# seung-lab/crackle

Hardware: AMD Instinct MI355X
Metric: voxels/s encode+decode, 1024x1024x512 uint32; bit-exact .ckl bytes (higher is better)
Workload: dtype u32

## Files before the change

### crackle_amd/_lib.py

```python
import ctypes as C
import os

HERE = os.path.dirname(os.path.abspath(__file__))
LIB_PATH = os.path.join(HERE, "libcrackle_amd_tuning.so" if os.environ.get("CKL_TUNING_LIB") else
                        ("libcrackle_amd_%s.so" % os.environ["CKL_LIB_AB"]) if os.environ.get("CKL_LIB_AB") else "libcrackle_amd.so")

CKL_OK, CKL_ERR_FORMAT, CKL_ERR_RUNTIME, CKL_ERR_ARG, CKL_ERR_NO_DEVICE, CKL_ERR_CRC = range(6)
MEM_HOST, MEM_DEVICE = 0, 1


class HeaderInfo(C.Structure):
  _fields_ = [
    ("format_version", C.c_uint32), ("label_format", C.c_uint32), ("crack_format", C.c_uint32),
    ("is_signed", C.c_uint32), ("data_width", C.c_uint32), ("stored_data_width", C.c_uint32),
    ("sx", C.c_uint32), ("sy", C.c_uint32), ("sz", C.c_uint32),
    ("fortran_order", C.c_uint32), ("markov_model_order", C.c_uint32), ("is_sorted", C.c_uint32),
    ("num_label_bytes", C.c_uint64), ("header_bytes", C.c_uint64),
  ]


MERGE_UNIQUE_FN = C.CFUNCTYPE(C.c_int, C.c_void_p, C.POINTER(C.c_uint64), C.c_uint64, C.POINTER(C.c_void_p), C.POINTER(C.c_uint64))


class EncodeOverrides(C.Structure):
# ... 7 lines not shown

EXPORTS = {
  "ckl_last_error": (C.c_char_p, []),
  "ckl_abi_version": (C.c_int, []),
  "ckl_device_count": (C.c_int, []),
  "ckl_header_info_from_bytes": (C.c_int, [C.c_char_p, C.c_uint64, C.POINTER(HeaderInfo)]),
  "ckl_compress": (C.c_int, [
    C.c_void_p, C.c_int, C.c_int, C.c_int, C.c_int64, C.c_int64, C.c_int64,
    C.c_int, C.c_int, C.c_uint64, C.c_int, C.c_int, C.c_int64,
    C.c_int, C.POINTER(C.c_void_p), C.POINTER(C.c_uint64)]),
  "ckl_free": (None, [C.c_void_p]),
  "ckl_decompress": (C.c_int, [
    C.c_void_p, C.c_uint64, C.c_void_p, C.c_uint64, C.c_int,
    C.c_int64, C.c_int64, C.c_int, C.c_uint64, C.c_int]),
  "ckl_decoder_create": (C.c_int, [C.c_void_p, C.c_uint64, C.c_int64, C.c_int64, C.c_int, C.POINTER(C.c_void_p)]),
  "ckl_decoder_create_device": (C.c_int, [C.c_void_p, C.c_uint64, C.c_int64, C.c_int64, C.c_int, C.POINTER(C.c_void_p)]),
  "ckl_encoder_keep_device_stream": (C.c_int, [C.c_void_p, C.c_int]),
  "ckl_encoder_async_host_copy": (C.c_int, [C.c_void_p, C.c_int]),
  "ckl_encoder_host_wait": (C.c_int, [C.c_void_p]),
  "ckl_encoder_device_stream": (C.c_int, [C.c_void_p, C.POINTER(C.c_void_p), C.POINTER(C.c_uint64)]),
  "ckl_decoder_run": (C.c_int, [C.c_void_p, C.c_void_p, C.c_uint64, C.c_int, C.c_uint64]),
  "ckl_decoder_label_stats": (C.c_int, [C.c_void_p, C.c_uint64, C.c_void_p, C.c_void_p, C.c_void_p, C.c_void_p, C.POINTER(C.c_uint64)]),
  "ckl_decoder_contacts": (C.c_int, [C.c_void_p, C.POINTER(C.c_void_p), C.POINTER(C.c_void_p), C.POINTER(C.c_uint64)]),
  "ckl_decoder_last_timing": (C.c_int, [C.c_void_p, C.POINTER(C.c_float), C.POINTER(C.c_float)]),
  "ckl_decoder_stage_timing": (C.c_int, [C.c_void_p, C.c_int, C.POINTER(C.c_char_p), C.POINTER(C.c_float)]),
  "ckl_decoder_set_stage_events": (C.c_int, [C.c_void_p, C.c_int]),
  "ckl_decoder_destroy": (None, [C.c_void_p]),
  "ckl_encoder_create": (C.c_int, [C.c_int64, C.c_int64, C.c_int64, C.c_int, C.c_int, C.POINTER(C.c_void_p)]),
  "ckl_encoder_run": (C.c_int, [
    C.c_void_p, C.c_void_p, C.c_int64, C.c_int64, C.c_int64,
    C.c_int, C.c_int, C.c_uint64, C.c_int, C.c_int, C.c_int64,
    C.POINTER(EncodeOverrides), C.POINTER(C.c_void_p), C.POINTER(C.c_uint64)]),
  "ckl_encoder_stats": (C.c_int, [
    C.c_void_p, C.c_void_p, C.c_int64, C.c_int64, C.c_int64,
    C.POINTER(C.c_uint64), C.POINTER(C.c_uint64), C.POINTER(C.c_uint64), C.POINTER(C.c_uint64)]),
  "ckl_encoder_markov_stats": (C.c_int, [
    C.c_void_p, C.c_void_p, C.c_int64, C.c_int64, C.c_int64, C.c_int, C.c_uint64, C.c_void_p]),
  "ckl_encoder_components": (C.c_int, [
    C.c_void_p, C.c_void_p, C.c_int64, C.c_int64, C.c_int64, C.c_uint32, C.c_void_p, C.c_void_p]),
  "ckl_encoder_components_device": (C.c_int, [
    C.c_void_p, C.c_void_p, C.c_int64, C.c_int64, C.c_int64, C.c_uint32, C.c_void_p, C.c_void_p]),
  "ckl_encoder_pin_labels": (C.c_int, [
    C.c_void_p, C.c_void_p, C.c_void_p, C.c_int64, C.c_int64, C.c_int64, C.c_void_p,
    C.c_int, C.c_int, C.c_int64, C.POINTER(C.c_void_p), C.POINTER(C.c_uint64)]),
  "ckl_pins_rows_first": (C.c_int, [C.c_void_p, C.c_void_p, C.c_void_p, C.c_int64, C.c_int64, C.c_int64, C.c_int64, C.c_uint64, C.c_void_p, C.c_void_p, C.c_void_p]),
  "ckl_pins_rows_best": (C.c_int, [C.c_void_p, C.c_void_p, C.c_void_p, C.c_int64, C.c_int64, C.c_int64, C.c_int64, C.c_uint64, C.c_void_p, C.c_void_p]),
  "ckl_pins_rows_extent": (C.c_int, [C.c_void_p, C.c_void_p, C.c_void_p, C.c_int64, C.c_int64, C.c_int64, C.c_int64, C.c_uint64, C.c_void_p, C.c_void_p, C.c_void_p, C.c_void_p]),
  "ckl_pins_rows_ids": (C.c_int, [C.c_void_p, C.c_void_p, C.c_int64, C.c_int64, C.c_int64, C.c_int64, C.c_uint64, C.c_void_p, C.c_void_p, C.c_void_p, C.c_void_p]),
  "ckl_pins_rows_section": (C.c_int, [C.c_void_p, C.c_int64, C.c_int64, C.c_int64, C.c_uint64, C.c_void_p, C.c_void_p, C.c_void_p, C.c_void_p, C.c_void_p, C.c_void_p, C.c_void_p,
                                       C.c_int, C.c_int, C.c_int64, C.POINTER(C.c_void_p), C.POINTER(C.c_uint64)]),
  "ckl_encoder_walk_step_kinds": (C.c_int, [C.c_void_p, C.POINTER(C.c_uint32), C.c_uint32, C.POINTER(C.c_uint32)]),
  "ckl_encoder_last_timing": (C.c_int, [C.c_void_p, C.POINTER(C.c_float), C.POINTER(C.c_float)]),
  "ckl_encoder_walk_paths": (C.c_int, [C.c_void_p, C.POINTER(C.c_uint32), C.POINTER(C.c_uint32)]),
  "ckl_encoder_destroy": (None, [C.c_void_p]),
  "ckl_pin_labels_host": (C.c_int, [
    C.c_void_p, C.c_int, C.c_void_p, C.c_int64, C.c_int64, C.c_int64, C.c_void_p,
    C.c_int, C.c_int, C.c_int64, C.POINTER(C.c_void_p), C.POINTER(C.c_uint64)]),
  "ckl_zstack": (C.c_int, [C.POINTER(C.c_char_p), C.POINTER(C.c_uint64), C.c_uint64, C.POINTER(C.c_void_p), C.POINTER(C.c_uint64)]),
  "ckl_decoder_check": (C.c_int, [C.c_void_p, C.c_void_p, C.c_uint64]),
  "ckl_decoder_vcg": (C.c_int, [C.c_void_p, C.c_void_p, C.c_uint64, C.c_int]),
  "ckl_voxel_connectivity_graph": (C.c_int, [C.c_void_p, C.c_uint64, C.c_int, C.c_int, C.c_void_p, C.c_uint64]),
  "ckl_voxel_connectivity_graph_range": (C.c_int, [C.c_void_p, C.c_uint64, C.c_int64, C.c_int64, C.c_int, C.c_int, C.c_void_p, C.c_uint64]),
  "ckl_point_cloud": (C.c_int, [
    C.c_void_p, C.c_uint64, C.c_int64, C.c_int64, C.c_void_p, C.c_uint64, C.c_int, C.c_int, C.c_int,
    C.POINTER(C.c_void_p), C.POINTER(C.c_void_p), C.POINTER(C.c_void_p), C.POINTER(C.c_uint64)]),
  "ckl_reencode_markov": (C.c_int, [C.c_void_p, C.c_uint64, C.c_int, C.c_int, C.POINTER(C.c_void_p), C.POINTER(C.c_uint64)]),
  "ckl_decoder_crack_planes": (C.c_int, [C.c_void_p, C.POINTER(C.c_void_p), C.POINTER(C.c_void_p), C.POINTER(C.c_uint32), C.POINTER(C.c_uint64)]),
  "ckl_zsplit": (C.c_int, [C.c_void_p, C.c_uint64, C.c_int64, C.c_int64, C.POINTER(C.c_void_p), C.POINTER(C.c_uint64)]),
  "ckl_encoder_defer_codes": (C.c_int, [C.c_void_p, C.c_int]),
  "ckl_encoder_codes_to_host": (C.c_int, [C.c_void_p, C.c_void_p, C.c_uint64, C.POINTER(C.c_uint64)]),
  "ckl_host_register": (C.c_int, [C.c_void_p, C.c_uint64]),
  "ckl_host_unregister": (C.c_int, [C.c_void_p]),
  "ckl_array_equal": (C.c_int, [C.c_void_p, C.c_uint64, C.c_void_p, C.c_uint64, C.c_int, C.POINTER(C.c_int)]),
  "ckl_mode_pooling_2x2x1": (C.c_int, [C.c_void_p, C.c_uint64, C.c_int64, C.c_int64, C.c_int, C.POINTER(C.c_void_p), C.POINTER(C.c_uint64), C.POINTER(C.c_void_p), C.POINTER(C.c_uint64)]),
  "ckl_crc32c": (C.c_uint32, [C.c_void_p, C.c_uint64]),
  "ckl_crc32c_combine": (C.c_uint32, [C.c_uint32, C.c_uint32, C.c_uint64]),
}

_lib = None


def lib():
  global _lib
  if _lib is None:
    if not os.path.exists(LIB_PATH):
      raise ImportError(
        f"{LIB_PATH} is missing: build the HIP extension first "
        "(python -m crackle_amd.build, or __graft_entry__.build()). "
        "crackle_amd has no CPU fallback."
      )
    L = C.CDLL(LIB_PATH)
    for name, (res, args) in EXPORTS.items():
      f = getattr(L, name)
      f.restype = res
      f.argtypes = args
    _lib = L
  return _lib


def last_error() -> str:
  return lib().ckl_last_error().decode("utf-8", "replace")


class HostStream:

  def __init__(self, ptr: int, n: int):
    self.ptr, self.n = int(ptr), int(n)

  def __len__(self):
    return self.n

  def view(self) -> memoryview:
    return memoryview((C.c_ubyte * self.n).from_address(self.ptr)).cast("B")

  def tobytes(self) -> bytes:
    return C.string_at(self.ptr, self.n)

  __bytes__ = tobytes

  def __eq__(self, other):
    if isinstance(other, HostStream):
      return self.tobytes() == other.tobytes()
    if isinstance(other, (bytes, bytearray, memoryview)):
      return self.tobytes() == bytes(other)
    return NotImplemented

  def __del__(self):
    try:
      if self.ptr:
        lib().ckl_free(self.ptr)
        self.ptr = 0
    except Exception:
      pass


def as_pointer(binary):
  if hasattr(binary, "ptr") and hasattr(binary, "n"):
    return binary.ptr, binary.n
  return binary, len(binary)
```

### crackle_amd/csrc/ckl_decode.hip

```cpp
#include "ckl_common.hpp"
#include "ckl_runs.hpp"
#include "ckl_strips.hpp"
#include "ckl_strips2.hpp"
#include "ckl_contours.hpp"
#include "ckl_pins.hpp"

#include <algorithm>
#include <deque>
#include <chrono>
#include <memory>
#include <mutex>
#include <type_traits>
#include <tuple>

namespace ckl {

using namespace dev;

enum : uint8_t { SYM_U = 0, SYM_R = 1, SYM_D = 2, SYM_L = 3, SYM_B = 4, SYM_T = 5 };

struct CrackArgs {
	const uint8_t* stream;
	const uint64_t* code_off;
	const uint32_t* code_len;
// ... 2369 lines not shown
		const uint64_t runs_cap = permissible ? d.sxy : std::min<uint64_t>(d.sxy, static_cast<uint64_t>(h.sy) + cap);
		cbase[zi] = ctot; ccap[zi] = static_cast<uint32_t>(cap); ctot += cap;
		est_codes += h.markov_model_order ? payload * 8 / 1.4 : payload * 4.0;
		nbase[zi] = ntot; ncap[zi] = static_cast<uint32_t>(nodes_cap); ntot += nodes_cap;
		rbase[zi] = rtot; rcap[zi] = static_cast<uint32_t>(runs_cap); rtot += runs_cap;
		d.max_rcap = std::max<uint32_t>(d.max_rcap, static_cast<uint32_t>(runs_cap));
	}
	pack.add(d.d_code_off, code_off);
	pack.add(d.d_code_len, code_len);
	pack.add(d.d_cbase, cbase);
	pack.add(d.d_ccap, ccap);
	pack.add(d.d_nbase, nbase);
	pack.add(d.d_ncap, ncap);
	pack.add(d.d_rbase, rbase);
	pack.add(d.d_rcap, rcap);
	std::vector<uint64_t> symbase(d.nslices, 0);
	{
		uint64_t stot = 0;
		for (uint32_t zi = 0; zi < d.nslices; zi++) {
			symbase[zi] = stot;
			const uint64_t tiles = static_cast<uint64_t>(ccap[zi]) / kCrackTile + 1;
			if (tiles > 1) stot += tiles * (4 * kCrackWords + 3) * kCrackBlock;
		}
		pack.add(d.d_symbase, symbase);
		d.d_symbuf.ensure(stot + 4);
	}
	std::vector<uint64_t> mkbase;
	if (h.markov_model_order) {
		d.d_upacked.ensure(ctot / 16 + 2ull * d.nslices + 4);
		mkbase.assign(d.nslices, 0);
		uint64_t mtot = 0;
		for (uint32_t zi = 0; zi < d.nslices; zi++) { mkbase[zi] = mtot; mtot += (code_len[zi] + 3ull) / 4 + 2 + ccap[zi] / 16 + 2; }
		pack.add(d.d_mkbase, mkbase);
		d.d_mkscratch.ensure(mtot + 4);
	}
	{
		const size_t ktot = ctot / 2 + 4ull * d.nslices + 8;
		d.d_ctl_kind.ensure(ktot); d.d_ctl_dx.ensure(ktot); d.d_ctl_dy.ensure(ktot);
		d.d_ctl_depth.ensure(ktot); d.d_ctl_lastT.ensure(ktot); d.d_ctl_link.ensure(ktot);
		d.d_seg_x.ensure(ktot); d.d_seg_y.ensure(ktot); d.d_ctl_gmin.ensure(ktot);
	}
	d.d_nodes.ensure(ntot);
	d.rtot = rtot;

	if (h.markov_model_order) {
		std::vector<uint8_t> model = markov_model_from_stored(buf + hb + gib + h.num_label_bytes, h.markov_model_bytes(), h.markov_model_order);
		pack.add(d.d_model, model);
	}

	d.row_words = (h.sx + 31) / 32;
	d.plane_words = static_cast<uint64_t>(d.row_words) * h.sy;
	d.d_planes.ensure(2 * d.plane_words * d.nslices);
	{
		d.strip_rows = std::max<uint32_t>(1u, kStripWords / d.row_words);
		if (!permissible && d.nslices) {
			const double runs_per_row = 1.0 + 0.5 * est_codes / (static_cast<double>(d.nslices) * h.sy);
			const uint32_t fit = static_cast<uint32_t>(0.7 * kStripCap / runs_per_row);
			d.strip_rows = std::max<uint32_t>(1u, std::min(d.strip_rows, fit));
		}
		if (const char* env = getenv("CKL_CCL_ROWS")) d.strip_rows = std::max<uint32_t>(1u, std::min<uint32_t>(kStripWords / d.row_words, static_cast<uint32_t>(std::max(1, atoi(env)))));
		d.nstrips = (h.sy + d.strip_rows - 1) / d.strip_rows;
		d.strip_ok = h.fortran_order && (h.sx % 4 == 0) && d.row_words <= kStripWords && d.nstrips <= kMaxStrips &&
			d.sxy < 0xFFFF0000ull && !getenv("CKL_DECODE_GENERAL");
		if (d.strip_ok) {
			const bool few = d.nslices <= static_cast<uint32_t>(std::max(1, d.n_cus));
			const size_t lds_share = few ? static_cast<size_t>(d.max_lds) - 8192u : static_cast<size_t>(d.max_lds) / 2u - 6144u;
			d.resolve_cap = static_cast<uint32_t>(std::min<size_t>(kResolveCap, (lds_share - (kMaxStrips + 64u) * 4u) / 4u));
			d.resolve_cap_max = static_cast<uint32_t>(std::min<size_t>(kResolveCap, (static_cast<size_t>(d.max_lds) - 8192u - (kMaxStrips + 64u) * 4u) / 4u));
			if (few && !getenv("CKL_LDS_CONTROLS")) {
				uint32_t nctl = 16384;
				while (nctl > 64 && rec_lds_bytes(nctl) > lds_share) nctl -= 64;
				if (rec_lds_bytes(nctl) <= lds_share && nctl > d.rec_lds_controls) {
					d.rec_lds_controls = nctl;
					d.rec_lds = lds_share & ~static_cast<size_t>(15);
					d.rec_block = kRecBlockWide;
					allow_dynamic_lds(reinterpret_cast<const void*>(&k_crack_match<kRecBlockWide>), d.device, d.rec_lds);
				}
			}
			const size_t nst = static_cast<size_t>(d.nstrips) * d.nslices;
			d.strip_cap = static_cast<uint32_t>(std::min<uint64_t>(kStripCap, static_cast<uint64_t>(d.strip_rows) * h.sx));
			d.d_row_run.ensure(static_cast<size_t>(h.sy) * d.nslices);
			d.d_strip_nruns.ensure(nst); d.d_strip_nsc.ensure(nst);
			d.d_seam_first.ensure(nst * d.row_words); d.d_seam_last.ensure(nst * d.row_words);
			d.d_run_lid.ensure(nst * d.strip_cap + 16); d.d_sc_w.ensure(nst * d.strip_cap);
			d.d_sc_label.ensure(nst * d.strip_cap);
			if (h.label_format != FLAT) d.d_sc_cc.ensure(nst * d.strip_cap);
			d.d_overflow.ensure(1);
			d.use_records = h.sx <= kRecMaxDim && h.sy <= kRecMaxDim && d.nstrips <= kRecMaxStrips && d.rec_lds_controls > 0 && !getenv("CKL_DECODE_RASTER");
			if (d.use_records) {
				const double per_strip = est_codes / 16.0 / (static_cast<double>(d.nslices) * d.nstrips);
				uint32_t cap = static_cast<uint32_t>(std::min<double>(per_strip * 3.0 + 256.0, 65536.0));
				if (const char* env = getenv("CKL_REC_CAP")) cap = static_cast<uint32_t>(std::max(1, atoi(env)));
				d.rec_cap = cap;
				d.d_rec.ensure(nst * cap);
				d.d_rec_count.ensure(nst);
				std::vector<uint64_t> word_off(d.nslices);
				uint64_t wtot = 0;
				d.max_words = 0;
				for (uint32_t zi = 0; zi < d.nslices; zi++) {
					const uint32_t nw = (ccap[zi] / rec_tile(d.rec_block) + 1u) * static_cast<uint32_t>(d.rec_block) * rec_words(d.rec_block);
					word_off[zi] = wtot; wtot += nw;
					d.max_words = std::max(d.max_words, nw);
				}
				pack.add(d.d_word_off, word_off);
				d.d_words.ensure(wtot);
			}
		}
	}
	d.d_ncomp.ensure(d.nslices);
	d.d_slice_err.ensure(d.nslices);
	d.d_crc_acc.ensure(d.nslices);

	struct PinBlock { uint8_t* p = nullptr; hipStream_t s = nullptr; ~PinBlock() { if (p) { (void)hipStreamSynchronize(s); host_out_free(p); } } } pin_block;
	pin_block.s = s;
	const uint8_t* lb = buf + hb + gib;
	const uint64_t nlb = h.num_label_bytes;
	const int sw = h.stored_data_width;
	const int component_width = byte_width(d.sxy);
	uint64_t offset;
	if (h.label_format == FLAT) {
		if (nlb < 8) throw Error(CKL_ERR_RUNTIME, "crackle: label section is malformed or corrupted.");
		d.num_unique = rd_le(lb, 8);
		d.uniq_offset = 8;
		if (d.num_unique > (nlb - 8) / sw) throw Error(CKL_ERR_RUNTIME, "crackle: label section is malformed or corrupted.");
		offset = 8 + static_cast<uint64_t>(sw) * d.num_unique;
	}
	else if (h.label_format == PINS_VARIABLE_WIDTH) {
		if (nlb < static_cast<uint64_t>(sw) + 8) throw Error(CKL_ERR_RUNTIME, "crackle: pin section is malformed or corrupted.");
		d.bgcolor = read_stored(h, lb, 0);
		d.num_unique = rd_le(lb + sw, 8);
		d.uniq_offset = static_cast<uint64_t>(sw) + 8;
		if (d.num_unique > (nlb - 8 - static_cast<uint64_t>(sw)) / sw) throw Error(CKL_ERR_RUNTIME, "crackle: pin section is malformed or corrupted.");
		offset = 8 + static_cast<uint64_t>(sw) * (d.num_unique + 1);
// ... 1671 lines not shown
```

### crackle_amd/csrc/ckl_encode.hip

```cpp
#include "ckl_common.hpp"
#include "ckl_runs.hpp"
#include "ckl_trail.hpp"
#include "ckl_pins_dev.hpp"

#include <algorithm>
#include <atomic>
#include <chrono>
#include <functional>
#include <memory>
#include <mutex>

namespace ckl {

using namespace dev;

template <typename LABEL>
__global__ void __launch_bounds__(kBlock) k_stats(const LABEL* __restrict__ labels, uint64_t voxels, unsigned long long* __restrict__ out ) {
	__shared__ unsigned long long s_max[kWaves], s_pairs[kWaves];
	unsigned long long mx = 0, pairs = 0;
	const uint64_t stride = static_cast<uint64_t>(gridDim.x) * kBlock;
	for (uint64_t i = static_cast<uint64_t>(blockIdx.x) * kBlock + threadIdx.x; i < voxels; i += stride) {
		const LABEL v = labels[i];
		if (static_cast<unsigned long long>(v) > mx) mx = v;
		if (i > 0) pairs += (labels[i - 1] == v);
	}
	for (int d = kWave / 2; d >= 1; d >>= 1) {
		const unsigned long long om = __shfl_xor(mx, d, kWave);
		const unsigned long long op = __shfl_xor(pairs, d, kWave);
		mx = om > mx ? om : mx;
		pairs += op;
	}
	const int lane = threadIdx.x & 63, wave = threadIdx.x >> 6;
	if (lane == 0) { s_max[wave] = mx; s_pairs[wave] = pairs; }
	__syncthreads();
	if (threadIdx.x == 0) {
		for (int w = 1; w < kWaves; w++) { mx = s_max[w] > mx ? s_max[w] : mx; pairs += s_pairs[w]; }
		atomicMax(out, mx);
		atomicAdd(out + 1, pairs);
	}
}

constexpr uint32_t kPlaneUnroll = 4;

template <typename LABEL>
__global__ void __launch_bounds__(kBlock) k_label_planes(
	const LABEL* __restrict__ labels, uint32_t sx, uint32_t sy, uint32_t chunks_per_row,
	uint32_t* __restrict__ planeV, uint32_t* __restrict__ planeH, uint32_t row_words, uint64_t plane_words,
	uint32_t* __restrict__ count_v, uint32_t* __restrict__ count_h
) {
	__shared__ uint32_t s_red[2 * kWaves];
	const uint32_t zi = blockIdx.y;
	const int lane = threadIdx.x & 63, wave = threadIdx.x >> 6;
	const uint32_t units = chunks_per_row * sy;
	const uint32_t unit0 = (blockIdx.x * kWaves + wave) * kPlaneUnroll;
	const LABEL* slice = labels + static_cast<uint64_t>(zi) * sy * sx;
	LABEL v[kPlaneUnroll], up[kPlaneUnroll], lf[kPlaneUnroll];
	uint32_t xs[kPlaneUnroll], ys[kPlaneUnroll];
#pragma unroll
	for (uint32_t k = 0; k < kPlaneUnroll; k++) {
		const uint32_t unit = unit0 + k;
		const uint32_t y = unit / chunks_per_row;
		const uint32_t x = (unit - y * chunks_per_row) * 64u + lane;
		xs[k] = x; ys[k] = y;
// ... 170 lines not shown
			}
			else {
				for (uint32_t q = 0; q < kVecWords; q++) if (word0 + w + q < row_words) { pv[at + q] = sv[r * WPR + w + q]; ph[at + q] = sh[r * WPR + w + q]; }
			}
		}
	}
	nv = wave_sum(nv); nh = wave_sum(nh); pairs = wave_sum(pairs);
	unsigned long long mx = static_cast<unsigned long long>(mxl);
	for (int d = kWave / 2; d >= 1; d >>= 1) { const unsigned long long o = __shfl_xor(mx, d, kWave); mx = o > mx ? o : mx; }
	if (lane == 0) { s_red[wave] = nv; s_red[kWaves + wave] = nh; s_red[2 * kWaves + wave] = pairs; s_max[wave] = mx; }
	__syncthreads();
	if (threadIdx.x == 0) {
		uint32_t tv = 0, th = 0, tp = 0;
		unsigned long long tm = 0;
		for (int w = 0; w < kWaves; w++) { tv += s_red[w]; th += s_red[kWaves + w]; tp += s_red[2 * kWaves + w]; tm = s_max[w] > tm ? s_max[w] : tm; }
		const uint64_t o = static_cast<uint64_t>(zi) * gridDim.x + blockIdx.x;
		partial[o * 4 + 0] = tv; partial[o * 4 + 1] = th; partial[o * 4 + 2] = tp; partial[o * 4 + 3] = 0;
		partial_max[o] = tm;
	}
}

__global__ void __launch_bounds__(kBlock) k_planes_from_cracks(
	const uint32_t* __restrict__ crackV, const uint32_t* __restrict__ crackH, uint32_t sx, uint32_t sy,
	uint32_t row_words, uint64_t plane_words, uint32_t permissible,
	uint32_t* __restrict__ planeV, uint32_t* __restrict__ planeH, uint32_t* __restrict__ counts, uint32_t nslices
) {
	__shared__ uint32_t s_red[kWaves];
	const uint32_t zi = blockIdx.y;
	const uint64_t i = static_cast<uint64_t>(blockIdx.x) * kBlock + threadIdx.x;
	uint32_t nv = 0, nh = 0;
	if (i < plane_words) {
		const uint32_t y = static_cast<uint32_t>(i / row_words);
		const uint32_t w = static_cast<uint32_t>(i - static_cast<uint64_t>(y) * row_words);
		const uint32_t left = sx - w * 32u;
		const uint32_t in_row = left >= 32u ? 0xFFFFFFFFu : ((1u << left) - 1u);
		const uint32_t mv = in_row & (w == 0 ? 0xFFFFFFFEu : 0xFFFFFFFFu);
		const uint32_t mh = y >= 1 ? in_row : 0u;
		const uint64_t at = zi * plane_words + i;
		const uint32_t inv = permissible ? 0xFFFFFFFFu : 0u;
		const uint32_t v = (crackV[at] ^ inv) & mv, h = (crackH[at] ^ inv) & mh;
		planeV[at] = v; planeH[at] = h;
		nv = __popc(v); nh = __popc(h);
	}
	nv = block_sum(nv, s_red); nh = block_sum(nh, s_red);
	if (threadIdx.x == 0) {
		if (nv) atomicAdd(counts + zi, nv);
		if (nh) atomicAdd(counts + nslices + zi, nh);
	}
}

__global__ void __launch_bounds__(kBlock) k_planes_reduce(
	const uint32_t* __restrict__ partial, const unsigned long long* __restrict__ partial_max, uint32_t nblk,
	unsigned long long* __restrict__ out ,
	unsigned long long* __restrict__ total_pairs
) {
	__shared__ uint32_t s_red[kWaves];
	__shared__ unsigned long long s_max[kWaves];
	const uint32_t zi = blockIdx.x;
	uint32_t tv = 0, th = 0, tp = 0;
	unsigned long long tm = 0;
	for (uint32_t b = threadIdx.x; b < nblk; b += kBlock) {
		const uint64_t o = static_cast<uint64_t>(zi) * nblk + b;
		tv += partial[o * 4 + 0]; th += partial[o * 4 + 1]; tp += partial[o * 4 + 2];
		const unsigned long long m = partial_max[o];
		tm = m > tm ? m : tm;
	}
	tv = block_sum(tv, s_red); th = block_sum(th, s_red); tp = block_sum(tp, s_red);
	for (int d = kWave / 2; d >= 1; d >>= 1) { const unsigned long long o = __shfl_xor(tm, d, kWave); tm = o > tm ? o : tm; }
	if ((threadIdx.x & 63) == 0) s_max[threadIdx.x >> 6] = tm;
	__syncthreads();
	if (threadIdx.x == 0) {
		for (int w = 0; w < kWaves; w++) tm = s_max[w] > tm ? s_max[w] : tm;
		out[4ull * zi + 0] = tv; out[4ull * zi + 1] = th; out[4ull * zi + 2] = tp; out[4ull * zi + 3] = tm;
		atomicAdd(total_pairs, static_cast<unsigned long long>(tp));
	}
}

enum : uint8_t { CODE_UP = 0, CODE_RIGHT = 1, CODE_DOWN = 2, CODE_LEFT = 3, CODE_NONE = 0xFE, CODE_TOMB = 0xFF };

struct FinishArgs {
	int sx, sy, xw, yw;
	uint32_t z0;
	uint32_t markov;
	const uint64_t* cbase;
	const uint64_t* kbase;
	const uint32_t* n_chains;
	const uint32_t* n_raw;
	const uint32_t* n_valid;
	const uint8_t* cp;
	const uint32_t* chain_node;
	const uint32_t* chain_off;
	const uint32_t* chain_clen;
	uint32_t* chain_order;
	uint32_t* chain_dst;
	uint32_t* chain_vstart;
	uint8_t* fcode;
	uint8_t* dcode;
	const uint64_t* pbase;
	uint8_t* payload;
	const uint64_t* bbase;
	uint8_t* boc;
	uint32_t* payload_len;
	uint32_t* boc_len;
};

__device__ __forceinline__ void put_le_dev(uint8_t* p, uint32_t v, int w) {
	for (int i = 0; i < w; i++) p[i] = static_cast<uint8_t>((v >> (8 * i)) & 0xFF);
}

constexpr int kFinishBlock = 1024;
constexpr int kFinishWaves = kFinishBlock / kWave;

constexpr uint32_t kFinishChains = 2048;

__global__ void __launch_bounds__(kFinishBlock) k_finish(FinishArgs a) {
	__shared__ uint32_t s_scan[kFinishWaves];
	__shared__ uint32_t s_node[kFinishChains], s_clen[kFinishChains], s_off[kFinishChains], s_ord[kFinishChains], s_dst[kFinishChains], s_vst[kFinishChains];
	const uint32_t zi = blockIdx.x + a.z0;
	const int tid = threadIdx.x;
	const uint32_t nch = a.n_chains[zi], nraw = a.n_raw[zi], nvalid = a.n_valid[zi];
	const uint8_t* cp = a.cp + a.cbase[zi];
	uint8_t* fcode = a.fcode + a.cbase[zi];
	const bool staged = nch <= kFinishChains;
	const uint32_t* ch_node = a.chain_node + a.kbase[zi];
	const uint32_t* ch_off = a.chain_off + a.kbase[zi];
	const uint32_t* ch_clen = a.chain_clen + a.kbase[zi];
// ... 205 lines not shown
		__syncthreads();
		for (uint32_t i = threadIdx.x; i < entries; i += kBlock) { const uint32_t v = s_hist[i]; if (v) atomicAdd(hist + i, v); }
	}
}

__global__ void __launch_bounds__(kBlock) k_markov_pack(
	const uint8_t* __restrict__ dcode, const uint64_t* __restrict__ cbase, const uint32_t* __restrict__ n_valid,
	int order, const uint8_t* __restrict__ model ,
	const uint64_t* __restrict__ pbase, uint8_t* __restrict__ payload, uint32_t* __restrict__ payload_len
) {
	__shared__ uint32_t s_scan[kWaves];
	const uint32_t zi = blockIdx.x;
	const uint8_t* d = dcode + cbase[zi];
	const uint32_t n = n_valid[zi];
	uint32_t* words = reinterpret_cast<uint32_t*>(payload + pbase[zi]);
	constexpr uint32_t kPer = 8;
	uint32_t carry = 0;
	for (uint32_t tile = 0; tile < n; tile += kBlock * kPer) {
		const uint32_t g0 = tile + threadIdx.x * kPer;
		uint32_t bits[kPer], lens[kPer], tot_len = 0;
#pragma unroll
		for (uint32_t k = 0; k < kPer; k++) {
			const uint32_t g = g0 + k;
			bits[k] = 0; lens[k] = 0;
			if (g < n) {
				if (g == 0) { bits[k] = d[0]; lens[k] = 2; }
				else {
					const uint32_t r = model[markov_ctx(d, g, order) * 4u + d[g]];
					bits[k] = (r == 0) ? 0u : (r == 1) ? 1u : (r == 2) ? 3u : 7u;
					lens[k] = (r == 0) ? 1u : (r == 1) ? 2u : 3u;
				}
			}
			tot_len += lens[k];
		}
		uint32_t v[1] = { tot_len }, tot[1];
		block_excl_add<1>(v, tot, s_scan);
		uint32_t off = carry + v[0];
#pragma unroll
		for (uint32_t k = 0; k < kPer; k++) {
			if (lens[k] && bits[k]) {
				const uint32_t w = off >> 5, sh = off & 31;
				atomicOr(words + w, bits[k] << sh);
				if (sh + lens[k] > 32) atomicOr(words + w + 1, bits[k] >> (32 - sh));
			}
			off += lens[k];
		}
		carry += tot[0];
	}
	if (threadIdx.x == 0) payload_len[zi] = (carry + 7) / 8;
}

template <typename LABEL>
__global__ void __launch_bounds__(kBlock) k_mapping_comps(
	const LABEL* __restrict__ labels, RunArrays r, uint64_t sxy,
	const uint64_t* __restrict__ comp_off, uint64_t* __restrict__ mapping
) {
	const uint32_t zi = blockIdx.y;
	const uint32_t c = blockIdx.x * kBlock + threadIdx.x;
	if (c >= r.ncomp[zi]) return;
	mapping[comp_off[zi] + c] = static_cast<uint64_t>(labels[zi * sxy + r.comp_pix[r.rbase[zi] + c]]);
}


__global__ void __launch_bounds__(kBlock) k_paint_components(
	const uint32_t* __restrict__ planeV, uint32_t row_words, uint64_t plane_words, uint32_t sx, uint64_t sxy,
	const uint32_t* __restrict__ word_base, const uint64_t* __restrict__ rbase, const uint32_t* __restrict__ run_cc,
	const uint64_t* __restrict__ comp_off, uint32_t id_base, uint32_t* __restrict__ out
) {
	const uint32_t zi = blockIdx.y;
	const uint32_t px = blockIdx.x * kBlock + threadIdx.x;
	if (px >= sxy) return;
	const uint32_t y = px / sx, x = px - y * sx;
	const uint32_t w = x >> 5, bit = x & 31u;
	const uint64_t wi = zi * plane_words + static_cast<uint64_t>(y) * row_words + w;
	uint32_t b = planeV[wi];
	if (w == 0) b |= 1u;
	const uint32_t run = word_base[wi] - 1u + __popc(b & (0xFFFFFFFFu >> (31u - bit)));
	out[zi * sxy + px] = run_cc[rbase[zi] + run] + static_cast<uint32_t>(comp_off[zi]) + id_base;
}

__global__ void __launch_bounds__(kBlock) k_paint_components4(
	const uint32_t* __restrict__ planeV, uint32_t row_words, uint64_t plane_words, uint32_t sx, uint64_t sxy,
	const uint32_t* __restrict__ word_base, const uint64_t* __restrict__ rbase, const uint32_t* __restrict__ run_cc,
	const uint64_t* __restrict__ comp_off, uint32_t id_base, uint32_t* __restrict__ out
) {
	const uint32_t zi = blockIdx.y;
	const uint32_t px = (blockIdx.x * kBlock + threadIdx.x) * 4u;
	if (px >= sxy) return;
	const uint32_t y = px / sx, x = px - y * sx;
	const uint32_t w = x >> 5, bit = x & 31u;
	const uint64_t wi = zi * plane_words + static_cast<uint64_t>(y) * row_words + w;
	uint32_t b = planeV[wi];
	if (w == 0) b |= 1u;
	const uint32_t* cc = run_cc + rbase[zi];
	const uint32_t add = static_cast<uint32_t>(comp_off[zi]) + id_base;
	uint32_t run = word_base[wi] - 1u + __popc(b & (0xFFFFFFFFu >> (31u - bit)));
	uint4 o;
	o.x = cc[run] + add;
	run += (b >> (bit + 1u)) & 1u; o.y = cc[run] + add;
	run += (b >> (bit + 2u)) & 1u; o.z = cc[run] + add;
	run += (b >> (bit + 3u)) & 1u; o.w = cc[run] + add;
	*reinterpret_cast<uint4*>(out + zi * sxy + px) = o;
}

inline void launch_paint_components(hipStream_t s, const uint32_t* planeV, uint32_t row_words, uint64_t plane_words, int64_t sx, int64_t sy, int64_t sz,
	const uint32_t* word_base, const uint64_t* rbase, const uint32_t* run_cc, const uint64_t* comp_off, uint32_t id_base, uint32_t* out) {
	const uint64_t sxy = static_cast<uint64_t>(sx) * sy;
	const bool four = sx % 4 == 0 && (reinterpret_cast<uintptr_t>(out) & 15u) == 0;
	const uint64_t threads = four ? sxy / 4 : sxy;
	const dim3 grid(static_cast<uint32_t>((threads + kBlock - 1) / kBlock), static_cast<uint32_t>(sz));
	if (four) hipLaunchKernelGGL(k_paint_components4, grid, dim3(kBlock), 0, s, planeV, row_words, plane_words, static_cast<uint32_t>(sx), sxy, word_base, rbase, run_cc, comp_off, id_base, out);
	else hipLaunchKernelGGL(k_paint_components, grid, dim3(kBlock), 0, s, planeV, row_words, plane_words, static_cast<uint32_t>(sx), sxy, word_base, rbase, run_cc, comp_off, id_base, out);
}
// ... 329 lines not shown
	hipLaunchKernelGGL(k_copy_bytes, dim3(blocks), dim3(kBlock), 0, s, src, dst, n);
}

struct VolumeStats { uint64_t max_label = 0, pairs = 0, first = 0, last = 0; };

struct ckl_encoder {
	int device = 0;
	hipStream_t stream = nullptr;
	hipStream_t stream2 = nullptr;
	hipEvent_t ev0 = nullptr, ev1 = nullptr, evk0 = nullptr, evk1 = nullptr, ev_in = nullptr;
	hipEvent_t evd0 = nullptr, evd1 = nullptr;
	float trail_ms = 0.f;
	hipEvent_t ev_prezero = nullptr;
	float pipeline_ms = 0.f, dominant_ms = 0.f;
	int64_t max_sx = 0, max_sy = 0, max_sz = 0;
	int dtype_bytes = 0;

	DevBuf<unsigned long long> d_stats;
	DevBuf<uint4> d_adjm;
	DevBuf<uint32_t> d_slice_err;
	DevBuf<uint64_t> d_cbase, d_sbase, d_kbase, d_pbase, d_bbase, d_out_off, d_comp_off;
	DevBuf<uint32_t> d_ccap, d_scap, d_kcap;
	DevBuf<uint8_t> d_crack_tables;
	DevBuf<uint8_t> d_cp, d_fcode, d_dcode, d_payload, d_boc, d_codes_out, d_model;
	DevBuf<uint32_t> d_code_report;
	uint64_t codes_capacity = 0;
	bool defer_codes = false;
	bool keep_device_stream = false;
	bool async_host_copy = false;
	bool host_copy_pending = false;
	hipStream_t stream_copy = nullptr;
	hipStream_t stream_tab = nullptr;
	hipEvent_t ev_codes = nullptr;
	void* tables_staging = nullptr;
	bool uploads_by_kernel = false;
	hipEvent_t ev_labels_crc = nullptr;
	DevBuf<uint32_t> d_labels_crc;
	DevBuf<uint8_t> d_stream_out;
	uint64_t device_stream_bytes = 0;
	uint64_t last_codes_total = 0;
	DevBuf<uint32_t> d_stack_node, d_stack_code;
	DevBuf<uint32_t> d_chain_node, d_chain_off, d_chain_clen, d_chain_order, d_chain_dst, d_chain_vstart;
	DevBuf<uint32_t> d_n_chains, d_n_raw, d_n_valid, d_payload_len, d_boc_len;
	DevBuf<uint32_t> d_hist;
	DevBuf<uint32_t> d_planes, d_count_vh;
	uint32_t row_words = 0;
	uint64_t plane_words = 0;
	std::vector<uint32_t> count_v, count_h;
	DevBuf<uint64_t> d_rbase;
	DevBuf<uint32_t> d_rcap, d_word_base, d_parent, d_run_start, d_run_cc, d_comp_pix, d_nruns, d_ncomp, d_idbits, d_blk_roots;
	DevBuf<uint16_t> d_run_local;
	DevBuf<uint32_t> d_G, d_crc_acc;
	DevBuf<uint32_t> d_flat_report;
	uint64_t g_table_pixels = 0;
	DevBuf<uint64_t> d_mapping, d_sorted, d_uniq, d_label_hash, d_label_list;
	DevBuf<uint8_t> d_keys;
	DevBuf<uint32_t> d_cc_volume;
	DevBuf<uint32_t> d_pin_kept, d_pin_u32;
	DevBuf<uint8_t> d_pin_tables;
	DevBuf<uint64_t> d_pin_u64;
	DevBuf<uint32_t> d_slice_err2, d_n_uniq, d_uniq_blk;
	DevBuf<uint8_t> d_labels_bin;
	uint32_t flat_max_rcap = 0;
	const void* planes_for = nullptr;
	const void* trail_for = nullptr;
	bool trail_perm = false;
	int trail_order = 0;
	VolumeStats planes_stats;
	int64_t planes_dims[3] = { 0, 0, 0 };
	std::vector<uint64_t> h_rbase;
	std::vector<uint32_t> h_rcap;
	std::vector<uint32_t> count_special, count_corner;
	DevBuf<uint32_t> d_plane_partial, t_blk_special, t_blk_corner;
	DevBuf<unsigned long long> d_plane_partial_max, d_plane_out;
	uint32_t graph_blocks = 0;
	uint32_t tiles_x = 0, tiles_y = 0, mtx2 = 0;
	uint64_t adjm_stride = 0;
	bool graph_permissible = false;
	bool planes_deferred = false;
	bool trail_zeroed = false;
	DevBuf<uint64_t> t_nbase, t_cobase, t_ibase;
	DevBuf<uint32_t> t_ncap, t_cocap, t_icap, t_max_steps;
	size_t last_trail_slices = 0;
	DevBuf<uint32_t> t_counters;
	DevBuf<uint32_t> t_node_vertex, t_vert2node, t_corner_vertex;
	DevBuf<uint8_t> t_node_adj;
	DevBuf<uint32_t> t_dart_end, t_dart_len, t_dart_minv, t_dart_minpos, t_parent, t_start_bits, t_starts;
	DevBuf<uint4> t_dart_codes;
	DevBuf<uint8_t> t_dart_inline;
	DevBuf<unsigned long long> t_compmin;
	DevBuf<uint32_t> t_items, t_item_off, t_chain_item0, t_events, t_chain_ev0, t_ev_lnd, t_ev_item;

	~ckl_encoder() {
		if (ev0) (void)hipEventDestroy(ev0);
		if (ev1) (void)hipEventDestroy(ev1);
		if (evk0) (void)hipEventDestroy(evk0);
		if (evk1) (void)hipEventDestroy(evk1);
		if (evd0) (void)hipEventDestroy(evd0);
		if (evd1) (void)hipEventDestroy(evd1);
		if (ev_in) (void)hipEventDestroy(ev_in);
		if (ev_prezero) (void)hipEventDestroy(ev_prezero);
		if (stream) (void)hipStreamDestroy(stream);
		if (stream2) (void)hipStreamDestroy(stream2);
		if (stream_copy) { (void)hipStreamSynchronize(stream_copy); (void)hipStreamDestroy(stream_copy); }
		if (stream_tab) { (void)hipStreamSynchronize(stream_tab); (void)hipStreamDestroy(stream_tab); }
		if (ev_codes) (void)hipEventDestroy(ev_codes);
		if (tables_staging) host_out_free(tables_staging);
		if (ev_labels_crc) (void)hipEventDestroy(ev_labels_crc);
	}
};

namespace {

template <typename T>
void upload(DevBuf<T>& d, const std::vector<T>& h, hipStream_t s) {
	d.ensure(h.size());
	if (!h.empty()) CKL_HIP(hipMemcpyAsync(d.p, h.data(), h.size() * sizeof(T), hipMemcpyHostToDevice, s));
}
struct UploadPacker {
	struct Item { void* buf; size_t off, count; void (*bind)(void*, uint8_t*, size_t); };
	std::vector<Item> items;
	std::vector<uint8_t> image;
	template <typename T>
	void add(DevBuf<T>& dst, const std::vector<T>& src) {
		const size_t off = (image.size() + 255) & ~static_cast<size_t>(255);
		image.resize(off + std::max<size_t>(src.size(), 1) * sizeof(T));
		if (!src.empty()) memcpy(image.data() + off, src.data(), src.size() * sizeof(T));
		items.push_back({ &dst, off, src.size(), [](void* b, uint8_t* base, size_t n) { static_cast<DevBuf<T>*>(b)->borrow(reinterpret_cast<T*>(base), n); } });
	}
	void commit(DevBuf<uint8_t>& block, hipStream_t s, void** staging = nullptr) {
		if (image.empty()) return;
		for (const Item& it : items) it.bind(it.buf, nullptr, 0);
		block.ensure(image.size());
		if (staging) {
			if (*staging) host_out_free(*staging);
			*staging = host_out_alloc(std::max<size_t>(image.size(), 64u << 10));
			memcpy(*staging, image.data(), image.size());
			upload_small(block.p, *staging, image.size(), s, *staging);
		}
		else CKL_HIP(hipMemcpyAsync(block.p, image.data(), image.size(), hipMemcpyHostToDevice, s));
		for (const Item& it : items) it.bind(it.buf, block.p + it.off, it.count);
	}
};

template <typename T>
std::vector<T> download(const T* p, size_t n, hipStream_t s) {
	std::vector<T> h(n);
	if (n) CKL_HIP(hipMemcpyAsync(h.data(), p, n * sizeof(T), hipMemcpyDeviceToHost, s));
	CKL_HIP(hipStreamSynchronize(s));
	return h;
}


template <typename LABEL>
VolumeStats volume_stats(ckl_encoder& e, const LABEL* labels, uint64_t voxels) {
	VolumeStats st;
	if (voxels == 0) return st;
	hipStream_t s = e.stream;
	e.d_stats.ensure(2);
	CKL_HIP(hipMemsetAsync(e.d_stats.p, 0, 2 * sizeof(unsigned long long), s));
	const uint32_t blocks = static_cast<uint32_t>(std::min<uint64_t>((voxels + kBlock - 1) / kBlock, 256ull * 8));
	hipLaunchKernelGGL(k_stats<LABEL>, dim3(blocks), dim3(kBlock), 0, s, labels, voxels, e.d_stats.p);
	auto r = download(e.d_stats.p, 2, s);
	st.max_label = r[0]; st.pairs = r[1];
	LABEL f, l;
// ... 33 lines not shown
	std::vector<unsigned long long> mine;
	if (!fetched) { mine = download(e.d_plane_out.p, 4ull * ns, e.stream); fetched = &mine; }
	const std::vector<unsigned long long>& o = *fetched;
	e.count_v.resize(ns); e.count_h.resize(ns);
	VolumeStats v;
	for (uint32_t zi = 0; zi < ns; zi++) {
		e.count_v[zi] = static_cast<uint32_t>(o[4ull * zi]);
		e.count_h[zi] = static_cast<uint32_t>(o[4ull * zi + 1]);
		v.pairs += o[4ull * zi + 2];
		v.max_label = std::max<uint64_t>(v.max_label, o[4ull * zi + 3]);
	}
	e.planes_deferred = false;
	if (st) *st = v;
}

void trail_prezero(ckl_encoder& e, int64_t sx, int64_t sy, int64_t sz) {
	hipStream_t s = e.stream2;
	const uint32_t ns = static_cast<uint32_t>(sz);
	const uint64_t nverts = static_cast<uint64_t>(sx + 1) * (sy + 1);
	const uint32_t start_words = static_cast<uint32_t>((nverts + 31) / 32);
	e.d_slice_err.ensure(ns);
	e.t_counters.ensure(7 * static_cast<size_t>(ns));
	e.t_start_bits.ensure(static_cast<size_t>(start_words) * ns);
	CKL_HIP(hipMemsetAsync(e.d_slice_err.p, 0, ns * sizeof(uint32_t), s));
	CKL_HIP(hipMemsetAsync(e.t_counters.p, 0, 7 * static_cast<size_t>(ns) * sizeof(uint32_t), s));
	CKL_HIP(hipMemsetAsync(e.t_start_bits.p, 0, static_cast<size_t>(start_words) * ns * sizeof(uint32_t), s));
	CKL_HIP(hipEventRecord(e.ev_prezero, s));
	e.trail_zeroed = true;
}

template <typename LABEL>
void planes_pass(ckl_encoder& e, const LABEL* labels, int64_t sx, int64_t sy, int64_t sz, VolumeStats* st, bool defer = false) {
	hipStream_t s = e.stream;
	const uint32_t ns = static_cast<uint32_t>(sz);
	e.trail_zeroed = false;
	e.planes_deferred = false;
	e.row_words = static_cast<uint32_t>((sx + 31) / 32);
	e.plane_words = static_cast<uint64_t>(e.row_words) * sy;
	e.d_planes.ensure(2 * e.plane_words * ns);
	constexpr uint32_t P = 16 / sizeof(LABEL);
	const bool fast = !getenv("CKL_PLANES_GENERIC") && sx >= static_cast<int64_t>(P) && sx % P == 0 && (reinterpret_cast<uintptr_t>(labels) & 15u) == 0;
	if (fast) {
		const uint32_t strips = static_cast<uint32_t>((sx + 64 * P - 1) / (64 * P));
		const uint32_t bands = static_cast<uint32_t>((sy + kBandRows - 1) / kBandRows);
		const uint32_t nblk = (strips * bands + kWaves - 1) / kWaves;
		e.d_plane_partial.ensure(4ull * nblk * ns);
		e.d_plane_partial_max.ensure(static_cast<size_t>(nblk) * ns);
		e.d_plane_out.ensure(4ull * ns + 1);
		trail_prezero(e, sx, sy, sz);
		hipLaunchKernelGGL(k_label_planes_stream<LABEL>, dim3(nblk, ns), dim3(kBlock), 0, s,
			labels, static_cast<uint32_t>(sx), static_cast<uint32_t>(sy), strips, bands,
			e.d_planes.p, e.d_planes.p + e.plane_words * ns, e.row_words, e.plane_words,
			e.d_plane_partial.p, e.d_plane_partial_max.p, e.d_plane_out.p + 4ull * ns);
		hipLaunchKernelGGL(k_planes_reduce, dim3(ns), dim3(kBlock), 0, s, e.d_plane_partial.p, e.d_plane_partial_max.p, nblk, e.d_plane_out.p, e.d_plane_out.p + 4ull * ns);
		e.planes_deferred = defer;
		if (!e.planes_deferred) planes_collect(e, ns, st);
		return;
	}
	if (st) *st = volume_stats<LABEL>(e, labels, static_cast<uint64_t>(sx) * sy * sz);
	e.d_count_vh.ensure(2 * static_cast<size_t>(ns));
	CKL_HIP(hipMemsetAsync(e.d_count_vh.p, 0, 2 * static_cast<size_t>(ns) * sizeof(uint32_t), s));
	const uint32_t chunks = static_cast<uint32_t>((sx + 63) / 64);
	const uint64_t units = static_cast<uint64_t>(chunks) * sy;
	hipLaunchKernelGGL(k_label_planes<LABEL>, dim3(static_cast<uint32_t>((units + kWaves * kPlaneUnroll - 1) / (kWaves * kPlaneUnroll)), ns), dim3(kBlock), 0, s,
		labels, static_cast<uint32_t>(sx), static_cast<uint32_t>(sy), chunks,
		e.d_planes.p, e.d_planes.p + e.plane_words * ns, e.row_words, e.plane_words,
		e.d_count_vh.p, e.d_count_vh.p + ns);
	std::vector<uint32_t> c = download(e.d_count_vh.p, 2 * static_cast<size_t>(ns), s);
	e.count_v.assign(c.begin(), c.begin() + ns);
	e.count_h.assign(c.begin() + ns, c.end());
}

void graph_pass(ckl_encoder& e, int64_t sx, int64_t sy, int64_t sz, int perm_mode, VolumeStats* st = nullptr) {
	hipStream_t s = e.stream;
	const uint32_t ns = static_cast<uint32_t>(sz);
	e.tiles_x = static_cast<uint32_t>((sx + 1 + kTrailTileDim - 1) / kTrailTileDim);
	e.tiles_y = static_cast<uint32_t>((sy + 1 + 7) / 8);
	const uint32_t mtx = static_cast<uint32_t>((sx + 1 + 7) / 8), mty = static_cast<uint32_t>((sy + 1 + 7) / 8);
	e.mtx2 = (mtx + 1) / 2;
	e.adjm_stride = static_cast<uint64_t>(e.mtx2) * ((mty + 1) / 2) * 4 * 2;
	e.d_adjm.ensure(e.adjm_stride * ns);
	e.graph_blocks = (e.tiles_x * e.tiles_y + kBlock - 1) / kBlock;
	e.t_blk_special.ensure(static_cast<size_t>(e.graph_blocks) * ns);
	e.t_blk_corner.ensure(static_cast<size_t>(e.graph_blocks) * ns);
	e.d_count_vh.ensure(4 * static_cast<size_t>(ns));
	if (perm_mode == 2 && !e.planes_deferred) throw Error(CKL_ERR_RUNTIME, "crackle_amd: internal: crack format left to the device without deferred counts");
	const unsigned long long half_voxels = static_cast<unsigned long long>(static_cast<int64_t>(static_cast<uint64_t>(sx) * sy * sz) / 2);
	hipLaunchKernelGGL(k_trail_graph, dim3(e.graph_blocks, ns), dim3(kBlock), 0, s,
		e.d_planes.p, e.d_planes.p + e.plane_words * ns, e.row_words, e.plane_words,
		static_cast<uint32_t>(sx), static_cast<uint32_t>(sy), static_cast<uint32_t>(perm_mode),
		perm_mode == 2 ? e.d_plane_out.p + 4ull * ns : nullptr, half_voxels,
		reinterpret_cast<uint32_t*>(e.d_adjm.p), e.adjm_stride * 4,
		e.mtx2, e.tiles_x, e.tiles_y, e.t_blk_special.p, e.t_blk_corner.p);
	hipLaunchKernelGGL(k_trail_count_scan, dim3(ns), dim3(kBlock), 0, s, e.t_blk_special.p, e.t_blk_corner.p, e.graph_blocks,
		e.d_count_vh.p + 2 * static_cast<size_t>(ns), e.d_count_vh.p + 3 * static_cast<size_t>(ns));
	std::vector<unsigned long long> po;
	if (e.planes_deferred) {
		po.resize(4ull * ns);
		CKL_HIP(hipMemcpyAsync(po.data(), e.d_plane_out.p, po.size() * sizeof(unsigned long long), hipMemcpyDeviceToHost, s));
	}
	std::vector<uint32_t> c = download(e.d_count_vh.p + 2 * static_cast<size_t>(ns), 2 * static_cast<size_t>(ns), s);
	e.count_special.assign(c.begin(), c.begin() + ns);
	e.count_corner.assign(c.begin() + ns, c.end());
	VolumeStats v;
	if (!po.empty()) planes_collect(e, ns, &v, &po);
	if (st && !po.empty()) *st = v;
	e.graph_permissible = perm_mode == 2 ? static_cast<int64_t>(v.pairs) < static_cast<int64_t>(static_cast<uint64_t>(sx) * sy * sz) / 2 : perm_mode == 1;
}

struct CrackResult {
	std::vector<uint32_t> code_len;
	uint64_t total = 0;
	bool any_chain = false;
};

inline size_t trail_walk_lds(uint32_t max_special) { return (static_cast<size_t>(max_special) + 256) * 16 + 1024; }

void crack_pass(
	ckl_encoder& e, int64_t sx, int64_t sy, int64_t sz, bool permissible,
	int markov_order, bool hist_only, const std::vector<uint8_t>* model_in,
	std::vector<uint32_t>* hist_out, std::vector<uint8_t>* model_out, CrackResult* result,
	const std::function<void()>& overlap = std::function<void()>(), bool reuse_trail = false
) {
	hipStream_t s = e.stream;
	const uint32_t ns = static_cast<uint32_t>(sz);
	const uint64_t nverts = static_cast<uint64_t>(sx + 1) * (sy + 1);
	e.d_slice_err.ensure(ns);
	const bool prezeroed = e.trail_zeroed && !reuse_trail;
	e.trail_zeroed = false;
	if (prezeroed) CKL_HIP(hipStreamWaitEvent(s, e.ev_prezero, 0));
	if (!reuse_trail && !prezeroed) CKL_HIP(hipMemsetAsync(e.d_slice_err.p, 0, ns * sizeof(uint32_t), s));
	const uint64_t interior = static_cast<uint64_t>(sx > 0 ? sx - 1 : 0) * sy + static_cast<uint64_t>(sx) * (sy > 0 ? sy - 1 : 0);

	std::vector<uint64_t> cbase(ns), sbase(ns), kbase(ns);
	std::vector<uint32_t> ccap(ns), scap(ns), kcap(ns), max_steps(ns);
	std::vector<uint64_t> nbase(ns), cobase(ns), ibase(ns);
	std::vector<uint32_t> ncap(ns), cocap(ns), icap(ns);
	uint64_t ctot = 0, stot = 0, ktot = 0, ntot = 0, cotot = 0, itot = 0;
	uint32_t max_ncap = 0, max_cocap = 0, max_icap = 0, max_special = 0;
	bool any = false;
	for (uint32_t zi = 0; zi < ns; zi++) {
		const uint64_t differ = static_cast<uint64_t>(e.count_v[zi]) + e.count_h[zi];
		const uint64_t E = permissible ? interior - differ : differ;
		any = any || E > 0;
		const uint64_t cc = ((7 * E + 16 + 15) / 16) * 16;
		if (cc > 0xFFFFFFF0ull) throw Error(CKL_ERR_RUNTIME, "crackle_amd: slice has too many crack edges");
		cbase[zi] = ctot; ccap[zi] = static_cast<uint32_t>(cc); ctot += cc;
		max_steps[zi] = static_cast<uint32_t>(E + 1);
		const uint64_t nc = ((static_cast<uint64_t>(e.count_special[zi]) + e.count_corner[zi] + 16) / 16) * 16;
		if (nc >= (1ull << 28)) throw Error(CKL_ERR_RUNTIME, "crackle_amd: slice has too many crack vertices");
		nbase[zi] = ntot; ncap[zi] = static_cast<uint32_t>(nc); ntot += nc;
		cobase[zi] = cotot; cocap[zi] = e.count_corner[zi]; cotot += e.count_corner[zi];
		const uint64_t ic = 7 * nc + 16;
		ibase[zi] = itot; icap[zi] = static_cast<uint32_t>(ic); itot += ic;
// ... 52 lines not shown
	fa.cp = e.d_cp.p; fa.chain_node = e.d_chain_node.p; fa.chain_off = e.d_chain_off.p; fa.chain_clen = e.d_chain_clen.p;
	fa.chain_order = e.d_chain_order.p; fa.chain_dst = e.d_chain_dst.p; fa.chain_vstart = e.d_chain_vstart.p;
	fa.fcode = e.d_fcode.p; fa.dcode = e.d_dcode.p;
	fa.pbase = e.d_pbase.p; fa.payload = e.d_payload.p; fa.bbase = e.d_bbase.p; fa.boc = e.d_boc.p;
	fa.payload_len = e.d_payload_len.p; fa.boc_len = e.d_boc_len.p;

	unsigned long long* ta_dbg = nullptr;
	size_t trail_lds_used = 0;
	DevBuf<unsigned long long> d_tdbg;
	CKL_HIP(hipEventRecord(e.evk0, s));
	if (!reuse_trail) {
		e.t_counters.ensure(7 * static_cast<size_t>(ns));
		if (!prezeroed) CKL_HIP(hipMemsetAsync(e.t_counters.p, 0, 7 * static_cast<size_t>(ns) * sizeof(uint32_t), s));
		e.t_node_vertex.ensure(ntot); e.t_node_adj.ensure(ntot + 16); e.t_vert2node.ensure(nverts * ns);
		e.t_corner_vertex.ensure(cotot);
		e.t_dart_end.ensure(4 * ntot); e.t_dart_len.ensure(4 * ntot); e.t_dart_minv.ensure(4 * ntot); e.t_dart_minpos.ensure(4 * ntot);
		e.t_dart_codes.ensure(4 * ntot); e.t_dart_inline.ensure(4 * ntot);
		e.t_parent.ensure(ntot); e.t_compmin.ensure(ntot); e.t_starts.ensure(ntot);
		const uint32_t start_words = static_cast<uint32_t>((nverts + 31) / 32);
		e.t_start_bits.ensure(static_cast<size_t>(start_words) * ns);
		if (!prezeroed) CKL_HIP(hipMemsetAsync(e.t_start_bits.p, 0, static_cast<size_t>(start_words) * ns * sizeof(uint32_t), s));
		e.t_items.ensure(itot); e.t_item_off.ensure(itot); e.t_chain_item0.ensure(ktot);
		e.t_events.ensure(itot); e.t_chain_ev0.ensure(ktot); e.t_ev_lnd.ensure(itot); e.t_ev_item.ensure(itot);

		TrailArgs ta;
		ta.adjm = e.d_adjm.p; ta.adjm_stride = e.adjm_stride; ta.mtx2 = e.mtx2; ta.tiles_x = e.tiles_x; ta.tiles_y = e.tiles_y;
		ta.planeV = e.d_planes.p; ta.planeH = e.d_planes.p + e.plane_words * ns; ta.row_words = e.row_words; ta.plane_words = e.plane_words;
		ta.sx = static_cast<uint32_t>(sx); ta.sy = static_cast<uint32_t>(sy); ta.inv = e.graph_permissible ? 0xFFFFFFFFu : 0u;
		ta.sxe = static_cast<uint32_t>(sx + 1); ta.sye = static_cast<uint32_t>(sy + 1); ta.nverts = static_cast<uint32_t>(nverts);
		ta.max_steps = e.t_max_steps.p;
		ta.nbase = e.t_nbase.p; ta.ncap = e.t_ncap.p;
		ta.n_nodes = e.t_counters.p; ta.n_corners = e.t_counters.p + 2 * ns;
		ta.n_starts = e.t_counters.p + 3 * ns; ta.n_items = e.t_counters.p + 4 * ns;
		ta.node_vertex = e.t_node_vertex.p; ta.node_adj = e.t_node_adj.p; ta.vert2node = e.t_vert2node.p;
		ta.cobase = e.t_cobase.p; ta.cocap = e.t_cocap.p; ta.corner_vertex = e.t_corner_vertex.p;
		ta.dart_end = e.t_dart_end.p; ta.dart_len = e.t_dart_len.p; ta.dart_minv = e.t_dart_minv.p; ta.dart_minpos = e.t_dart_minpos.p;
		ta.dart_codes = e.t_dart_codes.p; ta.dart_inline = e.t_dart_inline.p;
		ta.parent = e.t_parent.p; ta.compmin = e.t_compmin.p;
		ta.start_bits = e.t_start_bits.p; ta.start_words = start_words; ta.starts = e.t_starts.p;
		ta.ibase = e.t_ibase.p; ta.icap = e.t_icap.p; ta.items = e.t_items.p; ta.item_off = e.t_item_off.p;
		ta.sbase = e.d_sbase.p; ta.scap = e.d_scap.p; ta.stack_node = e.d_stack_node.p; ta.stack_item = e.d_stack_code.p;
		ta.kbase = e.d_kbase.p; ta.kcap = e.d_kcap.p;
		ta.chain_node = e.d_chain_node.p; ta.chain_item0 = e.t_chain_item0.p; ta.chain_off = e.d_chain_off.p; ta.chain_clen = e.d_chain_clen.p;
		ta.n_chains = e.d_n_chains.p; ta.n_raw = e.d_n_raw.p; ta.n_valid = e.d_n_valid.p;
		ta.cbase = e.d_cbase.p; ta.ccap = e.d_ccap.p; ta.cp = e.d_cp.p; ta.slice_err = e.d_slice_err.p;

		e.last_trail_slices = ns;
		ta.events = e.t_events.p; ta.n_events = e.t_counters.p + 5 * ns; ta.seg_len_sum = e.t_counters.p + 6 * ns; ta.chain_ev0 = e.t_chain_ev0.p; ta.ev_lnd = e.t_ev_lnd.p; ta.ev_item = e.t_ev_item.p;
		ta.dbg = nullptr;
		{ const char* env = getenv("CKL_TRAIL_WALK"); ta.walk_plain = (env && !strcmp(env, "plain")) ? 1u : 0u; ta.walk_no_regs = (env && !strcmp(env, "lds")) ? 1u : 0u; }
		{ const char* env = getenv("CKL_TRAIL_WALK_STACK"); ta.walk_stack_cap = env ? static_cast<uint32_t>(std::max(1, atoi(env))) : 0xFFFFFFFFu; }
		if (kTuning && getenv("CKL_TRAIL_DIAG")) { d_tdbg.ensure(16); CKL_HIP(hipMemsetAsync(d_tdbg.p, 0, 128, s)); ta.dbg = d_tdbg.p; ta_dbg = d_tdbg.p; }
		ta.graph_blocks = e.graph_blocks; ta.blk_special = e.t_blk_special.p; ta.blk_corner = e.t_blk_corner.p;
		int max_lds = 0;
		CKL_HIP(hipDeviceGetAttribute(&max_lds, hipDeviceAttributeMaxSharedMemoryPerBlock, e.device));
		const size_t budget = static_cast<size_t>(max_lds > 1024 ? max_lds - 1024 : 0);
		const uint32_t dart_blocks = (4 * max_ncap + kWalkChunk * kWaves - 1) / (kWalkChunk * kWaves);
		size_t clds = (static_cast<size_t>(max_special) + 1024) * 4;
		if (const char* env = getenv("CKL_TRAIL_LDS")) clds = static_cast<size_t>(std::max(0, atoi(env)));
		clds = (std::min(budget, std::max<size_t>(clds, 1024)) / 16) * 16;
		CKL_HIP(hipFuncSetAttribute(reinterpret_cast<const void*>(&k_trail_components), hipFuncAttributeMaxDynamicSharedMemorySize, static_cast<int>(clds)));
		size_t lds = trail_walk_lds(max_special);
		if (const char* env = getenv("CKL_TRAIL_LDS")) lds = static_cast<size_t>(std::max(0, atoi(env)));
		lds = std::min(budget, std::max<size_t>(lds, 4096));
		lds = (lds / 16) * 16;
		CKL_HIP(hipFuncSetAttribute(reinterpret_cast<const void*>(&k_trail_walk), hipFuncAttributeMaxDynamicSharedMemorySize, static_cast<int>(lds)));
		trail_lds_used = lds;
		HT_MARK("c:setup");

		ta.z0 = 0;
		fa.z0 = 0;
		if (any) {
			hipLaunchKernelGGL(k_trail_nodes, dim3(e.graph_blocks, ns), dim3(kBlock), 0, s, ta);
			hipLaunchKernelGGL(k_trail_segments, dim3(dart_blocks, ns), dim3(kBlock), 0, s, ta);
			if (max_cocap) hipLaunchKernelGGL(k_trail_loops, dim3((max_cocap + kBlock - 1) / kBlock, ns), dim3(kBlock), 0, s, ta);
			hipLaunchKernelGGL(k_trail_components, dim3(ns), dim3(kCompBlock), clds, s, ta, static_cast<uint32_t>(clds));
		}
		CKL_HIP(hipEventRecord(e.evd0, s));
		hipLaunchKernelGGL(k_trail_walk, dim3(ns), dim3(kWave), lds, s, ta, static_cast<uint32_t>(lds));
		CKL_HIP(hipEventRecord(e.evd1, s));
		hipLaunchKernelGGL(k_trail_items, dim3(ns), dim3(kItemsBlock), 0, s, ta);
		hipLaunchKernelGGL(k_trail_offsets, dim3(ns), dim3(kBlock), 0, s, ta);
		hipLaunchKernelGGL(k_trail_expand, dim3((max_icap + kExpandChunk * kWaves - 1) / (kExpandChunk * kWaves), ns), dim3(kBlock), 0, s, ta);
		hipLaunchKernelGGL(k_finish, dim3(ns), dim3(kFinishBlock), 0, s, fa);
	}
	CKL_HIP(hipEventRecord(e.evk1, s));
	HT_MARK("c:enqueue");
	if (kTuning && getenv("CKL_TRAIL_DIAG")) {
		std::vector<uint32_t> c = download(e.t_counters.p, 5 * static_cast<size_t>(ns), s);
		double m[5] = { 0 };
		for (int k = 0; k < 5; k++) for (uint32_t zi = 0; zi < ns; zi++) m[k] += static_cast<double>(c[static_cast<size_t>(k) * ns + zi]) / ns;
		double sp = 0, co = 0;
		for (uint32_t zi = 0; zi < ns; zi++) { sp += static_cast<double>(e.count_special[zi]) / ns; co += static_cast<double>(e.count_corner[zi]) / ns; }
		if (ta_dbg) {
			std::vector<unsigned long long> g = download(ta_dbg, 16, s);
			if (g[11]) fprintf(stderr, "[ckl trail diag, k_trail_walk] mean cycles per slice: table fill=%.0f fill + walk=%.0f\n", static_cast<double>(g[6]) / g[11], static_cast<double>(g[7]) / g[11]);
			if (g[11]) fprintf(stderr, "[ckl trail diag, k_trail_walk] slices=%llu iterations/slice=%.0f cycles/iteration=%.0f clock=%.2f GHz (cycles / 100 MHz ticks)\n",
				g[11], static_cast<double>(g[8]) / g[11], g[8] ? static_cast<double>(g[9]) / g[8] : 0.0, g[10] ? static_cast<double>(g[9]) / (g[10] * 10.0) : 0.0);
			fprintf(stderr, "[ckl trail diag, k_trail_components, mean cycles per slice] union=%.0f component minima=%.0f starts/splits=%.0f bitmap scan=%.0f\n",
				static_cast<double>(g[12]) / ns, static_cast<double>(g[13]) / ns, static_cast<double>(g[14]) / ns, static_cast<double>(g[15]) / ns);
			fprintf(stderr, "[ckl trail diag, k_trail_segments] waves=%llu iterations/wave mean=%.1f max=%llu cycles/wave mean=%.0f max=%llu cycles/iteration=%.0f active lanes/iteration=%.1f\n",
				g[4], g[4] ? static_cast<double>(g[0]) / g[4] : 0.0, g[1], g[4] ? static_cast<double>(g[2]) / g[4] : 0.0, g[3],
				g[0] ? static_cast<double>(g[2]) / g[0] : 0.0, g[0] ? static_cast<double>(g[5]) / g[0] : 0.0);
		}
		fprintf(stderr, "[ckl trail diag] max degree-1/3/4 vertices of a slice=%u, k_trail_walk LDS=%zu bytes\n", max_special, trail_lds_used);
		fprintf(stderr, "[ckl trail diag, mean per slice] degree-1/3/4 vertices=%.0f corners=%.0f nodes=%.0f starts=%.0f items=%.0f\n", sp, co, m[0], m[3], m[4]);
	}

	const bool early_tail = !markov_order && result != nullptr;
	auto enqueue_tail = [&]() {
		e.d_out_off.ensure(ns);
		e.d_code_report.ensure(static_cast<size_t>(ns) + 3);
		e.d_codes_out.ensure(e.codes_capacity + 8);
		hipLaunchKernelGGL(k_code_offsets, dim3(1), dim3(kBlock), 0, s, e.d_boc_len.p, e.d_payload_len.p, e.d_slice_err.p, ns, e.d_out_off.p, e.d_code_report.p);
		hipLaunchKernelGGL(k_gather_codes, dim3(ns), dim3(kBlock), 0, s, e.d_boc.p, e.d_bbase.p, e.d_boc_len.p,
			e.d_payload.p, e.d_pbase.p, e.d_payload_len.p, e.d_out_off.p, e.d_codes_out.p);
	};
	if (early_tail) enqueue_tail();
	if (overlap) overlap();
// ... 44 lines not shown
}

struct FlatResult {
	std::vector<uint32_t> ncomp;
	std::vector<uint32_t> crcs;
	uint64_t total = 0;
};

void ensure_geom_table(ckl_encoder& e, uint64_t sxy) {
	if (e.g_table_pixels == sxy && e.d_G.p) return;
	hipStream_t s = e.stream2;
	const uint32_t npx = static_cast<uint32_t>(sxy);
	const uint32_t B = 1024, nblk = npx / B + 1;
	std::vector<uint32_t> g_base(B), blk_g(nblk), blk_x(nblk);
	const uint32_t X = gf_xpow(32);
	g_base[0] = 0;
	for (uint32_t i = 1; i < B; i++) g_base[i] = gf_mul(X, g_base[i - 1] ^ 0x80000000u);
	const uint32_t gB = gf_mul(X, g_base[B - 1] ^ 0x80000000u);
	const uint32_t XB = gf_xpow(32ull * B);
	blk_g[0] = 0; blk_x[0] = 0x80000000u;
	for (uint32_t k = 1; k < nblk; k++) {
		blk_g[k] = blk_g[k - 1] ^ gf_mul(blk_x[k - 1], gB);
		blk_x[k] = gf_mul(blk_x[k - 1], XB);
	}
	DevBuf<uint32_t> t_base, t_g, t_x;
	upload(t_base, g_base, s); upload(t_g, blk_g, s); upload(t_x, blk_x, s);
	e.d_G.ensure(static_cast<size_t>(npx) + 1);
	hipLaunchKernelGGL(k_build_geom_table, dim3(npx / kBlock + 1), dim3(kBlock), 0, s, t_base.p, t_g.p, t_x.p, npx, e.d_G.p);
	CKL_HIP(hipStreamSynchronize(s));
	e.g_table_pixels = sxy;
}

void flat_enqueue(ckl_encoder& e, int64_t sx, int64_t sy, int64_t sz) {
	hipStream_t s = e.stream2;
	const uint32_t ns = static_cast<uint32_t>(sz);
	const uint64_t sxy = static_cast<uint64_t>(sx) * sy;
	ensure_geom_table(e, sxy);

	std::vector<uint64_t>& rbase = e.h_rbase;
	std::vector<uint32_t>& rcap = e.h_rcap;
	rbase.assign(ns, 0); rcap.assign(ns, 0);
	uint64_t rtot = 0;
	uint32_t max_rcap = 0;
	for (uint32_t zi = 0; zi < ns; zi++) {
		const uint64_t runs = static_cast<uint64_t>(sy) + e.count_v[zi];
		rbase[zi] = rtot; rcap[zi] = static_cast<uint32_t>(runs); rtot += runs;
		max_rcap = std::max<uint32_t>(max_rcap, static_cast<uint32_t>(runs));
	}
	e.flat_max_rcap = max_rcap;
	upload(e.d_rbase, rbase, s); upload(e.d_rcap, rcap, s);
	e.d_word_base.ensure(e.plane_words * ns);
	e.d_parent.ensure(rtot); e.d_run_start.ensure(rtot); e.d_run_cc.ensure(rtot); e.d_comp_pix.ensure(rtot);
	e.d_nruns.ensure(ns);
	e.d_flat_report.ensure(4 * static_cast<size_t>(ns));
	e.d_ncomp.borrow(e.d_flat_report.p, ns); e.d_crc_acc.borrow(e.d_flat_report.p + ns, ns);
	e.d_idbits.borrow(e.d_flat_report.p + 2 * static_cast<size_t>(ns), ns); e.d_slice_err2.borrow(e.d_flat_report.p + 3 * static_cast<size_t>(ns), ns);
	CKL_HIP(hipMemsetAsync(e.d_slice_err2.p, 0, ns * sizeof(uint32_t), s));

	RunGeom g;
	g.planeV = e.d_planes.p; g.planeH = e.d_planes.p + e.plane_words * ns;
	g.row_words = e.row_words; g.plane_words = e.plane_words;
	g.flip = 1u;
	g.sx = static_cast<uint32_t>(sx); g.sy = static_cast<uint32_t>(sy);
	RunArrays ra;
	ra.word_base = e.d_word_base.p; ra.rbase = e.d_rbase.p; ra.rcap = e.d_rcap.p;
	ra.parent = e.d_parent.p; ra.run_start = e.d_run_start.p; ra.run_cc = e.d_run_cc.p;
	ra.nruns = e.d_nruns.p; ra.ncomp = e.d_ncomp.p; ra.slice_err = e.d_slice_err2.p;
	ra.comp_pix = e.d_comp_pix.p;
	hipLaunchKernelGGL(k_run_index, dim3(ns), dim3(kIndexBlock), 0, s, g, ra);
	launch_run_union(s, ns, g, ra);
	ResolveScratch rs;
	rs.nblk = (max_rcap + kBlock - 1) / kBlock;
	e.d_run_local.ensure(rtot);
	e.d_blk_roots.ensure(static_cast<size_t>(rs.nblk) * ns);
	rs.run_local = e.d_run_local.p; rs.blk_roots = e.d_blk_roots.p;
	launch_run_resolve(s, ns, ra, rs, e.d_G.p, static_cast<uint32_t>(sxy), 0u, e.d_crc_acc.p, e.d_idbits.p);
	HT_MARK("f:enqueue");
}

template <typename LABEL>
void flat_collect(ckl_encoder& e, const LABEL* labels, int64_t sx, int64_t sy, int64_t sz, FlatResult& out) {
	hipStream_t s = e.stream2;
	const uint32_t ns = static_cast<uint32_t>(sz);
	const uint64_t sxy = static_cast<uint64_t>(sx) * sy;
	std::vector<uint32_t> acc, idbits, errs;
	if (e.d_ncomp.p == e.d_flat_report.p && e.d_flat_report.p) {
		const std::vector<uint32_t> rep = download(e.d_flat_report.p, 4 * static_cast<size_t>(ns), s);
		out.ncomp.assign(rep.begin(), rep.begin() + ns);
		acc.assign(rep.begin() + ns, rep.begin() + 2 * static_cast<size_t>(ns));
		idbits.assign(rep.begin() + 2 * static_cast<size_t>(ns), rep.begin() + 3 * static_cast<size_t>(ns));
		errs.assign(rep.begin() + 3 * static_cast<size_t>(ns), rep.end());
		HT_MARK("f:wait");
	}
	else {
		out.ncomp = download(e.d_ncomp.p, ns, s);
		HT_MARK("f:wait");
		acc = download(e.d_crc_acc.p, ns, s);
		idbits = download(e.d_idbits.p, ns, s);
		errs = download(e.d_slice_err2.p, ns, s);
	}
	for (uint32_t zi = 0; zi < ns; zi++) if (errs[zi]) throw Error(CKL_ERR_RUNTIME, "crackle_amd: run table overflow on z=" + std::to_string(zi));
	const uint32_t init_term = gf_mul(0xFFFFFFFFu, gf_xpow(32ull * sxy));
	out.crcs.resize(ns);
	uint32_t fix_bits = 0xFFFFFFFFu, fix = 0;
	for (uint32_t zi = 0; zi < ns; zi++) {
		if (idbits[zi] != fix_bits) { fix_bits = idbits[zi]; fix = gf_xpow(32 - fix_bits); }
		out.crcs[zi] = ~(gf_mul(acc[zi], fix) ^ init_term);
	}

	std::vector<uint64_t> comp_off(ns);
	uint64_t total = 0;
	for (uint32_t zi = 0; zi < ns; zi++) { comp_off[zi] = total; total += out.ncomp[zi]; }
	upload(e.d_comp_off, comp_off, s);
	e.d_mapping.ensure(total + 1);
	RunArrays ra;
	ra.word_base = e.d_word_base.p; ra.rbase = e.d_rbase.p; ra.rcap = e.d_rcap.p;
	ra.parent = e.d_parent.p; ra.run_start = e.d_run_start.p; ra.run_cc = e.d_run_cc.p;
	ra.nruns = e.d_nruns.p; ra.ncomp = e.d_ncomp.p; ra.slice_err = e.d_slice_err2.p;
	ra.comp_pix = e.d_comp_pix.p;
	uint32_t max_ncomp = 1;
	for (uint32_t zi = 0; zi < ns; zi++) max_ncomp = std::max(max_ncomp, out.ncomp[zi]);
	hipLaunchKernelGGL(k_mapping_comps<LABEL>, dim3((max_ncomp + kBlock - 1) / kBlock, ns), dim3(kBlock), 0, s,
		labels, ra, sxy, e.d_comp_off.p, e.d_mapping.p);
	CKL_HIP(hipStreamSynchronize(s));
	out.total = total;
}

struct PinLabelLists {
	DevBuf<uint64_t> d_tab;
	DevBuf<uint32_t> d_count;
	uint32_t slots = 0;
	hipEvent_t ready = nullptr;
	~PinLabelLists() { if (ready) (void)hipEventDestroy(ready); }
};
void pin_label_table_enqueue(ckl_encoder& e, const uint64_t* comp_label, const uint64_t* first_any_dev, uint64_t N, PinLabelLists& t) {
	hipStream_t s = e.stream2;
	if (N > (1ull << 30)) throw Error(CKL_ERR_RUNTIME, "crackle_amd: too many components for pin labels");
	uint32_t slots = 1024;
	while (slots < 2 * N) slots <<= 1;
	t.slots = slots;
	t.d_tab.ensure(4ull * slots + 1);
	t.d_count.ensure(1);
	CKL_HIP(hipMemsetAsync(t.d_tab.p, 0xFF, (2ull * slots) * sizeof(uint64_t), s));
	CKL_HIP(hipMemsetAsync(t.d_tab.p + 4ull * slots, 0xFF, sizeof(uint64_t), s));
	CKL_HIP(hipMemsetAsync(t.d_count.p, 0, sizeof(uint32_t), s));
	unsigned long long* tab = reinterpret_cast<unsigned long long*>(t.d_tab.p);
	hipLaunchKernelGGL(k_pin_label_first, dim3(static_cast<uint32_t>((N + kPinBlock - 1) / kPinBlock)), dim3(kPinBlock), 0, s,
		reinterpret_cast<const unsigned long long*>(comp_label), reinterpret_cast<const unsigned long long*>(first_any_dev), N, tab, tab + slots, slots - 1u, tab + 4ull * slots);
	hipLaunchKernelGGL(k_pin_label_list, dim3((slots + kPinBlock - 1) / kPinBlock), dim3(kPinBlock), 0, s, tab, tab + slots, slots, t.d_count.p, tab + 2ull * slots, tab + 3ull * slots);
	if (!t.ready) CKL_HIP(hipEventCreateWithFlags(&t.ready, hipEventDisableTiming));
	CKL_HIP(hipEventRecord(t.ready, s));
}
void pin_label_table_collect(ckl_encoder& e, PinLabelLists& t, PinCandidates& pc) {
	if (!e.stream_tab) CKL_HIP(hipStreamCreateWithFlags(&e.stream_tab, hipStreamNonBlocking));
	hipStream_t s = e.stream_tab;
	CKL_HIP(hipStreamWaitEvent(s, t.ready, 0));
	const uint32_t nl = download(t.d_count.p, 1, s)[0];
	pc.label_value = download(t.d_tab.p + 2ull * t.slots, nl, s);
	pc.label_first = download(t.d_tab.p + 3ull * t.slots, nl, s);
	const uint64_t max_first = download(t.d_tab.p + 4ull * t.slots, 1, s)[0];
	if (max_first != kPinNoKey) { pc.label_value.push_back(kPinNoKey); pc.label_first.push_back(max_first); }
}
void pin_label_table(ckl_encoder& e, const uint64_t* comp_label, const uint64_t* first_any_dev, uint64_t N, PinCandidates& pc) {
	PinLabelLists t;
	pin_label_table_enqueue(e, comp_label, first_any_dev, N, t);
	pin_label_table_collect(e, t, pc);
}

template <typename LABEL>
void pin_dedup_pass(ckl_encoder& e, const LABEL* labels, const PinVolume& v) {
	hipStream_t s = e.stream2;
	const bool by_thread = getenv("CKL_PINS_ROW_THREADS") != nullptr;
	if (v.sz <= 1024u && !by_thread) {
		const dim3 wgrid((v.sy + kPinWaves - 1) / kPinWaves), wblock(64 * kPinWaves);
		const bool groups = v.sx % 4u == 0 && (reinterpret_cast<uintptr_t>(labels) % (4 * sizeof(LABEL))) == 0 && !getenv("CKL_PINS_COLUMN_LOADS");
#define CKL_DEDUP(K) do { \
			if (groups) hipLaunchKernelGGL((k_pin_dedup_wave<LABEL, K, 4>), wgrid, wblock, 0, s, labels, v); \
			else hipLaunchKernelGGL((k_pin_dedup_wave<LABEL, K, 1>), wgrid, wblock, 0, s, labels, v); \
// ... 384 lines not shown
		hipLaunchKernelGGL(k_unique_scatter, dim3(ub), dim3(kBlock), 0, s, e.d_sorted.p, static_cast<uint32_t>(n_sort), e.d_uniq_blk.p, e.d_uniq.p);
	}
	}
	uint64_t uniq_bound = N;
	if (ov && ov->merge_unique) {
		HT_MARK("l:enqueue");
		const uint32_t n_local = merge_unsorted ? static_cast<uint32_t>(n_sort) : download(e.d_n_uniq.p, 1, s)[0];
		std::vector<uint64_t> local = download(merge_unsorted ? e.d_label_list.p : e.d_uniq.p, n_local, s);
		HT_MARK("l:local");
		const uint64_t* merged = nullptr;
		uint64_t n_merged = 0;
		if (ov->merge_unique(ov->merge_ctx, local.data(), n_local, &merged, &n_merged) != 0 || (!merged && n_merged))
			throw Error(CKL_ERR_RUNTIME, "crackle_amd: the merge_unique callback failed");
		HT_MARK("l:merge");
		if (n_merged < n_local || n_merged > 0xFFFFFFFFull) throw Error(CKL_ERR_ARG, "crackle_amd: merge_unique returned a list that cannot contain the slab's labels");
		e.d_uniq.ensure(n_merged + 1);
		if (n_merged) CKL_HIP(hipMemcpyAsync(e.d_uniq.p, merged, n_merged * sizeof(uint64_t), hipMemcpyHostToDevice, s));
		const uint32_t nm = static_cast<uint32_t>(n_merged);
		CKL_HIP(hipMemcpyAsync(e.d_n_uniq.p, &nm, sizeof(uint32_t), hipMemcpyHostToDevice, s));
		CKL_HIP(hipStreamSynchronize(s));
		e.d_labels_bin.ensure(8 + n_merged * static_cast<uint64_t>(stored_width) + static_cast<uint64_t>(ns) * component_width + N * 4 + 16);
		uniq_bound = std::max<uint64_t>(uniq_bound, n_merged);
	}
	e.d_labels_bin.ensure(8 + N * static_cast<uint64_t>(stored_width) + static_cast<uint64_t>(ns) * component_width + N * 4 + 16);
	const uint64_t work = std::max<uint64_t>(std::max<uint64_t>(uniq_bound, ns), 1);
	hipLaunchKernelGGL(k_flat_section, dim3(static_cast<uint32_t>((work + kBlock - 1) / kBlock)), dim3(kBlock), 0, s,
		e.d_uniq.p, e.d_n_uniq.p, stored_width, e.d_ncomp.p, ns, component_width, e.d_mapping.p, static_cast<uint32_t>(N), e.d_labels_bin.p);
	HT_MARK("l:enqueue");
	const uint32_t nu = download(e.d_n_uniq.p, 1, s)[0];
	HT_MARK("l:wait");
	return 8 + static_cast<uint64_t>(nu) * stored_width + static_cast<uint64_t>(ns) * component_width + N * static_cast<uint64_t>(byte_width(nu));
}

template <typename LABEL>
void encode_typed(
	ckl_encoder& e, const LABEL* labels, int64_t sx, int64_t sy, int64_t sz,
	bool allow_pins, bool fortran_order, uint64_t markov_model_order,
	bool optimize_pins, bool auto_bgcolor, int64_t manual_bgcolor,
	const ckl_encode_overrides* ov, uint8_t** out, uint64_t* out_len
) {
	const uint64_t voxels = static_cast<uint64_t>(sx) * sy * sz;
	hipStream_t s = e.stream;
	CKL_HIP(hipEventRecord(e.ev0, s));

	HostTimer ht;
	g_ht = &ht;
	VolumeStats st;
	e.trail_zeroed = false;
	const bool planes_cached = ov && voxels > 0 && e.planes_for == static_cast<const void*>(labels)
		&& e.planes_dims[0] == sx && e.planes_dims[1] == sy && e.planes_dims[2] == sz;
	e.planes_for = nullptr;
	const bool labels_first = getenv("CKL_NO_OVERLAP") || static_cast<uint64_t>(sx) * sy > (1536ull * 1536ull)
		|| (getenv("CKL_LABELS_AT_WALK") && atoi(getenv("CKL_LABELS_AT_WALK")) == 0);
	if (voxels > 0 && !planes_cached) planes_pass<LABEL>(e, labels, sx, sy, sz, &st, !labels_first);
	else if (planes_cached) st = e.planes_stats;
	ht.mark("planes");
	bool graph_done = false;
	if (e.planes_deferred) {
		int perm_mode = 2;
		if (ov && ov->force_crack_format >= 0) perm_mode = ov->force_crack_format == PERMISSIBLE ? 1 : 0;
		e.trail_for = nullptr;
		graph_pass(e, sx, sy, sz, perm_mode, &st);
		graph_done = true;
		ht.mark("graph");
	}
	int stored_width = byte_width(st.max_label);
	if (ov && ov->force_stored_width) stored_width = ov->force_stored_width;

	Header head;
	head.crack_format = IMPERMISSIBLE;
	head.label_format = PINS_VARIABLE_WIDTH;
	if (static_cast<int64_t>(st.pairs) < static_cast<int64_t>(voxels) / 2) {
		head.crack_format = PERMISSIBLE;
		head.label_format = FLAT;
	}
	if (ov && ov->force_crack_format >= 0) {
		head.crack_format = ov->force_crack_format;
		head.label_format = ov->force_crack_format == PERMISSIBLE ? FLAT : PINS_VARIABLE_WIDTH;
	}
	if (sz == 1 || !allow_pins) head.label_format = FLAT;
	if (ov && ov->force_label_format >= 0) head.label_format = ov->force_label_format;
	e.uploads_by_kernel = head.label_format == FLAT;
	head.is_signed = false;
	head.data_width = static_cast<int>(sizeof(LABEL));
	head.stored_data_width = stored_width;
	head.sx = static_cast<uint32_t>(sx); head.sy = static_cast<uint32_t>(sy); head.sz = static_cast<uint32_t>(sz);
	head.log2_grid_size = 31;
	head.fortran_order = fortran_order;
	head.markov_model_order = static_cast<int>(markov_model_order & 0xFF);
	head.is_sorted = true;

	if (voxels == 0) {
		std::vector<uint8_t> hb;
		head.write(hb);
		uint8_t* o = static_cast<uint8_t*>(malloc(hb.size()));
		if (!o) throw Error(CKL_ERR_RUNTIME, "crackle_amd: out of host memory");
		memcpy(o, hb.data(), hb.size());
		*out = o; *out_len = hb.size();
		return;
	}
	if (optimize_pins) throw Error(CKL_ERR_ARG, "crackle_amd: allow_pins=2 (find_optimal_pins) is out of scope");
	if (head.label_format != FLAT && head.label_format != PINS_VARIABLE_WIDTH) throw Error(CKL_ERR_ARG, "crackle_amd: unsupported label format");
	if (head.markov_model_order > 13) throw Error(CKL_ERR_ARG, "crackle_amd: markov_model_order > 13 is not supported on device");

	bool labels_at_walk = false;
	if (labels_first && !graph_done) flat_enqueue(e, sx, sy, sz);
	const bool trail_cached = !graph_done && planes_cached && ov && ov->has_model && head.markov_model_order > 0 && e.trail_for == static_cast<const void*>(labels)
		&& e.trail_perm == (head.crack_format == PERMISSIBLE) && e.trail_order == head.markov_model_order;
	e.trail_for = nullptr;
	if (graph_done && e.graph_permissible != (head.crack_format == PERMISSIBLE)) throw Error(CKL_ERR_RUNTIME, "crackle_amd: internal: device and host disagree on the crack format");
	if (!trail_cached && !graph_done) graph_pass(e, sx, sy, sz, head.crack_format == PERMISSIBLE ? 1 : 0);
	ht.mark("graph");
	if (!labels_first) {
		uint32_t max_special = 0;
		for (uint32_t v : e.count_special) max_special = std::max(max_special, v);
		int max_lds = 0;
		CKL_HIP(hipDeviceGetAttribute(&max_lds, hipDeviceAttributeMaxSharedMemoryPerBlock, e.device));
		labels_at_walk = max_special < 5000 && 2 * trail_walk_lds(max_special) + 40960 <= static_cast<size_t>(max_lds);
		if (!labels_at_walk) flat_enqueue(e, sx, sy, sz);
	}

	const bool permissible = head.crack_format == PERMISSIBLE;
	{
		const uint64_t interior = static_cast<uint64_t>(sx > 0 ? sx - 1 : 0) * sy + static_cast<uint64_t>(sx) * (sy > 0 ? sy - 1 : 0);
		bool any = false;
		for (int64_t z = 0; z < sz && !any; z++) {
			const uint64_t differ = static_cast<uint64_t>(e.count_v[z]) + e.count_h[z];
			any = (permissible ? interior - differ : differ) > 0;
		}
		if (!any && !(ov && ov->has_model)) head.markov_model_order = 0;
	}
	std::vector<uint8_t> forced_model;
	const std::vector<uint8_t>* model_in = nullptr;
	if (ov && ov->has_model && head.markov_model_order > 0) {
		const size_t rows = static_cast<size_t>(1) << (2 * head.markov_model_order);
		forced_model.assign(ov->model, ov->model + rows * 4);
		model_in = &forced_model;
	}

	FlatResult fr;
	std::vector<uint8_t> pins_binary;
	uint64_t label_bytes = 0;
	const uint64_t off_index = Header::kBytes;
	const uint64_t off_labels = off_index + 4ull * (sz + 1);
	uint64_t est_code_bytes = 0;
	{
		const uint64_t interior = static_cast<uint64_t>(sx > 0 ? sx - 1 : 0) * sy + static_cast<uint64_t>(sx) * (sy > 0 ? sy - 1 : 0);
		const int xw = byte_width(static_cast<uint64_t>(sx) + 1), yw = byte_width(static_cast<uint64_t>(sy) + 1);
		for (int64_t z = 0; z < sz; z++) {
			const uint64_t differ = static_cast<uint64_t>(e.count_v[z]) + e.count_h[z];
			const uint64_t E = permissible ? interior - differ : differ;
			const uint64_t codes = E + 4ull * (static_cast<uint64_t>(e.count_special[z]) + e.count_corner[z]) + 16;
			est_code_bytes += (head.markov_model_order ? (3 * codes + 7) / 8 : (codes + 3) / 4) + 8;
			est_code_bytes += 4 + yw + 64ull * (yw + 2 * xw);
		}
	}
	if (getenv("CKL_SMALL_ESTIMATE")) est_code_bytes = 0;
	const uint64_t model_bytes_est = head.markov_model_order ? (1ull << (2 * head.markov_model_order)) : 0;
	struct HostOut { void* p = nullptr; ~HostOut() { if (p) host_out_free(p); } } early;
	uint64_t early_cap = 0;
	uint32_t labels_crc = 0;
	const int component_width = byte_width(static_cast<uint64_t>(sx) * sy);
	hipStream_t s2 = e.stream2;
	bool labels_stay = false;
	auto label_side = [&]() {
		if (labels_at_walk) {
			CKL_HIP(hipStreamWaitEvent(s2, e.evd0, 0));
			flat_enqueue(e, sx, sy, sz);
		}
		flat_collect<LABEL>(e, labels, sx, sy, sz, fr);
		HT_MARK("flat");
		const uint64_t N = fr.total;
		if (head.label_format == PINS_VARIABLE_WIDTH) {
			if (N > 0xFFFFFFFFull) throw Error(CKL_ERR_RUNTIME, "crackle_amd: too many components");
			e.d_cc_volume.ensure(voxels);
			launch_paint_components(s2, e.d_planes.p, e.row_words, e.plane_words, sx, sy, sz, e.d_word_base.p, e.d_rbase.p, e.d_run_cc.p, e.d_comp_off.p, 0u, e.d_cc_volume.p);
			pins_binary = pins_section_plain<LABEL>(e, labels, e.d_cc_volume.p, e.d_mapping.p, sx, sy, sz, N, fr.ncomp, head.pin_index_width(), stored_width, auto_bgcolor, manual_bgcolor);
			label_bytes = pins_binary.size();
		}
		else {
			label_bytes = flat_section(e, N, stored_width, component_width, static_cast<uint32_t>(sz), ov);
			HT_MARK("label_table");
			labels_stay = e.async_host_copy && e.keep_device_stream && !e.defer_codes && label_bytes > 0;
			early_cap = off_labels + label_bytes + model_bytes_est + est_code_bytes + 4ull * (sz + 1) + 64;
			early.p = host_out_alloc(early_cap);
			HT_MARK("l:buffer");
			uint8_t* eo = static_cast<uint8_t*>(early.p);
			if (labels_stay) {
				e.d_labels_crc.ensure(1 + kBlock);
				if (!e.ev_labels_crc) CKL_HIP(hipEventCreateWithFlags(&e.ev_labels_crc, hipEventDisableTiming));
				crc32c_device(e.d_labels_bin.p, label_bytes, e.d_labels_crc.p + 1, e.d_labels_crc.p, s2);
				CKL_HIP(hipEventRecord(e.ev_labels_crc, s2));
			}
			else {
				if (label_bytes) CKL_HIP(hipMemcpyAsync(eo + off_labels, e.d_labels_bin.p, label_bytes, hipMemcpyDeviceToHost, s2));
				CKL_HIP(hipStreamSynchronize(s2));
				labels_crc = crc32c(eo + off_labels, label_bytes);
			}
			HT_MARK("labels_d2h");
		}
	};

	CrackResult cr;
	std::vector<uint8_t> model, stored_model;
	if (getenv("CKL_NO_OVERLAP")) {
		crack_pass(e, sx, sy, sz, permissible, head.markov_model_order, false, model_in, nullptr, &model, &cr, std::function<void()>(), trail_cached);
		label_side();
	}
	else crack_pass(e, sx, sy, sz, permissible, head.markov_model_order, false, model_in, nullptr, &model, &cr, label_side, trail_cached);
	ht.mark("cracks");
	if (head.markov_model_order > 0) stored_model = markov_model_to_stored(model);

	head.num_label_bytes = label_bytes;
	const uint64_t off_model = off_labels + label_bytes;
	const uint64_t off_codes = off_model + stored_model.size();
	const uint64_t off_tail = off_codes + cr.total;
	const uint64_t total = off_tail + 4ull * (sz + 1);
	uint8_t* o;
	if (early.p && total <= early_cap) { o = static_cast<uint8_t*>(early.p); early.p = nullptr; }
	else {
		o = static_cast<uint8_t*>(host_out_alloc(total));
		if (early.p && label_bytes) memcpy(o + off_labels, static_cast<uint8_t*>(early.p) + off_labels, label_bytes);
	}
	try {
		e.last_codes_total = cr.total;
		if (head.label_format == PINS_VARIABLE_WIDTH) {
			if (label_bytes) memcpy(o + off_labels, pins_binary.data(), label_bytes);
			labels_crc = crc32c(o + off_labels, label_bytes);
		}
		std::vector<uint8_t> hb;
		head.write(hb);
		memcpy(o, hb.data(), hb.size());
		auto put4 = [&](uint64_t at, uint32_t v) { for (int b = 0; b < 4; b++) o[at + b] = static_cast<uint8_t>((v >> (8 * b)) & 0xFF); };
		for (int64_t z = 0; z < sz; z++) put4(off_index + 4ull * z, cr.code_len[z]);
		put4(off_index + 4ull * sz, crc32c(o + off_index, 4ull * sz));
		if (!stored_model.empty()) memcpy(o + off_model, stored_model.data(), stored_model.size());
		for (int64_t z = 0; z < sz; z++) put4(off_tail + 4 + 4ull * z, fr.crcs[z]);
		put4(off_tail, labels_crc);
		e.device_stream_bytes = 0;
		if (e.keep_device_stream) {
			e.d_stream_out.ensure(total + 16);
			uint8_t* ds = e.d_stream_out.p;
			const void* up = head.label_format == FLAT ? o : nullptr;
			upload_small(ds, o, off_labels, s, up);
			if (label_bytes) {
				if (head.label_format == FLAT) copy_bytes_device(e.d_labels_bin.p, ds + off_labels, label_bytes, s);
				else CKL_HIP(hipMemcpyAsync(ds + off_labels, o + off_labels, label_bytes, hipMemcpyHostToDevice, s));
			}
			if (!stored_model.empty()) upload_small(ds + off_model, o + off_model, stored_model.size(), s, up);
			if (cr.total) copy_bytes_device(e.d_codes_out.p, ds + off_codes, cr.total, s);
			upload_small(ds + off_tail, o + off_tail, 4ull * (sz + 1), s, up);
			if (labels_stay) {
				CKL_HIP(hipStreamWaitEvent(s, e.ev_labels_crc, 0));
				CKL_HIP(hipMemcpyAsync(ds + off_tail, e.d_labels_crc.p, 4, hipMemcpyDeviceToDevice, s));
			}
			e.device_stream_bytes = total;
		}
		if (cr.total && !e.defer_codes) {
			if (e.async_host_copy && e.keep_device_stream) {
				if (!e.stream_copy) CKL_HIP(hipStreamCreateWithFlags(&e.stream_copy, hipStreamNonBlocking));
				if (!e.ev_codes) CKL_HIP(hipEventCreateWithFlags(&e.ev_codes, hipEventDisableTiming));
				CKL_HIP(hipEventRecord(e.ev_codes, s));
				CKL_HIP(hipStreamWaitEvent(e.stream_copy, e.ev_codes, 0));
				CKL_HIP(hipMemcpyAsync(o + off_codes, e.d_codes_out.p, cr.total, hipMemcpyDeviceToHost, e.stream_copy));
				if (labels_stay) {
					CKL_HIP(hipMemcpyAsync(o + off_labels, e.d_labels_bin.p, label_bytes, hipMemcpyDeviceToHost, e.stream_copy));
					CKL_HIP(hipMemcpyAsync(o + off_tail, e.d_labels_crc.p, 4, hipMemcpyDeviceToHost, e.stream_copy));
				}
				e.host_copy_pending = true;
			}
			else CKL_HIP(hipMemcpyAsync(o + off_codes, e.d_codes_out.p, cr.total, hipMemcpyDeviceToHost, s));
		}
		ht.mark("assembly");
		CKL_HIP(hipEventRecord(e.ev1, s));
		CKL_HIP(hipStreamSynchronize(s));
		ht.mark("codes_d2h");
		CKL_HIP(hipGetLastError());
		CKL_HIP(hipEventElapsedTime(&e.pipeline_ms, e.ev0, e.ev1));
		CKL_HIP(hipEventElapsedTime(&e.trail_ms, e.evk0, e.evk1));
		CKL_HIP(hipEventElapsedTime(&e.dominant_ms, e.evd0, e.evd1));
	}
	catch (...) {
		if (e.host_copy_pending) { (void)hipStreamSynchronize(e.stream_copy); e.host_copy_pending = false; }
		host_out_free(o);
		throw;
	}
	*out = o;
	*out_len = total;
}

void reencode_markov(const uint8_t* buf, uint64_t n, int markov_order, int device, uint8_t** out, uint64_t* out_len) {
	if (n < Header::kBytesV0) throw Error(CKL_ERR_FORMAT, "crackle: Input too small to be a valid stream. Bytes: " + std::to_string(n));
	Header head = Header::parse(buf, n);
	if (markov_order < 0 || markov_order > 13) throw Error(CKL_ERR_ARG, "crackle_amd: markov_model_order must be in [0, 13] on device");
	auto copy_out = [&](const uint8_t* p, uint64_t len) {
		uint8_t* o = static_cast<uint8_t*>(host_out_alloc(len));
		memcpy(o, p, len);
		*out = o; *out_len = len;
// ... 65 lines not shown
	try {
		if (cr.total) CKL_HIP(hipMemcpyAsync(o + off_codes, enc.e->d_codes_out.p, cr.total, hipMemcpyDeviceToHost, enc.e->stream));
		std::vector<uint8_t> hb;
		head.write(hb);
		memcpy(o, hb.data(), hb.size());
		auto put4 = [&](uint64_t at, uint32_t v) { for (int b = 0; b < 4; b++) o[at + b] = static_cast<uint8_t>((v >> (8 * b)) & 0xFF); };
		for (uint64_t z = 0; z < sz; z++) put4(off_index + 4 * z, cr.code_len[z]);
		if (!v0) put4(off_index + 4 * sz, crc32c(o + off_index, 4 * sz));
		memcpy(o + off_labels, buf + off_labels, head.num_label_bytes);
		if (!stored_model.empty()) memcpy(o + off_model, stored_model.data(), stored_model.size());
		if (tail_bytes) memcpy(o + off_tail, buf + old_tail, tail_bytes);
		if (cr.total) CKL_HIP(hipStreamSynchronize(enc.e->stream));
		lap("assembly");
	}
	catch (...) { host_out_free(o); throw; }
	*out = o;
	*out_len = total;
}

void check_dims(int64_t sx, int64_t sy, int64_t sz, int dtype_bytes, int is_signed) {
	if (is_signed) throw Error(CKL_ERR_ARG, "Signed integer data types are not currently supported.");
	if (dtype_bytes != 1 && dtype_bytes != 2 && dtype_bytes != 4 && dtype_bytes != 8) throw Error(CKL_ERR_ARG, "crackle_amd: dtype width must be 1, 2, 4 or 8 bytes");
	if (sx < 0 || sy < 0 || sz < 0) throw Error(CKL_ERR_ARG, "crackle_amd: negative dimension");
	if (sx > 0x7FFFFFF0ll || sy > 0x7FFFFFF0ll || sz > 0x7FFFFFF0ll) throw Error(CKL_ERR_ARG, "crackle_amd: dimension too large");
	if (static_cast<uint64_t>(sx + 1) * static_cast<uint64_t>(sy + 1) >= (1ull << 30)) throw Error(CKL_ERR_ARG, "crackle_amd: slices of 2^30 or more crack vertices are not supported");
}

}

extern "C" {

int ckl_encoder_create(int64_t sx, int64_t sy, int64_t sz, int dtype_bytes, int device, ckl_encoder** out) {
	try {
		if (!out) throw Error(CKL_ERR_ARG, "crackle_amd: null argument");
		check_dims(sx, sy, sz, dtype_bytes, 0);
		select_device(device);
		std::unique_ptr<ckl_encoder> e(new ckl_encoder());
		e->device = device;
		e->max_sx = sx; e->max_sy = sy; e->max_sz = sz; e->dtype_bytes = dtype_bytes;
		CKL_HIP(hipStreamCreateWithFlags(&e->stream, hipStreamNonBlocking));
		{
			int lo = 0, hi = 0;
			CKL_HIP(hipDeviceGetStreamPriorityRange(&lo, &hi));
			CKL_HIP(hipStreamCreateWithPriority(&e->stream2, hipStreamNonBlocking, hi));
		}
		CKL_HIP(hipEventCreate(&e->ev0));
		CKL_HIP(hipEventCreate(&e->ev1));
		CKL_HIP(hipEventCreate(&e->evk0));
		CKL_HIP(hipEventCreate(&e->evk1));
		CKL_HIP(hipEventCreate(&e->evd0));
		CKL_HIP(hipEventCreate(&e->evd1));
		CKL_HIP(hipEventCreateWithFlags(&e->ev_in, hipEventDisableTiming));
		CKL_HIP(hipEventCreateWithFlags(&e->ev_prezero, hipEventDisableTiming));
		*out = e.release();
		return CKL_OK;
	}
	catch (const Error& e) { set_last_error(e.what()); return e.status; }
	catch (const std::exception& e) { set_last_error(e.what()); return CKL_ERR_RUNTIME; }
}

int ckl_encoder_run(
	ckl_encoder* e, const void* labels_device, int64_t sx, int64_t sy, int64_t sz,
	int allow_pins, int fortran_order, uint64_t markov_model_order,
	int optimize_pins, int auto_bgcolor, int64_t manual_bgcolor,
	const ckl_encode_overrides* overrides, uint8_t** out, uint64_t* out_len
) {
	try {
		if (!e || !out || !out_len) throw Error(CKL_ERR_ARG, "crackle_amd: null argument");
		check_dims(sx, sy, sz, e->dtype_bytes, 0);
		if (markov_model_order > 15) throw Error(CKL_ERR_ARG, "crackle_amd: markov_model_order must be in [0, 15]");
		select_device(e->device);
		if (e->host_copy_pending) {
			CKL_HIP(hipStreamSynchronize(e->stream_copy));
			e->host_copy_pending = false;
		}
		wait_for_default_stream(e->stream, e->ev_in);
		wait_for_default_stream(e->stream2, e->ev_in);
		const auto t_run0 = std::chrono::steady_clock::now();
#define CKL_ENC(T) encode_typed<T>(*e, reinterpret_cast<const T*>(labels_device), sx, sy, sz, allow_pins != 0, fortran_order != 0, \
	markov_model_order, optimize_pins != 0, auto_bgcolor != 0, manual_bgcolor, overrides, out, out_len)
		if (e->dtype_bytes == 1) CKL_ENC(uint8_t);
		else if (e->dtype_bytes == 2) CKL_ENC(uint16_t);
		else if (e->dtype_bytes == 4) CKL_ENC(uint32_t);
		else CKL_ENC(uint64_t);
#undef CKL_ENC
		if (getenv("CKL_PROFILE")) {
			fprintf(stderr, "[ckl encoder_run ms] encode=%.2f\n", std::chrono::duration<double, std::milli>(std::chrono::steady_clock::now() - t_run0).count());
		}
		return CKL_OK;
	}
	catch (const Error& err) { set_last_error(err.what()); return err.status; }
	catch (const std::exception& err) { set_last_error(err.what()); return CKL_ERR_RUNTIME; }
}

int ckl_reencode_markov(const uint8_t* buf, uint64_t n, int markov_model_order, int device, uint8_t** out, uint64_t* out_len) {
	try {
		if (!buf || !out || !out_len) throw Error(CKL_ERR_ARG, "crackle_amd: null argument");
		select_device(device);
		reencode_markov(buf, n, markov_model_order, device, out, out_len);
		return CKL_OK;
	}
	catch (const Error& err) { set_last_error(err.what()); return err.status; }
	catch (const std::exception& err) { set_last_error(err.what()); return CKL_ERR_RUNTIME; }
}

int ckl_encoder_defer_codes(ckl_encoder* e, int defer) {
// ... 319 lines not shown

int ckl_pins_rows_section(ckl_encoder* e, int64_t sx, int64_t sy, int64_t sz, uint64_t n_components, const uint32_t* ncomp_host,
	const uint64_t* comp_label, const uint64_t* first_any, const uint64_t* choice, const uint32_t* ze_plus1, const uint64_t* offsets, const uint32_t* ids,
	int stored_width, int auto_bgcolor, int64_t manual_bgcolor, uint8_t** out, uint64_t* out_len) {
	try {
		if (!e || !ncomp_host || !comp_label || !first_any || !choice || !ze_plus1 || !offsets || !ids || !out || !out_len) throw Error(CKL_ERR_ARG, "crackle_amd: null argument");
		if (sx <= 0 || sy <= 0 || sz <= 0) throw Error(CKL_ERR_ARG, "crackle_amd: empty volume");
		if (stored_width != 1 && stored_width != 2 && stored_width != 4 && stored_width != 8) throw Error(CKL_ERR_ARG, "crackle_amd: stored width must be 1, 2, 4 or 8 bytes");
		const uint64_t N = n_components;
		if (N == 0 || N >= kPinNone) throw Error(CKL_ERR_ARG, "crackle_amd: component count out of range");
		select_device(e->device);
		wait_for_default_stream(e->stream2, e->ev_in);
		std::vector<uint32_t> nc(ncomp_host, ncomp_host + sz);
		HostTimer ht;
		g_ht = &ht;
		const std::vector<uint8_t> bin = pins_section_from_device(*e, sx, sy, sz, N, nc, comp_label, first_any, choice, ze_plus1, offsets, ids, stored_width, auto_bgcolor != 0, manual_bgcolor);
		ht.mark("p:cover");
		uint8_t* p = static_cast<uint8_t*>(host_out_alloc(bin.size() ? bin.size() : 1));
		memcpy(p, bin.data(), bin.size());
		*out = p;
		*out_len = bin.size();
		return CKL_OK;
	}
	catch (const Error& err) { set_last_error(err.what()); return err.status; }
	catch (const std::exception& err) { set_last_error(err.what()); return CKL_ERR_RUNTIME; }
}

int ckl_encoder_last_timing(const ckl_encoder* e, float* pipeline_ms, float* dominant_kernel_ms) {
	if (!e) { set_last_error("crackle_amd: null encoder"); return CKL_ERR_ARG; }
	if (pipeline_ms) *pipeline_ms = e->pipeline_ms;
	if (dominant_kernel_ms) *dominant_kernel_ms = e->dominant_ms;
	return CKL_OK;
}

int ckl_encoder_walk_paths(ckl_encoder* e, uint32_t* fast_slices, uint32_t* compiled_slices) {
	try {
		if (!e) throw Error(CKL_ERR_ARG, "crackle_amd: null encoder");
		uint32_t fast = 0, plain = 0;
		const size_t ns = e->last_trail_slices;
		if (ns && e->t_counters.p) {
			select_device(e->device);
			std::vector<uint32_t> nev(ns);
			CKL_HIP(hipMemcpy(nev.data(), e->t_counters.p + 5 * ns, ns * sizeof(uint32_t), hipMemcpyDeviceToHost));
			for (uint32_t v : nev) { if (v & (kEvFormatAddr12 | kEvWalkWide)) fast++; else if (v) plain++; }
		}
		if (fast_slices) *fast_slices = fast;
		if (compiled_slices) *compiled_slices = plain;
		return CKL_OK;
	}
	catch (const Error& err) { set_last_error(err.what()); return err.status; }
	catch (const std::exception& err) { set_last_error(err.what()); return CKL_ERR_RUNTIME; }
}

__global__ void __launch_bounds__(kBlock) k_trail_step_kinds(const uint32_t* __restrict__ events, const uint64_t* __restrict__ ibase, const uint32_t* __restrict__ n_events, uint32_t* __restrict__ counts) {
	__shared__ uint32_t s_c[5];
	const uint32_t zi = blockIdx.x;
	if (threadIdx.x < 5) s_c[threadIdx.x] = 0u;
	__syncthreads();
	const uint32_t n = n_events[zi] & ~(dev::kEvFormatAddr12 | dev::kEvWalkWide);
	const uint32_t* ev = events + ibase[zi];
	uint32_t c[4] = { 0, 0, 0, 0 };
	for (uint32_t i = threadIdx.x; i < n; i += kBlock) c[ev[i] >> 30]++;
	for (int k = 0; k < 4; k++) if (c[k]) atomicAdd(&s_c[k], c[k]);
	if (threadIdx.x == 0) {
		uint32_t run = 0, longest = 0;
		for (uint32_t i = 0; i < n; i++) { if ((ev[i] >> 30) == 1u) run = 0; else { run++; longest = run > longest ? run : longest; } }
		s_c[4] = longest;
	}
	__syncthreads();
	if (threadIdx.x < 5) counts[zi * 5u + threadIdx.x] = s_c[threadIdx.x];
}

int ckl_encoder_walk_step_kinds(ckl_encoder* e, uint32_t* counts, uint32_t max_slices, uint32_t* n_slices) {
	try {
		if (!e || !counts || !n_slices) throw Error(CKL_ERR_ARG, "crackle_amd: null argument");
		const size_t ns = e->last_trail_slices;
		*n_slices = static_cast<uint32_t>(ns);
		if (!ns || !e->t_counters.p || !e->t_events.p) { *n_slices = 0; return CKL_OK; }
		if (ns > max_slices) throw Error(CKL_ERR_ARG, "crackle_amd: counts holds fewer slices than the last run had");
		select_device(e->device);
		DevBuf<uint32_t> d_counts;
		d_counts.ensure(ns * 5);
		hipLaunchKernelGGL(k_trail_step_kinds, dim3(static_cast<uint32_t>(ns)), dim3(kBlock), 0, e->stream, e->t_events.p, e->t_ibase.p, e->t_counters.p + 5 * ns, d_counts.p);
		CKL_HIP(hipMemcpyAsync(counts, d_counts.p, ns * 5 * sizeof(uint32_t), hipMemcpyDeviceToHost, e->stream));
		CKL_HIP(hipStreamSynchronize(e->stream));
		return CKL_OK;
	}
	catch (const Error& err) { set_last_error(err.what()); return err.status; }
	catch (const std::exception& err) { set_last_error(err.what()); return CKL_ERR_RUNTIME; }
}

void ckl_encoder_destroy(ckl_encoder* e) { delete e; }

int ckl_compress(
	const void* labels, int labels_mem, int dtype_bytes, int is_signed,
	int64_t sx, int64_t sy, int64_t sz,
	int allow_pins, int fortran_order, uint64_t markov_model_order,
	int optimize_pins, int auto_bgcolor, int64_t manual_bgcolor,
	int device, uint8_t** out, uint64_t* out_len
) {
	ckl_encoder* e = nullptr;
	try {
		check_dims(sx, sy, sz, dtype_bytes, is_signed);
		if (!out || !out_len) throw Error(CKL_ERR_ARG, "crackle_amd: null argument");
		if (static_cast<uint64_t>(sx) * sy * sz == 0) {
			Header head;
// ... 41 lines not shown
```

### crackle_amd/csrc/ckl_strips.hpp

```cpp
#pragma once

#include "ckl_runs.hpp"
#include <type_traits>

namespace ckl {
namespace dev {

constexpr uint32_t kStripWords = 1024;
constexpr uint32_t kStripCap = 2560;
constexpr uint32_t kStripRunsPerThread = kStripCap / kBlock;
constexpr uint32_t kStripBitmapWords = kStripCap / 32;
constexpr uint32_t kStripEdgeCap = kStripWords + kStripCap / 2;
constexpr uint32_t kStripOverflow = 0xFFFFFFFFu;
constexpr int kResolveBlock = 1024;
constexpr uint32_t kResolveCap = 0xFFFFu;
constexpr uint32_t kMaxStrips = 1024;

struct StripArrays {
	uint16_t* run_lid;
	uint32_t* sc_w;
	uint32_t* sc_cc;
	void* sc_label;
	uint32_t* strip_nruns;
	uint32_t* strip_nsc;
// ... 43 lines not shown
		const uint32_t unit = horiz ? 1u : 0x10000u;
		const uint32_t neg = ((kind ^ (kind >> 1)) & 1u) ^ 1u;
		const uint32_t q = neg ? p - unit : p + unit;
		const uint32_t c = p < q ? p : q;
		const uint32_t col = c & 0xFFFFu, row = c >> 16;
		const uint32_t qx = q & 0xFFFFu, qy = q >> 16;
		if (qx > sx || qy > sy) bad |= 1u;
		else {
			const bool ok = horiz ? (row - 1u < sy - 1u && col < sx) : (col - 1u < sx - 1u && row < sy);
			const uint32_t rel = row - y0;
			if (ok && rel < rows) atomicOr((horiz ? sH : sV) + rel * rw + (col >> 5), 1u << (col & 31u));
		}
		p = q;
	}
}

__device__ __forceinline__ void raster_half_record(
	const uint4 rec, uint32_t h, uint32_t y0, uint32_t y1, uint32_t rlo_h, uint32_t sx, uint32_t sy, uint32_t rw, uint32_t* lds_v, uint32_t* lds_h, uint32_t& bad
) {
	constexpr uint32_t kLo = 0x55555555u;
	uint32_t p = rec.x;
	uint32_t kinds = rec.y, flags = rec.z;
	if (h) {
		const uint32_t ms = flags & kLo & 0xFFFFu, pv = kinds;
		const uint32_t mR = ms & ~(pv >> 1) & pv, mL = ms & (pv >> 1) & pv, mD = ms & (pv >> 1) & ~pv, mU = ms & ~(pv >> 1) & ~pv;
		p += __popc(mR) - __popc(mL) + ((__popc(mD) - __popc(mU)) << 16);
		if (flags & 0xAAAAu) p += rec.w;
		kinds >>= 16; flags >>= 16;
	}
#pragma unroll
	for (uint32_t k = 0; k < 8; k++) {
		const uint32_t j = (flags >> (2u * k + 1u)) & 1u;
		p += rec.w & (0u - j);
		const uint32_t e = (flags >> (2u * k)) & 1u;
		const uint32_t kind = (kinds >> (2u * k)) & 3u;
		const uint32_t horiz = kind & 1u;
		const uint32_t neg = ((kind ^ (kind >> 1)) & 1u) ^ 1u;
		const uint32_t unit = horiz ? 1u : 0x10000u;
		const uint32_t d = ((unit ^ (0u - neg)) + neg) & (0u - e);
		const uint32_t q = p + d;
		const uint32_t c = p < q ? p : q;
		const uint32_t col = c & 0xFFFFu, row = c >> 16;
		bad |= ((q & 0xFFFFu) > sx || (q >> 16) > sy) ? 1u : 0u;
		const uint32_t rlo = horiz ? rlo_h : y0, clo = horiz ? 0u : 1u;
		const bool ok = e != 0u && (row - rlo) <= (y1 - 1u - rlo) && row >= rlo && (col - clo) <= (sx - 1u - clo) && col >= clo;
		uint32_t* base = horiz ? lds_h : lds_v;
		const uint32_t at = ok ? (row - y0) * rw + (col >> 5) : 0u;
		atomicOr(base + at, ok ? (1u << (col & 31u)) : 0u);
		p = q;
	}
}

constexpr uint32_t kStripCclWords = (kStripCap + kStripEdgeCap + kStripWords / 2 + 2 * kStripBitmapWords + kWaves + 2 + 7) & ~7u;
template <bool DIAG, bool RECORDS>
__device__ __forceinline__ void strip_ccl_body(
	const RunGeom& g, const StripArrays& sa, const RecordLists& rl, const uint32_t* __restrict__ G, uint32_t n_pixels, unsigned long long* __restrict__ diag,
	uint32_t zi, uint32_t k, uint32_t* lds
) {
	uint32_t* s_parent = lds;
	uint32_t* s_mem = s_parent + kStripCap;
	uint16_t* s_wb = reinterpret_cast<uint16_t*>(s_mem + kStripEdgeCap);
	uint32_t* s_b = s_mem;
	uint16_t* s_pool = reinterpret_cast<uint16_t*>(s_mem + kStripWords);
	uint32_t* s_bm = s_mem + kStripEdgeCap + kStripWords / 2;
	uint32_t* s_bmbase = s_bm + kStripBitmapWords;
	uint32_t* s_scan = s_bmbase + kStripBitmapWords;
	uint32_t* s_misc = s_scan + kWaves;
	static_assert((kStripCap * 4) % 16 == 0 && (kStripEdgeCap * 4) % 16 == 0, "tables stay 16-byte aligned");
	unsigned long long d_t = DIAG ? __builtin_amdgcn_s_memtime() : 0ull;
	auto stamp = [&](int slot) {
		if (DIAG && threadIdx.x == 0) {
			const unsigned long long now = __builtin_amdgcn_s_memtime();
			atomicAdd(diag + slot, now - d_t);
			d_t = now;
		}
	};
	const uint32_t rw = g.row_words;
	const uint32_t t = threadIdx.x;
	const uint32_t si = zi * sa.nstrips + k;
	const uint32_t y0 = k * sa.strip_rows;
	const uint32_t y1 = min(y0 + sa.strip_rows, g.sy);
	const uint32_t nw = (y1 - y0) * rw;
	const uint64_t slot = static_cast<uint64_t>(si) * sa.cap;
	uint32_t b[4], up[4], upl[4], cnt = 0;
	if (RECORDS) {
		static_assert(kStripCap >= kStripWords, "plane H piece is built in the union-find table");
		uint32_t* sV = s_mem;
		uint32_t* sH = s_parent;
		const uint32_t n_rec = min(rl.count[si], rl.cap);
		const uint4* list = rl.rec + static_cast<uint64_t>(si) * rl.cap;
		uint4 first = list[(t >> 1) < rl.cap ? (t >> 1) : 0u];
#pragma unroll
		for (uint32_t j = 0; j < 4; j++) { sV[t * 4u + j] = 0u; sH[t * 4u + j] = 0u; }
		__syncthreads();
		uint32_t bad = 0;
		{
			const uint32_t half = t & 1u, rlo_h = y0 ? y0 : 1u;
			if ((t >> 1) < n_rec) raster_half_record(first, half, y0, y1, rlo_h, g.sx, g.sy, rw, sV, sH, bad);
			for (uint32_t r = (t >> 1) + kBlock / 2u; r < n_rec; r += kBlock / 2u) raster_half_record(list[r], half, y0, y1, rlo_h, g.sx, g.sy, rw, sV, sH, bad);
		}
		if (bad) atomicOr(sa.slice_err + zi, ERR_RANGE);
		__syncthreads();
		stamp(5);
		const uint4 v4 = *reinterpret_cast<const uint4*>(sV + t * 4u);
		const uint4 h4 = *reinterpret_cast<const uint4*>(sH + t * 4u);
		b[0] = v4.x; b[1] = v4.y; b[2] = v4.z; b[3] = v4.w;
		up[0] = h4.x; up[1] = h4.y; up[2] = h4.z; up[3] = h4.w;
		upl[0] = sH[t ? t * 4u - 1u : 0u];
		if (t * 4u < nw) {
			uint32_t* pv = const_cast<uint32_t*>(g.planeV) + zi * g.plane_words + static_cast<uint64_t>(y0) * rw;
// ... 14 lines not shown
#pragma unroll
		for (uint32_t j = 0; j < 4; j++) {
			const uint32_t wl = t * 4u + j;
			const uint32_t at = wl < nw ? wl : 0u;
			b[j] = pv[at];
			up[j] = ph[at];
		}
		upl[0] = ph[(t * 4u < nw && t) ? t * 4u - 1u : 0u];
	}
	uint32_t w[4];
	{
		const uint32_t yy = (t * 4u) / rw;
		uint32_t ww = t * 4u - yy * rw;
#pragma unroll
		for (uint32_t j = 0; j < 4; j++) { w[j] = ww; if (++ww == rw) ww = 0; }
	}
	upl[0] = (w[0] && t * 4u >= rw && t * 4u < nw) ? g.ups_of(upl[0], w[0] - 1u) : 0u;
#pragma unroll
	for (uint32_t j = 0; j < 4; j++) {
		const uint32_t wl = t * 4u + j;
		b[j] = wl < nw ? g.breaks_of(b[j], w[j]) : 0u;
		up[j] = (wl >= rw && wl < nw) ? g.ups_of(up[j], w[j]) : 0u;
		cnt += __popc(b[j]);
	}
#pragma unroll
	for (uint32_t j = 1; j < 4; j++) upl[j] = w[j] ? up[j - 1] : 0u;
	uint32_t v[1] = { cnt }, tot[1];
	block_excl_add<1>(v, tot, s_scan);
	const uint32_t nloc = tot[0];
	if (nloc > sa.cap) {
		if (t == 0) { sa.strip_nruns[si] = kStripOverflow; sa.strip_nsc[si] = 0u; atomicOr(sa.overflow, 1u); }
		return;
	}
	stamp(0);
	{
		uint32_t local = v[0];
		uint32_t px = ((t * 4u) / rw) * g.sx;
#pragma unroll
		for (uint32_t j = 0; j < 4; j++) {
			const uint32_t wl = t * 4u + j;
			if (j && w[j] == 0) px += g.sx;
			if (wl < nw) {
				s_b[wl] = b[j];
				s_wb[wl] = static_cast<uint16_t>(local);
				for (uint32_t m = b[j]; m; m &= m - 1u) s_pool[local++] = static_cast<uint16_t>(px + w[j] * 32u + (__ffs(m) - 1u));
			}
		}
	}
	for (uint32_t j = t; j < nloc; j += kBlock) s_parent[j] = j;
	if (t < kStripBitmapWords) s_bm[t] = 0u;
	__syncthreads();
	stamp(1);
	uint32_t gv[kStripRunsPerThread];
	{
		const uint32_t p0 = y0 * g.sx;
#pragma unroll
		for (uint32_t i = 0; i < kStripRunsPerThread; i++) {
			const uint32_t j = t + i * kBlock;
			gv[i] = G[n_pixels - (p0 + s_pool[j < nloc ? j : 0u])];
		}
	}
	{
		uint32_t yy = (t * 4u) / rw;
#pragma unroll
		for (uint32_t j = 0; j < 4; j++) {
			const uint32_t wl = t * 4u + j;
			if (j && w[j] == 0) yy++;
			if (wl >= nw) break;
			const uint16_t wbv = s_wb[wl];
			if (w[j] == 0) sa.row_run[static_cast<uint64_t>(zi) * g.sy + y0 + yy] = wbv;
			if (wl < rw) sa.seam_first[static_cast<uint64_t>(si) * rw + wl] = wbv;
			if (wl + rw >= nw) sa.seam_last[static_cast<uint64_t>(si) * rw + (wl + rw - nw)] = wbv;
		}
	}
	{
		uint32_t c[4], b_up[4], base_up[4], base_here[4], n_e = 0;
#pragma unroll
		for (uint32_t j = 0; j < 4; j++) {
			const uint32_t wl = t * 4u + j;
			const uint32_t above = up[j] ? wl - rw : 0u;
			b_up[j] = s_b[above]; base_up[j] = s_wb[above]; base_here[j] = s_wb[wl < nw ? wl : 0u];
			c[j] = up[j] & (~((up[j] << 1) | (upl[j] >> 31)) | b[j] | b_up[j]);
			n_e += __popc(c[j]);
		}
		uint32_t ve[1] = { n_e }, te[1];
		block_excl_add<1>(ve, te, s_scan);
		const uint32_t n_edges = te[0];
		if (n_edges <= kStripEdgeCap) {
			uint32_t at = ve[0];
#pragma unroll
			for (uint32_t j = 0; j < 4; j++) {
				for (uint32_t cc = c[j]; cc; cc &= cc - 1u) {
					const uint32_t m = mask_le(__ffs(cc) - 1u);
					s_mem[at++] = (base_here[j] + __popc(b[j] & m) - 1u) | ((base_up[j] + __popc(b_up[j] & m) - 1u) << 16);
				}
			}
			__syncthreads();
			for (uint32_t e = t; e < n_edges; e += kBlock) { const uint32_t pr = s_mem[e]; sm_unite(s_parent, pr & 0xFFFFu, pr >> 16); }
		}
		else {
#pragma unroll
			for (uint32_t j = 0; j < 4; j++) {
				for (uint32_t cc = c[j]; cc; cc &= cc - 1u) {
					const uint32_t m = mask_le(__ffs(cc) - 1u);
					sm_unite(s_parent, base_here[j] + __popc(b[j] & m) - 1u, base_up[j] + __popc(b_up[j] & m) - 1u);
				}
			}
		}
	}
	__syncthreads();
	stamp(2);
	uint32_t root[kStripRunsPerThread];
#pragma unroll
	for (uint32_t i = 0; i < kStripRunsPerThread; i++) {
		const uint32_t j = t + i * kBlock;
		root[i] = j < nloc ? sm_find(s_parent, j) : 0u;
		if (j < nloc && root[i] == j) atomicOr(s_bm + (j >> 5), 1u << (j & 31u));
	}
	__syncthreads();
	if (t < kWave) {
		static_assert(kStripBitmapWords <= 2 * kWave, "two bitmap words per lane");
		const uint32_t c0 = t < kStripBitmapWords ? __popc(s_bm[t]) : 0u;
		const uint32_t c1 = t + kWave < kStripBitmapWords ? __popc(s_bm[t + kWave]) : 0u;
		const uint32_t i0 = wave_incl_add(c0);
		const uint32_t tot0 = __shfl(i0, kWave - 1, kWave);
		const uint32_t i1 = wave_incl_add(c1);
		if (t < kStripBitmapWords) s_bmbase[t] = i0 - c0;
		if (t + kWave < kStripBitmapWords) s_bmbase[t + kWave] = tot0 + i1 - c1;
		if (t == kWave - 1) s_misc[1] = tot0 + i1;
	}
	__syncthreads();
	const uint32_t nsc = s_misc[1];
	uint16_t* lid_out = sa.run_lid + slot;
	const bool narrow = nsc <= 256u;
#pragma unroll
	for (uint32_t i = 0; i < kStripRunsPerThread; i++) {
		const uint32_t j = t + i * kBlock;
		if (j >= nloc) break;
		const uint32_t r = root[i];
		const uint32_t lid = s_bmbase[r >> 5] + __popc(s_bm[r >> 5] & ((1u << (r & 31u)) - 1u));
		s_pool[j] = static_cast<uint16_t>(lid);
		if (narrow) reinterpret_cast<uint8_t*>(lid_out)[j] = static_cast<uint8_t>(lid);
		else lid_out[j] = static_cast<uint16_t>(lid);
	}
	for (uint32_t j = t; j < nsc; j += kBlock) s_parent[j] = 0u;
	__syncthreads();
	stamp(3);
#pragma unroll
	for (uint32_t i = 0; i < kStripRunsPerThread; i++) {
		const uint32_t j = t + i * kBlock;
		if (j >= nloc) break;
		atomicXor(s_parent + s_pool[j], gv[i]);
		if (j) atomicXor(s_parent + s_pool[j - 1], gv[i]);
	}
	if (t == 0 && nloc) atomicXor(s_parent + s_pool[nloc - 1], G[n_pixels - y1 * g.sx]);
	__syncthreads();
	uint32_t* w_out = sa.sc_w + slot;
	for (uint32_t j = t; j < nsc; j += kBlock) w_out[j] = s_parent[j];
	if (t == 0) { sa.strip_nruns[si] = nloc; sa.strip_nsc[si] = nsc; }
	stamp(4);
}

template <bool DIAG, bool RECORDS>
static __global__ void __launch_bounds__(kBlock, 7) k_strip_ccl(RunGeom g, StripArrays sa, RecordLists rl, const uint32_t* __restrict__ G, uint32_t n_pixels, unsigned long long* __restrict__ diag) {
	__shared__ __attribute__((aligned(16))) uint32_t s_lds[kStripCclWords];
	strip_ccl_body<DIAG, RECORDS>(g, sa, rl, G, n_pixels, diag, blockIdx.y + sa.zbase, blockIdx.x, s_lds);
}

struct ResolveArgs {
	uint32_t idbits, crc_fix, check_crc;
	const uint32_t* crc_expect;
	const uint32_t* ncomp_expect;
	const uint64_t* comp_off;
	const uint64_t* label_map;
	const uint8_t* keys;
	const uint8_t* uniq;
	uint32_t key_width, stored_width, is_signed;
	uint64_t num_unique;
	uint32_t has_label;
	uint64_t label;
	uint32_t cap;
	uint32_t* host_flags;
	uint32_t host_flags_n;
};

template <int W>
__device__ __forceinline__ uint64_t ld_le(const uint8_t* p) {
	if constexpr (W == 1) return *p;
	else if constexpr (W == 2) { uint16_t v; __builtin_memcpy(&v, p, 2); return v; }
	else if constexpr (W == 4) { uint32_t v; __builtin_memcpy(&v, p, 4); return v; }
	else { uint64_t v; __builtin_memcpy(&v, p, 8); return v; }
}
template <typename F>
__device__ __forceinline__ void with_width(uint32_t w, F&& f) {
	switch (w) {
		case 1: f(std::integral_constant<int, 1>{}); break;
		case 2: f(std::integral_constant<int, 2>{}); break;
		case 4: f(std::integral_constant<int, 4>{}); break;
		default: f(std::integral_constant<int, 8>{}); break;
	}
}

template <typename OUT, bool LABELS, bool DIAG>
__device__ __forceinline__ bool slice_resolve_body(
	const RunGeom& g, const StripArrays& sa, const ResolveArgs& ra, uint32_t* __restrict__ ncomp_out, unsigned long long* __restrict__ diag,
	uint32_t zi, uint32_t* s_tab, uint32_t* s_scbase, uint32_t* s_scan, uint32_t* s_flag_p
) {
	uint32_t& s_flag = *s_flag_p;
	static_assert(kResolveCap <= 0xFFFFu, "index and rank share a table entry");
	constexpr int NW = kResolveBlock / kWave;
	unsigned long long d_t = DIAG ? __builtin_amdgcn_s_memtime() : 0ull;
	auto stamp = [&](int slot) {
		if (DIAG && threadIdx.x == 0) {
			const unsigned long long now = __builtin_amdgcn_s_memtime();
			atomicAdd(diag + slot, now - d_t);
			d_t = now;
		}
	};
	const uint32_t t = threadIdx.x;
	const uint32_t ns = sa.nstrips;
	const uint32_t rw = g.row_words;
	const uint32_t si0 = zi * ns;
	const uint32_t items = (ns - 1u) * rw;
	constexpr uint32_t kSeamPer = 2;
	uint32_t q_up[kSeamPer], q_prev[kSeamPer], q_bh[kSeamPer], q_bu[kSeamPer], q_wh[kSeamPer], q_wu[kSeamPer];
	auto seam_load = [&](uint32_t it0) {
#pragma unroll
		for (uint32_t u = 0; u < kSeamPer; u++) {
			const uint32_t it_raw = it0 + u * kResolveBlock + t;
			const uint32_t it = it_raw < items ? it_raw : 0u;
			const uint32_t seam = it / rw, w = it - seam * rw;
			const uint32_t k = seam + 1u, y = k * sa.strip_rows;
			const uint64_t at = zi * g.plane_words + static_cast<uint64_t>(y) * rw + w;
			const uint32_t h = g.planeH[at], hp = g.planeH[w ? at - 1u : at];
			const uint32_t vh = g.planeV[at], vu = g.planeV[at - rw];
			q_wh[u] = sa.seam_first[static_cast<uint64_t>(si0 + k) * rw + w];
			q_wu[u] = sa.seam_last[static_cast<uint64_t>(si0 + k - 1u) * rw + w];
			q_up[u] = it_raw < items ? g.ups_of(h, w) : 0u;
			q_prev[u] = w ? (g.ups_of(hp, w - 1u) >> 31) : 0u;
			q_bh[u] = g.breaks_of(vh, w); q_bu[u] = g.breaks_of(vu, w);
		}
	};
	if (items) seam_load(0);
	uint32_t my_nsc = 0;
	if (t == 0) s_flag = 0;
	__syncthreads();
	if (t < ns) {
		const uint32_t nr = sa.strip_nruns[si0 + t];
		if (nr == kStripOverflow) s_flag = 1;
		my_nsc = sa.strip_nsc[si0 + t];
	}
	uint32_t v[1] = { my_nsc }, tot[1];
	block_excl_add<1, NW>(v, tot, s_scan);
	if (t < ns) s_scbase[t] = v[0];
	if (t == 0) s_scbase[ns] = tot[0];
	const uint32_t total = tot[0];
	__syncthreads();
	if (s_flag || total > ra.cap) {
		if (t == 0) {
			atomicOr(sa.overflow, s_flag ? 1u : 2u);
			if (ra.host_flags) { ra.host_flags[ra.host_flags_n + (s_flag ? 0u : 1u)] = 1u; ra.host_flags[zi] = sa.slice_err[zi]; }
		}
		return false;
	}
	for (uint32_t i = t; i < total; i += kResolveBlock) s_tab[i] = i;
	__syncthreads();
	stamp(0);
	for (uint32_t it0 = 0; it0 < items; it0 += kSeamPer * kResolveBlock) {
		if (it0) seam_load(it0);
#pragma unroll
		for (uint32_t u = 0; u < kSeamPer; u++) {
			if (!q_up[u]) continue;
			const uint32_t it = it0 + u * kResolveBlock + t;
			const uint32_t k = it / rw + 1u;
			const uint16_t* lid_h = sa.run_lid + static_cast<uint64_t>(si0 + k) * sa.cap;
			const uint16_t* lid_u = sa.run_lid + static_cast<uint64_t>(si0 + k - 1u) * sa.cap;
			const uint32_t nsc_h = s_scbase[k + 1u] - s_scbase[k], nsc_u = s_scbase[k] - s_scbase[k - 1u];
			for (uint32_t c = q_up[u] & (~((q_up[u] << 1) | q_prev[u]) | q_bh[u] | q_bu[u]); c; c &= c - 1u) {
				const uint32_t m = mask_le(__ffs(c) - 1u);
				const uint32_t jh = q_wh[u] + __popc(q_bh[u] & m) - 1u, ju = q_wu[u] + __popc(q_bu[u] & m) - 1u;
				if (jh >= sa.cap || ju >= sa.cap) continue;
				const uint32_t lh = strip_lid(lid_h, nsc_h, jh), lu = strip_lid(lid_u, nsc_u, ju);
				if (lh < nsc_h && lu < nsc_u) sm_unite(s_tab, s_scbase[k] + lh, s_scbase[k - 1u] + lu);
			}
		}
	}
	__syncthreads();
	stamp(1);
	const uint32_t per = (total + kResolveBlock - 1) / kResolveBlock;
	const uint32_t i0 = min(total, t * per), i1 = min(total, i0 + per);
	for (uint32_t i = i0; i < i1; i++) sm_store(s_tab, i, sm_find(s_tab, i));
	__syncthreads();
	uint32_t nroot = 0;
	for (uint32_t i = i0; i < i1; i++) nroot += s_tab[i] == i ? 1u : 0u;
	constexpr uint32_t kPer = 4;
	uint32_t strip0 = 0;
	if (i0 < i1) {
		uint32_t lo = 0, hi = ns;
		while (lo + 1 < hi) { const uint32_t mid = (lo + hi) >> 1; if (s_scbase[mid] <= i0) lo = mid; else hi = mid; }
		strip0 = lo;
	}
	uint32_t v2[1] = { nroot }, tot2[1];
	block_excl_add<1, NW>(v2, tot2, s_scan);
	{
		uint32_t rk = v2[0];
		for (uint32_t i = i0; i < i1; i++) if (s_tab[i] == i) s_tab[i] = i | (rk++ << 16);
	}
	__syncthreads();
	stamp(2);
	const uint32_t ncomp = tot2[0];
	const uint32_t nexp = ra.ncomp_expect[zi];
	const uint64_t coff = ra.comp_off[zi];
	uint32_t part = 0;
	uint32_t sidx = strip0;
	for (uint32_t r0 = i0; r0 < i1; r0 += kPer) {
		uint32_t cc[kPer], wgt[kPer];
		uint64_t gi[kPer], key[kPer];
#pragma unroll
		for (uint32_t q = 0; q < kPer; q++) {
			const uint32_t i = r0 + q;
			const bool on = i < i1;
			const uint32_t ii = on ? i : i0;
			if (on) while (sidx + 1 < ns && s_scbase[sidx + 1] <= ii) sidx++;
			const uint32_t sq = on ? sidx : strip0;
			gi[q] = static_cast<uint64_t>(si0 + sq) * sa.cap + (ii - s_scbase[sq]);
			cc[q] = s_tab[s_tab[ii] & 0xFFFFu] >> 16;
			wgt[q] = sa.sc_w[gi[q]];
			key[q] = 0;
		}
		uint64_t lab[kPer];
		if (LABELS) {
			with_width(ra.key_width, [&](auto W) {
#pragma unroll
				for (uint32_t q = 0; q < kPer; q++) key[q] = ld_le<decltype(W)::value>(ra.keys + (coff + (cc[q] < nexp ? cc[q] : 0u)) * static_cast<uint64_t>(decltype(W)::value));
			});
#pragma unroll
			for (uint32_t q = 0; q < kPer; q++) lab[q] = 0;
			if (ra.num_unique) {
				with_width(ra.stored_width, [&](auto W) {
#pragma unroll
					for (uint32_t q = 0; q < kPer; q++) lab[q] = ld_le<decltype(W)::value>(ra.uniq + (key[q] < ra.num_unique ? key[q] : 0ull) * static_cast<uint64_t>(decltype(W)::value));
				});
			}
		}
#pragma unroll
		for (uint32_t q = 0; q < kPer; q++) {
			if (r0 + q >= i1) continue;
			if (LABELS) {
				uint64_t val = 0;
				if (cc[q] < nexp && key[q] < ra.num_unique) {
					val = lab[q];
					if (ra.is_signed && ra.stored_width < 8u && (val >> (8u * ra.stored_width - 1u))) val |= ~0ull << (8u * ra.stored_width);
				}
				if (ra.has_label) val = (val == ra.label);
				static_cast<OUT*>(sa.sc_label)[gi[q]] = static_cast<OUT>(val);
			}
			else sa.sc_cc[gi[q]] = cc[q];
			uint32_t wg = wgt[q];
			for (int j = static_cast<int>(ra.idbits) - 1; j >= 0; j--) {
				part ^= ((cc[q] >> j) & 1u) ? wg : 0u;
				wg = (wg >> 1) ^ ((wg & 1u) ? kCrcPoly : 0u);
			}
		}
	}
	part = wave_xor(part);
	if ((t & (kWave - 1)) == 0) s_scan[t >> 6] = part;
	__syncthreads();
	if (t == 0) {
		uint32_t x = 0;
		for (int wv = 0; wv < NW; wv++) x ^= s_scan[wv];
		uint32_t e = 0;
		if (ncomp != nexp) e |= ERR_NCOMP;
		else if (ra.check_crc && gf_mul(x, ra.crc_fix) != ra.crc_expect[zi]) e |= ERR_CRC;
		if (e) atomicOr(sa.slice_err + zi, e);
		ncomp_out[zi] = ncomp;
		if (ra.host_flags) ra.host_flags[zi] = sa.slice_err[zi] | e;
	}
	stamp(3);
	return true;
}

template <typename OUT, bool LABELS, bool DIAG>
static __global__ void __launch_bounds__(kResolveBlock, 8) k_slice_resolve(RunGeom g, StripArrays sa, ResolveArgs ra, uint32_t* __restrict__ ncomp_out, unsigned long long* __restrict__ diag) {
	extern __shared__ __attribute__((aligned(16))) uint32_t s_tab[];
	__shared__ uint32_t s_scbase[kMaxStrips + 1];
	__shared__ uint32_t s_scan[kResolveBlock / kWave];
	__shared__ uint32_t s_flag;
	slice_resolve_body<OUT, LABELS, DIAG>(g, sa, ra, ncomp_out, diag, blockIdx.x + sa.zbase, s_tab, s_scbase, s_scan, &s_flag);
}

template <typename OUT>
static __global__ void __launch_bounds__(kBlock) k_strip_labels(StripArrays sa, ResolveArgs ra) {
	const uint32_t zi = blockIdx.y + sa.zbase;
	const uint32_t si = zi * sa.nstrips + blockIdx.x;
	if (sa.strip_nruns[si] == kStripOverflow) return;
	const uint32_t n = min(sa.strip_nsc[si], sa.cap);
	const uint32_t nexp = ra.ncomp_expect[zi];
	const uint64_t coff = ra.comp_off[zi];
	const uint64_t slot = static_cast<uint64_t>(si) * sa.cap;
	for (uint32_t j = threadIdx.x; j < n; j += kBlock) {
		const uint32_t c = sa.sc_cc[slot + j];
		uint64_t val = c < nexp ? ra.label_map[coff + c] : 0ull;
		if (ra.has_label) val = (val == ra.label);
		static_cast<OUT*>(sa.sc_label)[slot + j] = static_cast<OUT>(val);
	}
}

__device__ __forceinline__ uint32_t strip_component_of_pixel(const RunGeom& g, const StripArrays& sa, uint32_t zi, uint32_t x, uint32_t y) {
	const uint32_t k = y / sa.strip_rows;
	const uint32_t si = zi * sa.nstrips + k;
	const uint32_t nr = sa.strip_nruns[si];
	if (nr == kStripOverflow) return 0xFFFFFFFFu;
	uint32_t run = sa.row_run[static_cast<uint64_t>(zi) * g.sy + y];
	const uint32_t wx = x >> 5;
	for (uint32_t w = 0; w < wx; w++) run += __popc(g.breaks(zi, y, w));
	run += __popc(g.breaks(zi, y, wx) & mask_le(x & 31u)) - 1u;
	if (run >= nr || run >= sa.cap) return 0xFFFFFFFFu;
	const uint64_t slot = static_cast<uint64_t>(si) * sa.cap;
	const uint32_t lid = strip_lid(sa.run_lid + slot, sa.strip_nsc[si], run);
	return lid < sa.cap ? sa.sc_cc[slot + lid] : 0xFFFFFFFFu;
}

}
// ... 2 lines not shown
```

### crackle_amd/csrc/ckl_trail.hpp

```cpp
#pragma once

#include "ckl_device.hpp"

namespace ckl {
namespace dev {

constexpr uint32_t kTrailTileShift = 5, kTrailTileDim = 32;
__device__ __forceinline__ uint32_t mt_index(uint32_t mx, uint32_t my, uint32_t mtx2) {
	return (((my >> 1) * mtx2 + (mx >> 1)) << 2) | ((my & 1u) << 1) | (mx & 1u);
}
struct MicroTile {
	uint4 lo, hi;
	uint32_t mx, my;
	__device__ __forceinline__ bool holds(uint32_t x, uint32_t y) const { return (x >> 3) == mx && (y >> 3) == my; }
	__device__ __forceinline__ uint32_t nib(uint32_t x, uint32_t y) const {
		const uint32_t r = y & 7u;
		const uint32_t a0 = (r & 1u) ? lo.y : lo.x, a1 = (r & 1u) ? lo.w : lo.z, a2 = (r & 1u) ? hi.y : hi.x, a3 = (r & 1u) ? hi.w : hi.z;
		const uint32_t b0 = (r & 2u) ? a1 : a0, b1 = (r & 2u) ? a3 : a2;
		return (((r & 4u) ? b1 : b0) >> ((x & 7u) * 4u)) & 15u;
	}
};

enum : uint32_t { TRAIL_ERR_CAPACITY = 1u };
constexpr uint32_t kDartNone = 0xFFFFFFFFu;
// ... 166 lines not shown
) {
	__shared__ uint32_t s_red[2 * kWaves];
	__shared__ uint4 s_out[kWaves][kWave * 8];
	const int lane = threadIdx.x & 63, wave = threadIdx.x >> 6;
	const uint32_t zi = blockIdx.y;
	const bool permissible = perm_mode == 2u ? static_cast<long long>(*total_pairs) < static_cast<long long>(half_voxels) : perm_mode != 0u;
	const uint32_t item = blockIdx.x * kBlock + threadIdx.x;
	const uint32_t mtx = (sx + 1u + 7u) >> 3;
	uint32_t ns = 0, nc = 0;
	uint32_t my_base = 0, my_tiles = 0;
	if (item < tiles_x * tiles_y) {
		const uint32_t ty = item / tiles_x, tx = item - ty * tiles_x;
		TileRowBits b[8];
		trail_rows8(planeV + zi * plane_words, planeH + zi * plane_words, row_words, sx, sy, tx, ty << 3, permissible ? 0xFFFFFFFFu : 0u, b);
		my_base = mt_index(tx * 4u, ty, mtx2) * 32u;
		my_tiles = min(4u, mtx - min(mtx, tx * 4u));
#pragma unroll
		for (uint32_t q = 0; q < 4; q++) {
			uint32_t w[8];
#pragma unroll
			for (uint32_t k = 0; k < 8; k++)
				w[k] = spread8((b[k].R >> (8 * q)) & 255u) | (spread8((b[k].L >> (8 * q)) & 255u) << 1)
					| (spread8((b[k].D >> (8 * q)) & 255u) << 2) | (spread8((b[k].U >> (8 * q)) & 255u) << 3);
			s_out[wave][lane * 8 + ((2u * q) ^ (lane & 7))] = make_uint4(w[0], w[1], w[2], w[3]);
			s_out[wave][lane * 8 + ((2u * q + 1u) ^ (lane & 7))] = make_uint4(w[4], w[5], w[6], w[7]);
		}
#pragma unroll
		for (uint32_t k = 0; k < 8; k++) { ns += __popc(trail_special_mask(b[k])); nc += __popc(trail_corner_mask(b[k])); }
	}
	{
		uint8_t* dst = reinterpret_cast<uint8_t*>(adjm_words + zi * adjm_stride_words);
#pragma unroll
		for (uint32_t i = 0; i < 8; i++) {
			const uint32_t owner = i * 8u + (lane >> 3), p = lane & 7u;
			const uint32_t base = __shfl(my_base, owner, kWave), have = __shfl(my_tiles, owner, kWave);
			const uint4 v = s_out[wave][owner * 8u + (p ^ (owner & 7u))];
			const uint32_t q = p >> 1;
			if (q < have) *reinterpret_cast<uint4*>(dst + base + (q >> 1) * 128u + (q & 1u) * 32u + (p & 1u) * 16u) = v;
		}
	}
	ns = wave_sum(ns); nc = wave_sum(nc);
	if (lane == 0) { s_red[wave] = ns; s_red[kWaves + wave] = nc; }
	__syncthreads();
	if (threadIdx.x == 0) {
		uint32_t ts = 0, tc = 0;
		for (int w = 0; w < kWaves; w++) { ts += s_red[w]; tc += s_red[kWaves + w]; }
		blk_special[static_cast<uint64_t>(zi) * gridDim.x + blockIdx.x] = ts;
		blk_corner[static_cast<uint64_t>(zi) * gridDim.x + blockIdx.x] = tc;
	}
}

static __global__ void __launch_bounds__(kBlock) k_trail_count_scan(
	uint32_t* __restrict__ blk_special, uint32_t* __restrict__ blk_corner, uint32_t nblk,
	uint32_t* __restrict__ tot_special, uint32_t* __restrict__ tot_corner
) {
	__shared__ uint32_t s_scan[2 * kWaves];
	const uint32_t zi = blockIdx.x;
	uint32_t* bs = blk_special + static_cast<uint64_t>(zi) * nblk;
	uint32_t* bc = blk_corner + static_cast<uint64_t>(zi) * nblk;
	uint32_t cs = 0, cc = 0;
	for (uint32_t b0 = 0; b0 < nblk; b0 += kBlock) {
		const uint32_t b = b0 + threadIdx.x;
		uint32_t v[2] = { b < nblk ? bs[b] : 0u, b < nblk ? bc[b] : 0u }, tot[2];
		block_excl_add<2>(v, tot, s_scan);
		if (b < nblk) { bs[b] = cs + v[0]; bc[b] = cc + v[1]; }
		cs += tot[0]; cc += tot[1];
	}
	if (threadIdx.x == 0) { tot_special[zi] = cs; tot_corner[zi] = cc; }
}

static __global__ void __launch_bounds__(kBlock) k_trail_nodes(TrailArgs a) {
	__shared__ uint32_t s_scan[2 * kWaves];
	const uint32_t zi = blockIdx.y + a.z0;
	const uint32_t item = blockIdx.x * kBlock + threadIdx.x;
	TileRowBits b[8];
	uint32_t x0 = 0, y0 = 0;
	if (item < a.tiles_x * a.tiles_y) {
		const uint32_t ty = item / a.tiles_x, tx = item - ty * a.tiles_x;
		x0 = tx << kTrailTileShift; y0 = ty << 3;
		trail_rows8(a.planeV + zi * a.plane_words, a.planeH + zi * a.plane_words, a.row_words, a.sx, a.sy, tx, y0, a.inv, b);
	}
	else {
#pragma unroll
		for (int k = 0; k < 8; k++) b[k] = TileRowBits{ 0, 0, 0, 0 };
	}
	uint32_t v[2] = { 0, 0 }, tot[2];
#pragma unroll
	for (uint32_t k = 0; k < 8; k++) { v[0] += __popc(trail_special_mask(b[k])); v[1] += __popc(trail_corner_mask(b[k])); }
	block_excl_add<2>(v, tot, s_scan);
	uint32_t j = a.blk_special[static_cast<uint64_t>(zi) * a.graph_blocks + blockIdx.x] + v[0];
	uint32_t c = a.blk_corner[static_cast<uint64_t>(zi) * a.graph_blocks + blockIdx.x] + v[1];
	const uint64_t nb = a.nbase[zi];
	const uint32_t ncap = a.ncap[zi], cocap = a.cocap[zi];
	uint32_t err = 0;
#pragma unroll
	for (uint32_t k = 0; k < 8; k++) {
		const uint32_t y = y0 + k;
		const TileRowBits& r = b[k];
		for (uint32_t m = trail_special_mask(r); m; m &= m - 1u) {
			const uint32_t i = __ffs(m) - 1;
			const uint32_t vtx = y * a.sxe + x0 + i;
			if (j < ncap) {
				a.node_vertex[nb + j] = vtx;
				a.node_adj[nb + j] = static_cast<uint8_t>(((r.R >> i) & 1u) | (((r.L >> i) & 1u) << 1) | (((r.D >> i) & 1u) << 2) | (((r.U >> i) & 1u) << 3));
				a.vert2node[static_cast<uint64_t>(zi) * a.nverts + vtx] = j;
			}
			else err = TRAIL_ERR_CAPACITY;
			j++;
		}
		for (uint32_t m = trail_corner_mask(r); m; m &= m - 1u) {
			const uint32_t i = __ffs(m) - 1;
			if (c < cocap) a.corner_vertex[a.cobase[zi] + c] = y * a.sxe + x0 + i;
			else err = TRAIL_ERR_CAPACITY;
			c++;
		}
	}
	if (err) atomicOr(a.slice_err + zi, err);
	if (blockIdx.x == gridDim.x - 1 && threadIdx.x == kBlock - 1) {
		a.n_nodes[zi] = min(j, ncap);
		a.n_corners[zi] = min(c, cocap);
	}
// ... 1347 lines not shown
```

### crackle_amd/distributed.py

```python
import ctypes as C
from typing import Optional, Sequence, Tuple

import numpy as np
import torch
import torch.distributed as dist

from . import _lib

FLAT = 0
IMPERMISSIBLE, PERMISSIBLE = 0, 1


def _byte_width(x: int) -> int:
  return 1 if x <= 0xFF else 2 if x <= 0xFFFF else 4 if x <= 0xFFFFFFFF else 8


def stats_to_model(hist: np.ndarray) -> np.ndarray:
  hist = np.asarray(hist, dtype=np.uint64).reshape(-1, 4)
  order = np.lexsort((-np.arange(4)[None, :].repeat(hist.shape[0], 0), -hist.astype(np.int64)), axis=1)
  model = np.empty_like(order, dtype=np.uint8)
  rows = np.arange(hist.shape[0])[:, None]
  model[rows, order] = np.arange(4, dtype=np.uint8)[None, :]
  return np.ascontiguousarray(model)

# ... 387 lines not shown
                    first_kept.data_ptr(), best.data_ptr(), choice.data_ptr(), ze_plus1.data_ptr())

  def pins_rows_ids(self, cc_rows, sx, rows, sz, y0, n, choice, ze_plus1, offsets, ids):
    self._rows_call(self._L.ckl_pins_rows_ids, cc_rows.data_ptr(), sx, rows, sz, y0, n, choice.data_ptr(), ze_plus1.data_ptr(), offsets.data_ptr(), ids.data_ptr())

  def pins_rows_section(self, sx, sy, sz, n, ncomp_all: np.ndarray, comp_label, first_any, choice, ze_plus1, offsets, ids, stored_width: int) -> np.ndarray:
    nc = np.ascontiguousarray(ncomp_all, dtype=np.uint32)
    out_p, out_n = C.c_void_p(), C.c_uint64()
    self._rows_call(self._L.ckl_pins_rows_section, sx, sy, sz, n, nc.ctypes.data, comp_label.data_ptr(), first_any.data_ptr(), choice.data_ptr(),
                    ze_plus1.data_ptr(), offsets.data_ptr(), ids.data_ptr(), int(stored_width), 1, 0, C.byref(out_p), C.byref(out_n))
    try:
      return np.frombuffer(C.string_at(out_p.value, out_n.value), dtype=np.uint8)
    finally:
      self._L.ckl_free(out_p)

  def keep_device_stream(self, shape, itemsize: int, keep: bool = True):
    self._L.ckl_encoder_keep_device_stream(self._encoder(shape, itemsize), int(bool(keep)))

  def async_host_copy(self, shape, itemsize: int, on: bool = True):
    self._L.ckl_encoder_async_host_copy(self._encoder(shape, itemsize), int(bool(on)))

  def host_wait(self):
    if self._enc and self._L.ckl_encoder_host_wait(self._enc) != _lib.CKL_OK:
      raise RuntimeError(_lib.last_error())

  def device_stream(self) -> DeviceStream:
    p, n = C.c_void_p(), C.c_uint64()
    rc = self._L.ckl_encoder_device_stream(self._enc, C.byref(p), C.byref(n))
    if rc != _lib.CKL_OK:
      raise RuntimeError(_lib.last_error())
    return DeviceStream(p.value, n.value, owner=self, generation=self._stream_generation)

  def defer_codes(self, shape, itemsize: int, defer: bool):
    self._L.ckl_encoder_defer_codes(self._encoder(shape, itemsize), int(bool(defer)))

  def codes_to_host(self, dst_ptr: int, capacity: int) -> int:
    n = C.c_uint64()
    rc = self._L.ckl_encoder_codes_to_host(self._enc, dst_ptr, capacity, C.byref(n))
    if rc != _lib.CKL_OK:
      raise RuntimeError(_lib.last_error())
    return int(n.value)

  def encoder_timing(self) -> Tuple[float, float]:
    p, k = C.c_float(), C.c_float()
    if self._enc:
      self._L.ckl_encoder_last_timing(self._enc, C.byref(p), C.byref(k))
    return p.value, k.value

  def walk_paths(self) -> Tuple[int, int]:
    f, c = C.c_uint32(), C.c_uint32()
    if self._enc and self._L.ckl_encoder_walk_paths(self._enc, C.byref(f), C.byref(c)) != _lib.CKL_OK:
      raise RuntimeError(_lib.last_error())
    return f.value, c.value

  def walk_step_kinds(self, max_slices: int = 1 << 16):
    buf = (C.c_uint32 * (5 * max_slices))()
    n = C.c_uint32()
    if not self._enc:
      return np.zeros((0, 5), np.uint32)
    if self._L.ckl_encoder_walk_step_kinds(self._enc, buf, max_slices, C.byref(n)) != _lib.CKL_OK:
      raise RuntimeError(_lib.last_error())
    return np.frombuffer(buf, dtype=np.uint32, count=5 * n.value).reshape(n.value, 5).copy()

  def open_decoder(self, binary: bytes, z_start: int, z_end: int):
    return HipDecodeSession(binary, z_start, z_end, self.device_index)

  def __del__(self):
    try:
      if self._enc:
        self._L.ckl_encoder_destroy(self._enc)
    except Exception:
      pass


class ShardedCodec:

  def __init__(self, backend, rank: int = 0, world: int = 1, device="cpu", compute_device=None, force_sharded: bool = False):
    self.force_sharded = bool(force_sharded)
    self.backend = backend
    self.rank, self.world = int(rank), int(world)
    self.device = torch.device(device)
    self.compute_device = torch.device(compute_device) if compute_device is not None else self.device
    self._shared = None
    self._shared_vol = None

  def _gather_rows(self, mine: np.ndarray) -> np.ndarray:
    t = torch.from_numpy(np.ascontiguousarray(mine, dtype=np.int64)).to(self.device)
    import os
    if dist.get_backend() == "nccl" and not os.environ.get("CKL_SHARDED_LIST_GATHER"):
      out = torch.empty(self.world * t.numel(), dtype=torch.int64, device=self.device)
      dist.all_gather_into_tensor(out, t)
      return out.cpu().numpy().reshape(self.world, t.numel())
    parts = [torch.empty_like(t) for _ in range(self.world)]
    dist.all_gather(parts, t)
    return torch.stack(parts).cpu().numpy()

  def compress(self, vol, slab_shape, markov_model_order: int = 0, allow_pins: bool = False, fortran_order: bool = True, defer: bool = False):
    be = self.backend
    if self.world == 1 and not self.force_sharded:
      whole = be.encode(vol, slab_shape, allow_pins, fortran_order, markov_model_order, None)
      def _done():
        if hasattr(be, "host_wait"):
          be.host_wait()
        return whole
      return _done if defer else _done()
    import os, time
# ... 458 lines not shown
```

### include/crackle_amd.h

```cpp
#ifndef CRACKLE_AMD_H
#define CRACKLE_AMD_H

#include <stdint.h>

#ifdef __cplusplus
extern "C" {
#endif

typedef enum ckl_status {
	CKL_OK = 0,
	CKL_ERR_FORMAT = 1,
	CKL_ERR_RUNTIME = 2,
	CKL_ERR_ARG = 3,
	CKL_ERR_NO_DEVICE = 4,
	CKL_ERR_CRC = 5
} ckl_status;

enum { CKL_MEM_HOST = 0, CKL_MEM_DEVICE = 1 };

const char* ckl_last_error(void);

int ckl_abi_version(void);

int ckl_device_count(void);
// ... 87 lines not shown
int ckl_encoder_run(
	ckl_encoder* e, const void* labels_device,
	int64_t sx, int64_t sy, int64_t sz,
	int allow_pins, int fortran_order, uint64_t markov_model_order,
	int optimize_pins, int auto_bgcolor, int64_t manual_bgcolor,
	const ckl_encode_overrides* overrides,
	uint8_t** out, uint64_t* out_len);

int ckl_encoder_defer_codes(ckl_encoder* e, int defer);
int ckl_encoder_keep_device_stream(ckl_encoder* e, int keep);
int ckl_encoder_async_host_copy(ckl_encoder* e, int on);
int ckl_encoder_host_wait(ckl_encoder* e);
int ckl_encoder_device_stream(const ckl_encoder* e, const uint8_t** stream_device, uint64_t* n_bytes);
int ckl_encoder_codes_to_host(ckl_encoder* e, uint8_t* dst_host, uint64_t capacity, uint64_t* n_bytes);
int ckl_host_register(void* p, uint64_t bytes);
int ckl_host_unregister(void* p);

int ckl_encoder_stats(
	ckl_encoder* e, const void* labels_device, int64_t sx, int64_t sy, int64_t sz,
	uint64_t* max_label, uint64_t* pixel_pairs, uint64_t* first_voxel, uint64_t* last_voxel);

int ckl_encoder_markov_stats(
	ckl_encoder* e, const void* labels_device, int64_t sx, int64_t sy, int64_t sz,
	int crack_format, uint64_t markov_model_order, uint32_t* hist);

int ckl_encoder_components(
	ckl_encoder* e, const void* labels_device, int64_t sx, int64_t sy, int64_t sz,
	uint32_t id_base, uint32_t* cc_host, uint32_t* ncomp_host);

int ckl_encoder_components_device(
	ckl_encoder* e, const void* labels_device, int64_t sx, int64_t sy, int64_t sz,
	uint32_t id_base, uint32_t* cc_device, uint32_t* ncomp_host);

int ckl_encoder_pin_labels(
	ckl_encoder* e, const void* labels_device, const uint32_t* cc_device,
	int64_t sx, int64_t sy, int64_t sz, const uint32_t* ncomp_host,
	int stored_width, int auto_bgcolor, int64_t manual_bgcolor,
	uint8_t** out, uint64_t* out_len);

int ckl_pins_rows_first(ckl_encoder* e, const void* labels_rows, const uint32_t* cc_rows, int64_t sx, int64_t rows, int64_t sz, int64_t y0,
	uint64_t n_components, uint64_t* first_any, uint64_t* first_kept, uint64_t* comp_label);
int ckl_pins_rows_best(ckl_encoder* e, const void* labels_rows, const uint32_t* cc_rows, int64_t sx, int64_t rows, int64_t sz, int64_t y0,
	uint64_t n_components, const uint64_t* first_kept, uint64_t* best);
int ckl_pins_rows_extent(ckl_encoder* e, const void* labels_rows, const uint32_t* cc_rows, int64_t sx, int64_t rows, int64_t sz, int64_t y0,
	uint64_t n_components, const uint64_t* first_kept, const uint64_t* best, uint64_t* choice, uint32_t* ze_plus1);
int ckl_pins_rows_ids(ckl_encoder* e, const uint32_t* cc_rows, int64_t sx, int64_t rows, int64_t sz, int64_t y0,
	uint64_t n_components, const uint64_t* choice, const uint32_t* ze_plus1, const uint64_t* offsets, uint32_t* ids);
int ckl_pins_rows_section(ckl_encoder* e, int64_t sx, int64_t sy, int64_t sz, uint64_t n_components, const uint32_t* ncomp_host,
	const uint64_t* comp_label, const uint64_t* first_any, const uint64_t* choice, const uint32_t* ze_plus1, const uint64_t* offsets, const uint32_t* ids,
	int stored_width, int auto_bgcolor, int64_t manual_bgcolor, uint8_t** out, uint64_t* out_len);

int ckl_encoder_last_timing(const ckl_encoder* e, float* pipeline_ms, float* dominant_kernel_ms);
int ckl_encoder_walk_paths(ckl_encoder* e, uint32_t* fast_slices, uint32_t* compiled_slices);
int ckl_encoder_walk_step_kinds(ckl_encoder* e, uint32_t* counts, uint32_t max_slices, uint32_t* n_slices);
void ckl_encoder_destroy(ckl_encoder* e);


int ckl_zstack(
	const uint8_t* const* bufs, const uint64_t* lens, uint64_t count,
	uint8_t** out, uint64_t* out_len);

int ckl_pin_labels_host(
	const void* labels, int dtype_bytes, const uint32_t* cc,
	int64_t sx, int64_t sy, int64_t sz, const uint32_t* ncomp,
	int stored_width, int auto_bgcolor, int64_t manual_bgcolor,
	uint8_t** out, uint64_t* out_len);

int ckl_point_cloud(
	const uint8_t* buf, uint64_t n, int64_t z_start, int64_t z_end,
	const uint64_t* labels, uint64_t n_labels, int has_labels, int skip_background, int device,
	uint64_t** labels_out, uint64_t** offsets_out, uint16_t** points_out, uint64_t* n_out);

int ckl_reencode_markov(const uint8_t* buf, uint64_t n, int markov_model_order, int device, uint8_t** out, uint64_t* out_len);

int ckl_zsplit(const uint8_t* buf, uint64_t n, int64_t z_start, int64_t z_end, uint8_t** out, uint64_t* out_len);

uint32_t ckl_crc32c(const uint8_t* data, uint64_t n);
uint32_t ckl_crc32c_combine(uint32_t crc_a, uint32_t crc_b, uint64_t len_b);

#ifdef __cplusplus
}
#endif
#endif
```

Before: 150.0 billion.

## Reuse decoder strip CCL for encoder component labeling on a side stream

Ports the decoder's strip-based connected-component labeling and slice-resolve kernels into the encoder. Encoder variants record each component's first pixel, CRC accumulator and id bits, and are launched on a second stream once the trail counts are ready, so they overlap with the rest of the pipeline. Plane and node counts are also written straight into pinned host memory, which removes separate device-to-host copies, and dynamic-LDS attribute calls are cached per kernel and device. This adds eligibility checks, overflow fallback to the run-based path, and extra cross-stream synchronization.

```diff
diff --git a/crackle_amd/_lib.py b/crackle_amd/_lib.py
--- a/crackle_amd/_lib.py
+++ b/crackle_amd/_lib.py
@@ -83,6 +83,7 @@
   "ckl_encoder_walk_step_kinds": (C.c_int, [C.c_void_p, C.POINTER(C.c_uint32), C.c_uint32, C.POINTER(C.c_uint32)]),
   "ckl_encoder_last_timing": (C.c_int, [C.c_void_p, C.POINTER(C.c_float), C.POINTER(C.c_float)]),
   "ckl_encoder_walk_paths": (C.c_int, [C.c_void_p, C.POINTER(C.c_uint32), C.POINTER(C.c_uint32)]),
+  "ckl_encoder_label_path": (C.c_int, [C.c_void_p, C.POINTER(C.c_uint32), C.POINTER(C.c_uint32)]),
   "ckl_encoder_destroy": (None, [C.c_void_p]),
   "ckl_pin_labels_host": (C.c_int, [
     C.c_void_p, C.c_int, C.c_void_p, C.c_int64, C.c_int64, C.c_int64, C.c_void_p,
@@ -122,6 +123,8 @@
       )
     L = C.CDLL(LIB_PATH)
     for name, (res, args) in EXPORTS.items():
+      if os.environ.get("CKL_LIB_AB") and not hasattr(L, name):
+        continue
       f = getattr(L, name)
       f.restype = res
       f.argtypes = args
diff --git a/crackle_amd/csrc/ckl_decode.hip b/crackle_amd/csrc/ckl_decode.hip
--- a/crackle_amd/csrc/ckl_decode.hip
+++ b/crackle_amd/csrc/ckl_decode.hip
@@ -2445,21 +2445,22 @@
 	d.plane_words = static_cast<uint64_t>(d.row_words) * h.sy;
 	d.d_planes.ensure(2 * d.plane_words * d.nslices);
 	{
-		d.strip_rows = std::max<uint32_t>(1u, kStripWords / d.row_words);
+		uint32_t max_rows = 0xFFFFFFFFu;
 		if (!permissible && d.nslices) {
 			const double runs_per_row = 1.0 + 0.5 * est_codes / (static_cast<double>(d.nslices) * h.sy);
-			const uint32_t fit = static_cast<uint32_t>(0.7 * kStripCap / runs_per_row);
-			d.strip_rows = std::max<uint32_t>(1u, std::min(d.strip_rows, fit));
-		}
-		if (const char* env = getenv("CKL_CCL_ROWS")) d.strip_rows = std::max<uint32_t>(1u, std::min<uint32_t>(kStripWords / d.row_words, static_cast<uint32_t>(std::max(1, atoi(env)))));
-		d.nstrips = (h.sy + d.strip_rows - 1) / d.strip_rows;
+			max_rows = static_cast<uint32_t>(0.7 * kStripCap / runs_per_row);
+		}
+		if (const char* env = getenv("CKL_CCL_ROWS")) max_rows = static_cast<uint32_t>(std::max(1, atoi(env)));
+		const StripShape shape = strip_shape(h.sx, h.sy, d.row_words, max_rows);
+		d.strip_rows = shape.strip_rows;
+		d.nstrips = shape.nstrips;
 		d.strip_ok = h.fortran_order && (h.sx % 4 == 0) && d.row_words <= kStripWords && d.nstrips <= kMaxStrips &&
 			d.sxy < 0xFFFF0000ull && !getenv("CKL_DECODE_GENERAL");
 		if (d.strip_ok) {
 			const bool few = d.nslices <= static_cast<uint32_t>(std::max(1, d.n_cus));
 			const size_t lds_share = few ? static_cast<size_t>(d.max_lds) - 8192u : static_cast<size_t>(d.max_lds) / 2u - 6144u;
-			d.resolve_cap = static_cast<uint32_t>(std::min<size_t>(kResolveCap, (lds_share - (kMaxStrips + 64u) * 4u) / 4u));
-			d.resolve_cap_max = static_cast<uint32_t>(std::min<size_t>(kResolveCap, (static_cast<size_t>(d.max_lds) - 8192u - (kMaxStrips + 64u) * 4u) / 4u));
+			d.resolve_cap = resolve_cap_for(lds_share);
+			d.resolve_cap_max = resolve_cap_for(static_cast<size_t>(d.max_lds) - 8192u);
 			if (few && !getenv("CKL_LDS_CONTROLS")) {
 				uint32_t nctl = 16384;
 				while (nctl > 64 && rec_lds_bytes(nctl) > lds_share) nctl -= 64;
@@ -2471,7 +2472,7 @@
 				}
 			}
 			const size_t nst = static_cast<size_t>(d.nstrips) * d.nslices;
-			d.strip_cap = static_cast<uint32_t>(std::min<uint64_t>(kStripCap, static_cast<uint64_t>(d.strip_rows) * h.sx));
+			d.strip_cap = shape.cap;
 			d.d_row_run.ensure(static_cast<size_t>(h.sy) * d.nslices);
 			d.d_strip_nruns.ensure(nst); d.d_strip_nsc.ensure(nst);
 			d.d_seam_first.ensure(nst * d.row_words); d.d_seam_last.ensure(nst * d.row_words);
diff --git a/crackle_amd/csrc/ckl_encode.hip b/crackle_amd/csrc/ckl_encode.hip
--- a/crackle_amd/csrc/ckl_encode.hip
+++ b/crackle_amd/csrc/ckl_encode.hip
@@ -1,5 +1,6 @@
 #include "ckl_common.hpp"
 #include "ckl_runs.hpp"
+#include "ckl_strips.hpp"
 #include "ckl_trail.hpp"
 #include "ckl_pins_dev.hpp"
 
@@ -9,6 +10,7 @@
 #include <functional>
 #include <memory>
 #include <mutex>
+#include <tuple>
 
 namespace ckl {
 
@@ -285,7 +287,8 @@
 __global__ void __launch_bounds__(kBlock) k_planes_reduce(
 	const uint32_t* __restrict__ partial, const unsigned long long* __restrict__ partial_max, uint32_t nblk,
 	unsigned long long* __restrict__ out ,
-	unsigned long long* __restrict__ total_pairs
+	unsigned long long* __restrict__ total_pairs ,
+	unsigned long long* __restrict__ host_out
 ) {
 	__shared__ uint32_t s_red[kWaves];
 	__shared__ unsigned long long s_max[kWaves];
@@ -305,6 +308,7 @@
 	if (threadIdx.x == 0) {
 		for (int w = 0; w < kWaves; w++) tm = s_max[w] > tm ? s_max[w] : tm;
 		out[4ull * zi + 0] = tv; out[4ull * zi + 1] = th; out[4ull * zi + 2] = tp; out[4ull * zi + 3] = tm;
+		if (host_out) { host_out[4ull * zi + 0] = tv; host_out[4ull * zi + 1] = th; host_out[4ull * zi + 2] = tp; host_out[4ull * zi + 3] = tm; }
 		atomicAdd(total_pairs, static_cast<unsigned long long>(tp));
 	}
 }
@@ -616,13 +620,27 @@
 
 template <typename LABEL>
 __global__ void __launch_bounds__(kBlock) k_mapping_comps(
-	const LABEL* __restrict__ labels, RunArrays r, uint64_t sxy,
+	const LABEL* __restrict__ labels, const uint32_t* __restrict__ ncomp, const uint32_t* __restrict__ first_pix,
+	const uint64_t* __restrict__ rbase, uint64_t stride, uint64_t sxy,
 	const uint64_t* __restrict__ comp_off, uint64_t* __restrict__ mapping
 ) {
 	const uint32_t zi = blockIdx.y;
 	const uint32_t c = blockIdx.x * kBlock + threadIdx.x;
-	if (c >= r.ncomp[zi]) return;
-	mapping[comp_off[zi] + c] = static_cast<uint64_t>(labels[zi * sxy + r.comp_pix[r.rbase[zi] + c]]);
+	if (c >= ncomp[zi]) return;
+	const uint64_t base = rbase ? rbase[zi] : zi * stride;
+	mapping[comp_off[zi] + c] = static_cast<uint64_t>(labels[zi * sxy + first_pix[base + c]]);
+}
+
+static __global__ void __launch_bounds__(kBlock, 7) k_strip_ccl_first(RunGeom g, StripArrays sa, const uint32_t* __restrict__ G, uint32_t n_pixels, uint32_t* __restrict__ sc_first) {
+	__shared__ __attribute__((aligned(16))) uint32_t s_lds[kStripCclWords];
+	strip_ccl_body<false, false, true>(g, sa, RecordLists{}, G, n_pixels, nullptr, blockIdx.y + sa.zbase, blockIdx.x, s_lds, sc_first);
+}
+static __global__ void __launch_bounds__(kResolveBlock, 8) k_slice_resolve_enc(RunGeom g, StripArrays sa, ResolveArgs ra, EncResolveOut en, uint32_t* __restrict__ ncomp_out) {
+	extern __shared__ __attribute__((aligned(16))) uint32_t s_tab[];
+	__shared__ uint32_t s_scbase[kMaxStrips + 1];
+	__shared__ uint32_t s_scan[kResolveBlock / kWave];
+	__shared__ uint32_t s_flag;
+	slice_resolve_body<uint32_t, false, false, true>(g, sa, ra, ncomp_out, nullptr, blockIdx.x + sa.zbase, s_tab, s_scbase, s_scan, &s_flag, &en);
 }
 
 
@@ -1058,6 +1076,28 @@
 	DevBuf<uint16_t> d_run_local;
 	DevBuf<uint32_t> d_G, d_crc_acc;
 	DevBuf<uint32_t> d_flat_report;
+	DevBuf<uint16_t> s_run_lid, s_row_run, s_seam_first, s_seam_last;
+	DevBuf<uint32_t> s_sc_w, s_sc_first, s_strip_nruns, s_strip_nsc, s_first_pix;
+	uint32_t strip_resolve_cap = 0;
+	StripShape strip_shape_used = { 0, 0, 0 };
+	bool strips_enqueued = false;
+	uint32_t strip_overflow = 0;
+	uint32_t label_strips = 0, label_runs = 0;
+	hipEvent_t ev_planes = nullptr;
+	hipEvent_t ev_counts = nullptr;
+	bool strips_pending = false;
+	void* h_counts = nullptr;
+	size_t h_counts_slices = 0;
+	unsigned long long* h_plane_out(uint32_t ns) {
+		if (h_counts && h_counts_slices < ns) { host_out_free(h_counts); h_counts = nullptr; }
+		if (!h_counts) {
+			h_counts = host_out_alloc(std::max<size_t>(64u << 10, static_cast<size_t>(ns) * 40u));
+			h_counts_slices = ns;
+			if (!host_out_is_pinned(h_counts)) { host_out_free(h_counts); h_counts = nullptr; h_counts_slices = 0; }
+		}
+		return static_cast<unsigned long long*>(h_counts);
+	}
+	int max_lds = 0, n_cus = 0;
 	uint64_t g_table_pixels = 0;
 	DevBuf<uint64_t> d_mapping, d_sorted, d_uniq, d_label_hash, d_label_list;
 	DevBuf<uint8_t> d_keys;
@@ -1106,17 +1146,35 @@
 		if (evd1) (void)hipEventDestroy(evd1);
 		if (ev_in) (void)hipEventDestroy(ev_in);
 		if (ev_prezero) (void)hipEventDestroy(ev_prezero);
+		if (ev_planes) (void)hipEventDestroy(ev_planes);
+		if (ev_counts) (void)hipEventDestroy(ev_counts);
 		if (stream) (void)hipStreamDestroy(stream);
 		if (stream2) (void)hipStreamDestroy(stream2);
 		if (stream_copy) { (void)hipStreamSynchronize(stream_copy); (void)hipStreamDestroy(stream_copy); }
 		if (stream_tab) { (void)hipStreamSynchronize(stream_tab); (void)hipStreamDestroy(stream_tab); }
 		if (ev_codes) (void)hipEventDestroy(ev_codes);
 		if (tables_staging) host_out_free(tables_staging);
+		if (h_counts) host_out_free(h_counts);
 		if (ev_labels_crc) (void)hipEventDestroy(ev_labels_crc);
 	}
 };
 
 namespace {
+
+void allow_dynamic_lds(const void* fn, int device, size_t bytes) {
+	static std::mutex mu;
+	static std::vector<std::tuple<const void*, int, size_t>>& done = *new std::vector<std::tuple<const void*, int, size_t>>();
+	std::lock_guard<std::mutex> lock(mu);
+	for (auto& d : done) {
+		if (std::get<0>(d) != fn || std::get<1>(d) != device) continue;
+		if (std::get<2>(d) >= bytes) return;
+		CKL_HIP(hipFuncSetAttribute(fn, hipFuncAttributeMaxDynamicSharedMemorySize, static_cast<int>(bytes)));
+		std::get<2>(d) = bytes;
+		return;
+	}
+	CKL_HIP(hipFuncSetAttribute(fn, hipFuncAttributeMaxDynamicSharedMemorySize, static_cast<int>(bytes)));
+	done.emplace_back(fn, device, bytes);
+}
 
 template <typename T>
 void upload(DevBuf<T>& d, const std::vector<T>& h, hipStream_t s) {
@@ -1256,7 +1314,8 @@
 			labels, static_cast<uint32_t>(sx), static_cast<uint32_t>(sy), strips, bands,
 			e.d_planes.p, e.d_planes.p + e.plane_words * ns, e.row_words, e.plane_words,
 			e.d_plane_partial.p, e.d_plane_partial_max.p, e.d_plane_out.p + 4ull * ns);
-		hipLaunchKernelGGL(k_planes_reduce, dim3(ns), dim3(kBlock), 0, s, e.d_plane_partial.p, e.d_plane_partial_max.p, nblk, e.d_plane_out.p, e.d_plane_out.p + 4ull * ns);
+		hipLaunchKernelGGL(k_planes_reduce, dim3(ns), dim3(kBlock), 0, s, e.d_plane_partial.p, e.d_plane_partial_max.p, nblk, e.d_plane_out.p, e.d_plane_out.p + 4ull * ns,
+			defer ? e.h_plane_out(ns) : static_cast<unsigned long long*>(nullptr));
 		e.planes_deferred = defer;
 		if (!e.planes_deferred) planes_collect(e, ns, st);
 		return;
@@ -1275,6 +1334,7 @@
 	e.count_h.assign(c.begin() + ns, c.end());
 }
 
+void strips_enqueue(ckl_encoder& e, int64_t sx, int64_t sy, int64_t sz, uint32_t max_rows);
 void graph_pass(ckl_encoder& e, int64_t sx, int64_t sy, int64_t sz, int perm_mode, VolumeStats* st = nullptr) {
 	hipStream_t s = e.stream;
 	const uint32_t ns = static_cast<uint32_t>(sz);
@@ -1296,14 +1356,30 @@
 		perm_mode == 2 ? e.d_plane_out.p + 4ull * ns : nullptr, half_voxels,
 		reinterpret_cast<uint32_t*>(e.d_adjm.p), e.adjm_stride * 4,
 		e.mtx2, e.tiles_x, e.tiles_y, e.t_blk_special.p, e.t_blk_corner.p);
+	unsigned long long* h_planes = e.h_plane_out(ns);
+	uint32_t* h_nodes = h_planes ? reinterpret_cast<uint32_t*>(h_planes + 4ull * ns) : nullptr;
 	hipLaunchKernelGGL(k_trail_count_scan, dim3(ns), dim3(kBlock), 0, s, e.t_blk_special.p, e.t_blk_corner.p, e.graph_blocks,
-		e.d_count_vh.p + 2 * static_cast<size_t>(ns), e.d_count_vh.p + 3 * static_cast<size_t>(ns));
+		e.d_count_vh.p + 2 * static_cast<size_t>(ns), e.d_count_vh.p + 3 * static_cast<size_t>(ns), h_nodes, h_nodes ? h_nodes + ns : nullptr);
+	if (e.strips_pending) {
+		CKL_HIP(hipEventRecord(e.ev_counts, s));
+		CKL_HIP(hipStreamWaitEvent(e.stream2, e.ev_counts, 0));
+		strips_enqueue(e, sx, sy, sz, 0xFFFFFFFFu);
+		e.strips_pending = false;
+	}
 	std::vector<unsigned long long> po;
-	if (e.planes_deferred) {
-		po.resize(4ull * ns);
-		CKL_HIP(hipMemcpyAsync(po.data(), e.d_plane_out.p, po.size() * sizeof(unsigned long long), hipMemcpyDeviceToHost, s));
-	}
-	std::vector<uint32_t> c = download(e.d_count_vh.p + 2 * static_cast<size_t>(ns), 2 * static_cast<size_t>(ns), s);
+	std::vector<uint32_t> c(2 * static_cast<size_t>(ns));
+	if (h_nodes) {
+		CKL_HIP(hipStreamSynchronize(s));
+		if (e.planes_deferred) po.assign(h_planes, h_planes + 4ull * ns);
+		memcpy(c.data(), h_nodes, c.size() * sizeof(uint32_t));
+	}
+	else {
+		if (e.planes_deferred) {
+			po.resize(4ull * ns);
+			CKL_HIP(hipMemcpyAsync(po.data(), e.d_plane_out.p, po.size() * sizeof(unsigned long long), hipMemcpyDeviceToHost, s));
+		}
+		c = download(e.d_count_vh.p + 2 * static_cast<size_t>(ns), 2 * static_cast<size_t>(ns), s);
+	}
 	e.count_special.assign(c.begin(), c.begin() + ns);
 	e.count_corner.assign(c.begin() + ns, c.end());
 	VolumeStats v;
@@ -1462,19 +1538,18 @@
 		{ const char* env = getenv("CKL_TRAIL_WALK_STACK"); ta.walk_stack_cap = env ? static_cast<uint32_t>(std::max(1, atoi(env))) : 0xFFFFFFFFu; }
 		if (kTuning && getenv("CKL_TRAIL_DIAG")) { d_tdbg.ensure(16); CKL_HIP(hipMemsetAsync(d_tdbg.p, 0, 128, s)); ta.dbg = d_tdbg.p; ta_dbg = d_tdbg.p; }
 		ta.graph_blocks = e.graph_blocks; ta.blk_special = e.t_blk_special.p; ta.blk_corner = e.t_blk_corner.p;
-		int max_lds = 0;
-		CKL_HIP(hipDeviceGetAttribute(&max_lds, hipDeviceAttributeMaxSharedMemoryPerBlock, e.device));
+		const int max_lds = e.max_lds;
 		const size_t budget = static_cast<size_t>(max_lds > 1024 ? max_lds - 1024 : 0);
 		const uint32_t dart_blocks = (4 * max_ncap + kWalkChunk * kWaves - 1) / (kWalkChunk * kWaves);
 		size_t clds = (static_cast<size_t>(max_special) + 1024) * 4;
 		if (const char* env = getenv("CKL_TRAIL_LDS")) clds = static_cast<size_t>(std::max(0, atoi(env)));
 		clds = (std::min(budget, std::max<size_t>(clds, 1024)) / 16) * 16;
-		CKL_HIP(hipFuncSetAttribute(reinterpret_cast<const void*>(&k_trail_components), hipFuncAttributeMaxDynamicSharedMemorySize, static_cast<int>(clds)));
+		allow_dynamic_lds(reinterpret_cast<const void*>(&k_trail_components), e.device, clds);
 		size_t lds = trail_walk_lds(max_special);
 		if (const char* env = getenv("CKL_TRAIL_LDS")) lds = static_cast<size_t>(std::max(0, atoi(env)));
 		lds = std::min(budget, std::max<size_t>(lds, 4096));
 		lds = (lds / 16) * 16;
-		CKL_HIP(hipFuncSetAttribute(reinterpret_cast<const void*>(&k_trail_walk), hipFuncAttributeMaxDynamicSharedMemorySize, static_cast<int>(lds)));
+		allow_dynamic_lds(reinterpret_cast<const void*>(&k_trail_walk), e.device, lds);
 		trail_lds_used = lds;
 		HT_MARK("c:setup");
 
@@ -1625,7 +1700,7 @@
 	e.d_word_base.ensure(e.plane_words * ns);
 	e.d_parent.ensure(rtot); e.d_run_start.ensure(rtot); e.d_run_cc.ensure(rtot); e.d_comp_pix.ensure(rtot);
 	e.d_nruns.ensure(ns);
-	e.d_flat_report.ensure(4 * static_cast<size_t>(ns));
+	e.d_flat_report.ensure(4 * static_cast<size_t>(ns) + 1);
 	e.d_ncomp.borrow(e.d_flat_report.p, ns); e.d_crc_acc.borrow(e.d_flat_report.p + ns, ns);
 	e.d_idbits.borrow(e.d_flat_report.p + 2 * static_cast<size_t>(ns), ns); e.d_slice_err2.borrow(e.d_flat_report.p + 3 * static_cast<size_t>(ns), ns);
 	CKL_HIP(hipMemsetAsync(e.d_slice_err2.p, 0, ns * sizeof(uint32_t), s));
@@ -1651,18 +1726,93 @@
 	HT_MARK("f:enqueue");
 }
 
+bool strips_eligible(int64_t sx, int64_t sy) {
+	const uint32_t row_words = static_cast<uint32_t>((sx + 31) / 32);
+	if (row_words == 0 || row_words > kStripWords) return false;
+	return strip_shape(static_cast<uint32_t>(sx), static_cast<uint32_t>(sy), row_words).nstrips <= kMaxStrips
+		&& static_cast<uint64_t>(sx) * sy < 0xFFFF0000ull;
+}
+uint32_t strips_fit_rows(const ckl_encoder& e, int64_t sx, int64_t sy) {
+	uint32_t most = 0;
+	for (uint32_t v : e.count_v) most = std::max(most, v);
+	const double runs_per_row = 1.0 + static_cast<double>(most) / static_cast<double>(std::max<int64_t>(sy, 1));
+	const uint32_t fit = static_cast<uint32_t>(0.7 * kStripCap / runs_per_row);
+	const StripShape whole = strip_shape(static_cast<uint32_t>(sx), static_cast<uint32_t>(sy), e.row_words);
+	if (fit >= whole.strip_rows) return whole.strip_rows;
+	if (4 * static_cast<uint64_t>(fit) < whole.strip_rows) return 0;
+	return strip_shape(static_cast<uint32_t>(sx), static_cast<uint32_t>(sy), e.row_words, fit).nstrips <= kMaxStrips ? fit : 0;
+}
+static void strips_views(ckl_encoder& e, int64_t sx, int64_t sy, int64_t sz, RunGeom& g, StripArrays& sa) {
+	const uint32_t ns = static_cast<uint32_t>(sz);
+	g.planeV = e.d_planes.p; g.planeH = e.d_planes.p + e.plane_words * ns;
+	g.row_words = e.row_words; g.plane_words = e.plane_words;
+	g.flip = 1u;
+	g.sx = static_cast<uint32_t>(sx); g.sy = static_cast<uint32_t>(sy);
+	sa = StripArrays{};
+	sa.run_lid = e.s_run_lid.p; sa.sc_w = e.s_sc_w.p;
+	sa.strip_nruns = e.s_strip_nruns.p; sa.strip_nsc = e.s_strip_nsc.p; sa.row_run = e.s_row_run.p;
+	sa.seam_first = e.s_seam_first.p; sa.seam_last = e.s_seam_last.p;
+	sa.slice_err = e.d_slice_err2.p; sa.overflow = e.d_flat_report.p + 4 * static_cast<size_t>(ns);
+	sa.nstrips = e.strip_shape_used.nstrips; sa.strip_rows = e.strip_shape_used.strip_rows; sa.cap = e.strip_shape_used.cap; sa.zbase = 0;
+}
+void strips_enqueue(ckl_encoder& e, int64_t sx, int64_t sy, int64_t sz, uint32_t max_rows) {
+	hipStream_t s = e.stream2;
+	const uint32_t ns = static_cast<uint32_t>(sz);
+	const uint64_t sxy = static_cast<uint64_t>(sx) * sy;
+	ensure_geom_table(e, sxy);
+	const StripShape shape = strip_shape(static_cast<uint32_t>(sx), static_cast<uint32_t>(sy), e.row_words, max_rows);
+	e.strip_shape_used = shape;
+	const size_t nst = static_cast<size_t>(shape.nstrips) * ns;
+	e.s_row_run.ensure(static_cast<size_t>(sy) * ns);
+	e.s_strip_nruns.ensure(nst); e.s_strip_nsc.ensure(nst);
+	e.s_seam_first.ensure(nst * e.row_words); e.s_seam_last.ensure(nst * e.row_words);
+	e.s_run_lid.ensure(nst * shape.cap + 16); e.s_sc_w.ensure(nst * shape.cap); e.s_sc_first.ensure(nst * shape.cap);
+	e.d_flat_report.ensure(4 * static_cast<size_t>(ns) + 1);
+	e.d_ncomp.borrow(e.d_flat_report.p, ns); e.d_crc_acc.borrow(e.d_flat_report.p + ns, ns);
+	e.d_idbits.borrow(e.d_flat_report.p + 2 * static_cast<size_t>(ns), ns); e.d_slice_err2.borrow(e.d_flat_report.p + 3 * static_cast<size_t>(ns), ns);
+	CKL_HIP(hipMemsetAsync(e.d_slice_err2.p, 0, (static_cast<size_t>(ns) + 1) * sizeof(uint32_t), s));
+	RunGeom g;
+	StripArrays sa;
+	strips_views(e, sx, sy, sz, g, sa);
+	hipLaunchKernelGGL(k_strip_ccl_first, dim3(shape.nstrips, ns), dim3(kBlock), 0, s, g, sa, e.d_G.p, static_cast<uint32_t>(sxy), e.s_sc_first.p);
+	e.strips_enqueued = true;
+	HT_MARK("f:strips");
+}
+void strips_resolve(ckl_encoder& e, int64_t sx, int64_t sy, int64_t sz, size_t resolve_lds) {
+	hipStream_t s = e.stream2;
+	const uint32_t ns = static_cast<uint32_t>(sz);
+	uint32_t rcap = resolve_cap_for(resolve_lds);
+	if (const char* env = getenv("CKL_RESOLVE_CAP")) rcap = std::min<uint32_t>(rcap, static_cast<uint32_t>(std::max(1, atoi(env))));
+	rcap = std::max<uint32_t>(rcap, 1u);
+	e.strip_resolve_cap = rcap;
+	e.s_first_pix.ensure(static_cast<size_t>(ns) * rcap);
+	RunGeom g;
+	StripArrays sa;
+	strips_views(e, sx, sy, sz, g, sa);
+	ResolveArgs ra = {};
+	ra.cap = rcap;
+	EncResolveOut en;
+	en.sc_first = e.s_sc_first.p; en.first_pix = e.s_first_pix.p; en.crc_acc = e.d_crc_acc.p; en.idbits = e.d_idbits.p;
+	const size_t tab_bytes = static_cast<size_t>(rcap) * sizeof(uint32_t);
+	allow_dynamic_lds(reinterpret_cast<const void*>(&k_slice_resolve_enc), e.device, tab_bytes);
+	hipLaunchKernelGGL(k_slice_resolve_enc, dim3(ns), dim3(kResolveBlock), tab_bytes, s, g, sa, ra, en, e.d_ncomp.p);
+	HT_MARK("f:resolve");
+}
+
 template <typename LABEL>
-void flat_collect(ckl_encoder& e, const LABEL* labels, int64_t sx, int64_t sy, int64_t sz, FlatResult& out) {
+bool flat_collect(ckl_encoder& e, const LABEL* labels, int64_t sx, int64_t sy, int64_t sz, FlatResult& out, bool strips = false) {
 	hipStream_t s = e.stream2;
 	const uint32_t ns = static_cast<uint32_t>(sz);
 	const uint64_t sxy = static_cast<uint64_t>(sx) * sy;
 	std::vector<uint32_t> acc, idbits, errs;
 	if (e.d_ncomp.p == e.d_flat_report.p && e.d_flat_report.p) {
-		const std::vector<uint32_t> rep = download(e.d_flat_report.p, 4 * static_cast<size_t>(ns), s);
+		const std::vector<uint32_t> rep = download(e.d_flat_report.p, 4 * static_cast<size_t>(ns) + 1, s);
+		e.strip_overflow = strips ? rep[4 * static_cast<size_t>(ns)] : 0u;
+		if (e.strip_overflow) return false;
 		out.ncomp.assign(rep.begin(), rep.begin() + ns);
 		acc.assign(rep.begin() + ns, rep.begin() + 2 * static_cast<size_t>(ns));
 		idbits.assign(rep.begin() + 2 * static_cast<size_t>(ns), rep.begin() + 3 * static_cast<size_t>(ns));
-		errs.assign(rep.begin() + 3 * static_cast<size_t>(ns), rep.end());
+		errs.assign(rep.begin() + 3 * static_cast<size_t>(ns), rep.begin() + 4 * static_cast<size_t>(ns));
 		HT_MARK("f:wait");
 	}
 	else {
@@ -1686,17 +1836,15 @@
 	for (uint32_t zi = 0; zi < ns; zi++) { comp_off[zi] = total; total += out.ncomp[zi]; }
 	upload(e.d_comp_off, comp_off, s);
 	e.d_mapping.ensure(total + 1);
-	RunArrays ra;
-	ra.word_base = e.d_word_base.p; ra.rbase = e.d_rbase.p; ra.rcap = e.d_rcap.p;
-	ra.parent = e.d_parent.p; ra.run_start = e.d_run_start.p; ra.run_cc = e.d_run_cc.p;
-	ra.nruns = e.d_nruns.p; ra.ncomp = e.d_ncomp.p; ra.slice_err = e.d_slice_err2.p;
-	ra.comp_pix = e.d_comp_pix.p;
 	uint32_t max_ncomp = 1;
 	for (uint32_t zi = 0; zi < ns; zi++) max_ncomp = std::max(max_ncomp, out.ncomp[zi]);
-	hipLaunchKernelGGL(k_mapping_comps<LABEL>, dim3((max_ncomp + kBlock - 1) / kBlock, ns), dim3(kBlock), 0, s,
-		labels, ra, sxy, e.d_comp_off.p, e.d_mapping.p);
+	if (strips) hipLaunchKernelGGL(k_mapping_comps<LABEL>, dim3((max_ncomp + kBlock - 1) / kBlock, ns), dim3(kBlock), 0, s,
+		labels, e.d_ncomp.p, e.s_first_pix.p, static_cast<const uint64_t*>(nullptr), static_cast<uint64_t>(e.strip_resolve_cap), sxy, e.d_comp_off.p, e.d_mapping.p);
+	else hipLaunchKernelGGL(k_mapping_comps<LABEL>, dim3((max_ncomp + kBlock - 1) / kBlock, ns), dim3(kBlock), 0, s,
+		labels, e.d_ncomp.p, e.d_comp_pix.p, e.d_rbase.p, 0ull, sxy, e.d_comp_off.p, e.d_mapping.p);
 	CKL_HIP(hipStreamSynchronize(s));
 	out.total = total;
+	return true;
 }
 
 struct PinLabelLists {
@@ -2187,9 +2335,21 @@
 	e.planes_for = nullptr;
 	const bool labels_first = getenv("CKL_NO_OVERLAP") || static_cast<uint64_t>(sx) * sy > (1536ull * 1536ull)
 		|| (getenv("CKL_LABELS_AT_WALK") && atoi(getenv("CKL_LABELS_AT_WALK")) == 0);
-	if (voxels > 0 && !planes_cached) planes_pass<LABEL>(e, labels, sx, sy, sz, &st, !labels_first);
+	const char* enc_labels = getenv("CKL_ENC_LABELS");
+	const bool want_strips = voxels > 0 && enc_labels && (!strcmp(enc_labels, "strips") || !strcmp(enc_labels, "walk")) && strips_eligible(sx, sy);
+	const bool flat_certain = (ov && ov->force_label_format >= 0) ? ov->force_label_format == FLAT
+		: (sz == 1 || !allow_pins || (ov && ov->force_crack_format == PERMISSIBLE));
+	const bool strips_early = want_strips && flat_certain && !getenv("CKL_NO_OVERLAP") && !(enc_labels && !strcmp(enc_labels, "walk"));
+	e.strips_enqueued = false;
+	e.label_strips = e.label_runs = 0;
+	if (voxels > 0 && !planes_cached) planes_pass<LABEL>(e, labels, sx, sy, sz, &st, !labels_first || strips_early);
 	else if (planes_cached) st = e.planes_stats;
+	if (voxels > 0) {
+		CKL_HIP(hipEventRecord(e.ev_planes, s));
+		CKL_HIP(hipStreamWaitEvent(e.stream2, e.ev_planes, 0));
+	}
 	ht.mark("planes");
+	e.strips_pending = strips_early;
 	bool graph_done = false;
 	if (e.planes_deferred) {
 		int perm_mode = 2;
@@ -2239,20 +2399,26 @@
 	if (head.markov_model_order > 13) throw Error(CKL_ERR_ARG, "crackle_amd: markov_model_order > 13 is not supported on device");
 
 	bool labels_at_walk = false;
-	if (labels_first && !graph_done) flat_enqueue(e, sx, sy, sz);
+	const bool use_strips = want_strips && head.label_format == FLAT;
+	if (labels_first && !graph_done && !use_strips) flat_enqueue(e, sx, sy, sz);
 	const bool trail_cached = !graph_done && planes_cached && ov && ov->has_model && head.markov_model_order > 0 && e.trail_for == static_cast<const void*>(labels)
 		&& e.trail_perm == (head.crack_format == PERMISSIBLE) && e.trail_order == head.markov_model_order;
 	e.trail_for = nullptr;
 	if (graph_done && e.graph_permissible != (head.crack_format == PERMISSIBLE)) throw Error(CKL_ERR_RUNTIME, "crackle_amd: internal: device and host disagree on the crack format");
 	if (!trail_cached && !graph_done) graph_pass(e, sx, sy, sz, head.crack_format == PERMISSIBLE ? 1 : 0);
+	e.strips_pending = false;
 	ht.mark("graph");
 	if (!labels_first) {
 		uint32_t max_special = 0;
 		for (uint32_t v : e.count_special) max_special = std::max(max_special, v);
-		int max_lds = 0;
-		CKL_HIP(hipDeviceGetAttribute(&max_lds, hipDeviceAttributeMaxSharedMemoryPerBlock, e.device));
-		labels_at_walk = max_special < 5000 && 2 * trail_walk_lds(max_special) + 40960 <= static_cast<size_t>(max_lds);
-		if (!labels_at_walk) flat_enqueue(e, sx, sy, sz);
+		labels_at_walk = max_special < 5000 && 2 * trail_walk_lds(max_special) + 40960 <= static_cast<size_t>(e.max_lds);
+		if (!labels_at_walk && !use_strips) flat_enqueue(e, sx, sy, sz);
+	}
+	size_t late_resolve_lds = static_cast<uint64_t>(sz) <= static_cast<uint64_t>(std::max(1, e.n_cus)) ? static_cast<size_t>(e.max_lds) - 8192u : static_cast<size_t>(e.max_lds) / 2u - 6144u;
+	if (labels_at_walk) {
+		uint32_t max_special = 0;
+		for (uint32_t v : e.count_special) max_special = std::max(max_special, v);
+		late_resolve_lds = static_cast<size_t>(e.max_lds) - 2 * trail_walk_lds(max_special) - 2048u;
 	}
 
 	const bool permissible = head.crack_format == PERMISSIBLE;
@@ -2298,12 +2464,35 @@
 	const int component_width = byte_width(static_cast<uint64_t>(sx) * sy);
 	hipStream_t s2 = e.stream2;
 	bool labels_stay = false;
+	const uint8_t* section_in_stream = nullptr;
 	auto label_side = [&]() {
-		if (labels_at_walk) {
-			CKL_HIP(hipStreamWaitEvent(s2, e.evd0, 0));
-			flat_enqueue(e, sx, sy, sz);
-		}
-		flat_collect<LABEL>(e, labels, sx, sy, sz, fr);
+		bool by_strips = e.strips_enqueued;
+		const uint32_t fit_rows = use_strips ? strips_fit_rows(e, sx, sy) : 0u;
+		const bool at_walk = !trail_cached && !getenv("CKL_NO_OVERLAP");
+		if (!by_strips && fit_rows) {
+			if (labels_at_walk) CKL_HIP(hipStreamWaitEvent(s2, e.evd0, 0));
+			strips_enqueue(e, sx, sy, sz, fit_rows);
+			by_strips = true;
+		}
+		else if (by_strips && at_walk) CKL_HIP(hipStreamWaitEvent(s2, e.evd0, 0));
+		if (by_strips) {
+			strips_resolve(e, sx, sy, sz, late_resolve_lds);
+			by_strips = flat_collect<LABEL>(e, labels, sx, sy, sz, fr, true);
+		}
+		if (!by_strips && e.strips_enqueued && e.strip_overflow == 1u && fit_rows && fit_rows < e.strip_shape_used.strip_rows) {
+			strips_enqueue(e, sx, sy, sz, fit_rows);
+			strips_resolve(e, sx, sy, sz, late_resolve_lds);
+			by_strips = flat_collect<LABEL>(e, labels, sx, sy, sz, fr, true);
+		}
+		if (by_strips) e.label_strips = static_cast<uint32_t>(sz);
+		else {
+			if (labels_at_walk || use_strips) {
+				if (labels_at_walk) CKL_HIP(hipStreamWaitEvent(s2, e.evd0, 0));
+				flat_enqueue(e, sx, sy, sz);
+			}
+			flat_collect<LABEL>(e, labels, sx, sy, sz, fr);
+			e.label_runs = static_cast<uint32_t>(sz);
+		}
 		HT_MARK("flat");
 		const uint64_t N = fr.total;
 		if (head.label_format == PINS_VARIABLE_WIDTH) {
@@ -2325,6 +2514,9 @@
 				e.d_labels_crc.ensure(1 + kBlock);
 				if (!e.ev_labels_crc) CKL_HIP(hipEventCreateWithFlags(&e.ev_labels_crc, hipEventDisableTiming));
 				crc32c_device(e.d_labels_bin.p, label_bytes, e.d_labels_crc.p + 1, e.d_labels_crc.p, s2);
+				e.d_stream_out.ensure(early_cap + 16);
+				copy_bytes_device(e.d_labels_bin.p, e.d_stream_out.p + off_labels, label_bytes, s2);
+				section_in_stream = e.d_stream_out.p;
 				CKL_HIP(hipEventRecord(e.ev_labels_crc, s2));
 			}
 			else {
@@ -2374,11 +2566,12 @@
 		put4(off_tail, labels_crc);
 		e.device_stream_bytes = 0;
 		if (e.keep_device_stream) {
+			if (section_in_stream && e.d_stream_out.n < total + 16) CKL_HIP(hipEventSynchronize(e.ev_labels_crc));
 			e.d_stream_out.ensure(total + 16);
 			uint8_t* ds = e.d_stream_out.p;
 			const void* up = head.label_format == FLAT ? o : nullptr;
 			upload_small(ds, o, off_labels, s, up);
-			if (label_bytes) {
+			if (label_bytes && section_in_stream != ds) {
 				if (head.label_format == FLAT) copy_bytes_device(e.d_labels_bin.p, ds + off_labels, label_bytes, s);
 				else CKL_HIP(hipMemcpyAsync(ds + off_labels, o + off_labels, label_bytes, hipMemcpyHostToDevice, s));
 			}
@@ -2550,6 +2743,10 @@
 		CKL_HIP(hipEventCreate(&e->evd1));
 		CKL_HIP(hipEventCreateWithFlags(&e->ev_in, hipEventDisableTiming));
 		CKL_HIP(hipEventCreateWithFlags(&e->ev_prezero, hipEventDisableTiming));
+		CKL_HIP(hipEventCreateWithFlags(&e->ev_planes, hipEventDisableTiming));
+		CKL_HIP(hipEventCreateWithFlags(&e->ev_counts, hipEventDisableTiming));
+		CKL_HIP(hipDeviceGetAttribute(&e->max_lds, hipDeviceAttributeMaxSharedMemoryPerBlock, device));
+		CKL_HIP(hipDeviceGetAttribute(&e->n_cus, hipDeviceAttributeMultiprocessorCount, device));
 		*out = e.release();
 		return CKL_OK;
 	}
@@ -2975,6 +3172,13 @@
 	catch (const std::exception& err) { set_last_error(err.what()); return CKL_ERR_RUNTIME; }
 }
 
+int ckl_encoder_label_path(ckl_encoder* e, uint32_t* strip_slices, uint32_t* run_slices) {
+	if (!e) { set_last_error("crackle_amd: null encoder"); return CKL_ERR_ARG; }
+	if (strip_slices) *strip_slices = e->label_strips;
+	if (run_slices) *run_slices = e->label_runs;
+	return CKL_OK;
+}
+
 __global__ void __launch_bounds__(kBlock) k_trail_step_kinds(const uint32_t* __restrict__ events, const uint64_t* __restrict__ ibase, const uint32_t* __restrict__ n_events, uint32_t* __restrict__ counts) {
 	__shared__ uint32_t s_c[5];
 	const uint32_t zi = blockIdx.x;
diff --git a/crackle_amd/csrc/ckl_strips.hpp b/crackle_amd/csrc/ckl_strips.hpp
--- a/crackle_amd/csrc/ckl_strips.hpp
+++ b/crackle_amd/csrc/ckl_strips.hpp
@@ -119,10 +119,10 @@
 }
 
 constexpr uint32_t kStripCclWords = (kStripCap + kStripEdgeCap + kStripWords / 2 + 2 * kStripBitmapWords + kWaves + 2 + 7) & ~7u;
-template <bool DIAG, bool RECORDS>
+template <bool DIAG, bool RECORDS, bool FIRST = false>
 __device__ __forceinline__ void strip_ccl_body(
 	const RunGeom& g, const StripArrays& sa, const RecordLists& rl, const uint32_t* __restrict__ G, uint32_t n_pixels, unsigned long long* __restrict__ diag,
-	uint32_t zi, uint32_t k, uint32_t* lds
+	uint32_t zi, uint32_t k, uint32_t* lds, uint32_t* __restrict__ sc_first = nullptr
 ) {
 	uint32_t* s_parent = lds;
 	uint32_t* s_mem = s_parent + kStripCap;
@@ -243,12 +243,16 @@
 	__syncthreads();
 	stamp(1);
 	uint32_t gv[kStripRunsPerThread];
+	static_assert(kStripRunsPerThread % 2 == 0, "run starts are kept two to a register");
+	uint32_t first_px[FIRST ? kStripRunsPerThread / 2 : 1] = {};
 	{
 		const uint32_t p0 = y0 * g.sx;
 #pragma unroll
 		for (uint32_t i = 0; i < kStripRunsPerThread; i++) {
 			const uint32_t j = t + i * kBlock;
-			gv[i] = G[n_pixels - (p0 + s_pool[j < nloc ? j : 0u])];
+			const uint32_t start = s_pool[j < nloc ? j : 0u];
+			gv[i] = G[n_pixels - (p0 + start)];
+			if (FIRST) first_px[i >> 1] |= start << (16u * (i & 1u));
 		}
 	}
 	{
@@ -331,6 +335,7 @@
 		const uint32_t r = root[i];
 		const uint32_t lid = s_bmbase[r >> 5] + __popc(s_bm[r >> 5] & ((1u << (r & 31u)) - 1u));
 		s_pool[j] = static_cast<uint16_t>(lid);
+		if (FIRST && r == j) sc_first[slot + lid] = y0 * g.sx + ((first_px[i >> 1] >> (16u * (i & 1u))) & 0xFFFFu);
 		if (narrow) reinterpret_cast<uint8_t*>(lid_out)[j] = static_cast<uint8_t>(lid);
 		else lid_out[j] = static_cast<uint16_t>(lid);
 	}
@@ -356,6 +361,23 @@
 static __global__ void __launch_bounds__(kBlock, 7) k_strip_ccl(RunGeom g, StripArrays sa, RecordLists rl, const uint32_t* __restrict__ G, uint32_t n_pixels, unsigned long long* __restrict__ diag) {
 	__shared__ __attribute__((aligned(16))) uint32_t s_lds[kStripCclWords];
 	strip_ccl_body<DIAG, RECORDS>(g, sa, rl, G, n_pixels, diag, blockIdx.y + sa.zbase, blockIdx.x, s_lds);
+}
+
+struct StripShape { uint32_t strip_rows, nstrips, cap; };
+static inline StripShape strip_shape(uint32_t sx, uint32_t sy, uint32_t row_words, uint32_t max_rows = 0xFFFFFFFFu) {
+	StripShape p;
+	p.strip_rows = row_words ? kStripWords / row_words : 1u;
+	p.strip_rows = p.strip_rows < max_rows ? p.strip_rows : max_rows;
+	p.strip_rows = p.strip_rows ? p.strip_rows : 1u;
+	p.nstrips = (sy + p.strip_rows - 1) / p.strip_rows;
+	const uint64_t px = static_cast<uint64_t>(p.strip_rows) * sx;
+	p.cap = static_cast<uint32_t>(px < kStripCap ? px : kStripCap);
+	return p;
+}
+static inline uint32_t resolve_cap_for(size_t lds_bytes) {
+	const size_t fixed = (kMaxStrips + 64u) * 4u;
+	const size_t n = lds_bytes > fixed ? (lds_bytes - fixed) / 4u : 0u;
+	return static_cast<uint32_t>(n < kResolveCap ? n : kResolveCap);
 }
 
 struct ResolveArgs {
@@ -392,11 +414,18 @@
 	}
 }
 
-template <typename OUT, bool LABELS, bool DIAG>
+struct EncResolveOut {
+	const uint32_t* sc_first;
+	uint32_t* first_pix;
+	uint32_t* crc_acc;
+	uint32_t* idbits;
+};
+template <typename OUT, bool LABELS, bool DIAG, bool ENC = false>
 __device__ __forceinline__ bool slice_resolve_body(
 	const RunGeom& g, const StripArrays& sa, const ResolveArgs& ra, uint32_t* __restrict__ ncomp_out, unsigned long long* __restrict__ diag,
-	uint32_t zi, uint32_t* s_tab, uint32_t* s_scbase, uint32_t* s_scan, uint32_t* s_flag_p
+	uint32_t zi, uint32_t* s_tab, uint32_t* s_scbase, uint32_t* s_scan, uint32_t* s_flag_p, const EncResolveOut* en = nullptr
 ) {
+	static_assert(!(ENC && LABELS), "the encoder's resolve looks no labels up");
 	uint32_t& s_flag = *s_flag_p;
 	static_assert(kResolveCap <= 0xFFFFu, "index and rank share a table entry");
 	constexpr int NW = kResolveBlock / kWave;
@@ -500,8 +529,9 @@
 	__syncthreads();
 	stamp(2);
 	const uint32_t ncomp = tot2[0];
-	const uint32_t nexp = ra.ncomp_expect[zi];
-	const uint64_t coff = ra.comp_off[zi];
+	const uint32_t nexp = ENC ? 0u : ra.ncomp_expect[zi];
+	const uint64_t coff = ENC ? 0ull : ra.comp_off[zi];
+	const uint32_t idbits = ENC ? (ncomp > 1u ? 32u - __clz(ncomp - 1u) : 1u) : ra.idbits;
 	uint32_t part = 0;
 	uint32_t sidx = strip0;
 	for (uint32_t r0 = i0; r0 < i1; r0 += kPer) {
@@ -546,9 +576,12 @@
 				if (ra.has_label) val = (val == ra.label);
 				static_cast<OUT*>(sa.sc_label)[gi[q]] = static_cast<OUT>(val);
 			}
+			else if (ENC) {
+				if ((s_tab[r0 + q] & 0xFFFFu) == r0 + q) en->first_pix[static_cast<uint64_t>(zi) * ra.cap + cc[q]] = en->sc_first[gi[q]];
+			}
 			else sa.sc_cc[gi[q]] = cc[q];
 			uint32_t wg = wgt[q];
-			for (int j = static_cast<int>(ra.idbits) - 1; j >= 0; j--) {
+			for (int j = static_cast<int>(idbits) - 1; j >= 0; j--) {
 				part ^= ((cc[q] >> j) & 1u) ? wg : 0u;
 				wg = (wg >> 1) ^ ((wg & 1u) ? kCrcPoly : 0u);
 			}
@@ -560,6 +593,12 @@
 	if (t == 0) {
 		uint32_t x = 0;
 		for (int wv = 0; wv < NW; wv++) x ^= s_scan[wv];
+		if (ENC) {
+			ncomp_out[zi] = ncomp;
+			en->crc_acc[zi] = x;
+			en->idbits[zi] = idbits;
+			return true;
+		}
 		uint32_t e = 0;
 		if (ncomp != nexp) e |= ERR_NCOMP;
 		else if (ra.check_crc && gf_mul(x, ra.crc_fix) != ra.crc_expect[zi]) e |= ERR_CRC;
diff --git a/crackle_amd/csrc/ckl_trail.hpp b/crackle_amd/csrc/ckl_trail.hpp
--- a/crackle_amd/csrc/ckl_trail.hpp
+++ b/crackle_amd/csrc/ckl_trail.hpp
@@ -242,7 +242,8 @@
 
 static __global__ void __launch_bounds__(kBlock) k_trail_count_scan(
 	uint32_t* __restrict__ blk_special, uint32_t* __restrict__ blk_corner, uint32_t nblk,
-	uint32_t* __restrict__ tot_special, uint32_t* __restrict__ tot_corner
+	uint32_t* __restrict__ tot_special, uint32_t* __restrict__ tot_corner,
+	uint32_t* __restrict__ host_special, uint32_t* __restrict__ host_corner
 ) {
 	__shared__ uint32_t s_scan[2 * kWaves];
 	const uint32_t zi = blockIdx.x;
@@ -256,7 +257,10 @@
 		if (b < nblk) { bs[b] = cs + v[0]; bc[b] = cc + v[1]; }
 		cs += tot[0]; cc += tot[1];
 	}
-	if (threadIdx.x == 0) { tot_special[zi] = cs; tot_corner[zi] = cc; }
+	if (threadIdx.x == 0) {
+		tot_special[zi] = cs; tot_corner[zi] = cc;
+		if (host_special) { host_special[zi] = cs; host_corner[zi] = cc; }
+	}
 }
 
 static __global__ void __launch_bounds__(kBlock) k_trail_nodes(TrailArgs a) {
diff --git a/crackle_amd/distributed.py b/crackle_amd/distributed.py
--- a/crackle_amd/distributed.py
+++ b/crackle_amd/distributed.py
@@ -463,6 +463,12 @@
     if self._enc and self._L.ckl_encoder_walk_paths(self._enc, C.byref(f), C.byref(c)) != _lib.CKL_OK:
       raise RuntimeError(_lib.last_error())
     return f.value, c.value
+
+  def label_path(self) -> Tuple[int, int]:
+    a, b = C.c_uint32(), C.c_uint32()
+    if self._enc and self._L.ckl_encoder_label_path(self._enc, C.byref(a), C.byref(b)) != _lib.CKL_OK:
+      raise RuntimeError(_lib.last_error())
+    return a.value, b.value
 
   def walk_step_kinds(self, max_slices: int = 1 << 16):
     buf = (C.c_uint32 * (5 * max_slices))()
diff --git a/include/crackle_amd.h b/include/crackle_amd.h
--- a/include/crackle_amd.h
+++ b/include/crackle_amd.h
@@ -163,6 +163,7 @@
 
 int ckl_encoder_last_timing(const ckl_encoder* e, float* pipeline_ms, float* dominant_kernel_ms);
 int ckl_encoder_walk_paths(ckl_encoder* e, uint32_t* fast_slices, uint32_t* compiled_slices);
+int ckl_encoder_label_path(ckl_encoder* e, uint32_t* strip_slices, uint32_t* run_slices);
 int ckl_encoder_walk_step_kinds(ckl_encoder* e, uint32_t* counts, uint32_t max_slices, uint32_t* n_slices);
 void ckl_encoder_destroy(ckl_encoder* e);
 
```

Measured after the change: 151.5 billion, median of 6. 1.0% higher.
